# kuwt/model_matching

Measured on AMD Instinct MI355X. Metric: candidate poses verified/sec, higher is better.
Workload: dtype f32; 1 GPU; Cm: synthetic 20000-pt scene vs 5000-pt model, 65536 candidate transforms per step per GPU, eps=5mm; scene_points=20000, model_points=5000

## Files before the change

### include/stocs_hip.h

```cpp
#ifndef STOCS_HIP_H
#define STOCS_HIP_H

#include <stdint.h>

#ifdef __cplusplus
extern "C" {
#endif

typedef struct stocs_ctx stocs_ctx;

typedef enum stocs_status {
    STOCS_OK = 0,
    STOCS_ERR_INVALID = -1,
    STOCS_ERR_NO_DEVICE = -2,
    STOCS_ERR_HIP = -3,
    STOCS_ERR_CAPACITY = -4,
    STOCS_ERR_STATE = -5,
    STOCS_ERR_NOMEM = -6
} stocs_status;

typedef struct stocs_params {
    float distance_threshold;
    int   ppf_tr_discretization;
    int   ppf_rot_discretization;
    float plane_threshold;
    float min_distance_base;
    float internal_angle_threshold;
    float lcp_normal_angle;
    int   image_width, image_height;
    int   number_of_bases;
    int   maximum_congruent_sets;
} stocs_params;

void stocs_default_params(stocs_params* p);
const char* stocs_last_error(void);
const char* stocs_version(void);

int stocs_ctx_create(const stocs_params* prm,
                     const float* scene_pos3, const float* scene_nrm3, const float* scene_prob,
                     const int32_t* scene_pixel2, int nS,
                     const float* model_pos3, const float* model_nrm3, int nM,
                     int build_index, int device, stocs_ctx** out);
int stocs_ctx_destroy(stocs_ctx* ctx);
int stocs_ctx_set_scene(stocs_ctx* ctx, const float* scene_pos3, const float* scene_nrm3, const float* scene_prob,
                        const int32_t* scene_pixel2, int nS);

int stocs_get_centroids(const stocs_ctx* ctx, float* scene3, float* model3);
int stocs_get_sizes(const stocs_ctx* ctx, int* nS, int* nM);
int stocs_set_edge_map(stocs_ctx* ctx, const uint8_t* edge);
int stocs_reset_trial(stocs_ctx* ctx);

int stocs_ppf_compute_host(const float* p1, const float* n1, const float* p2, const float* n2,
                           int tr, int rot, int32_t* key4);
int stocs_index_exists(const stocs_ctx* ctx, const int32_t* key4, int* exists);
int stocs_index_lookup(stocs_ctx* ctx, const int32_t* key4, int32_t* pairs2, int64_t cap, int64_t* n);
int stocs_index_stats(const stocs_ctx* ctx, int64_t* n_pairs, int64_t* n_buckets, int64_t* n_keys);
int stocs_index_save(stocs_ctx* ctx, const char* path);
int stocs_index_load(stocs_ctx* ctx, const char* path);

int stocs_sample_bases(stocs_ctx* ctx, int mode, uint64_t seed, int first_attempt, int n_attempts,
                       float dispersion, int32_t* base_ids4, float* inv2, int32_t* valid);
int stocs_get_segment(const stocs_ctx* ctx, int32_t* scene_idx, int cap, int* n);
int stocs_get_scene(const stocs_ctx* ctx, float* pos3_centred, float* nrm3, float* class_prob, int32_t* pixel2);
int stocs_set_bases(stocs_ctx* ctx, int n, const int32_t* base_ids4, const float* inv2);
int stocs_clear_bases(stocs_ctx* ctx);
int stocs_num_bases(const stocs_ctx* ctx);
int stocs_class_pass(stocs_ctx* ctx, int pass, const int32_t* b3, const float* w_in, float* w_out);
int stocs_ppf_filter_check(stocs_ctx* ctx, uint64_t seed, int64_t n_pairs, int64_t* n_tested, int64_t* n_undecided, int64_t* n_mismatch);
int stocs_weight_fix_check(stocs_ctx* ctx, int64_t* n_mismatch);
int stocs_try_sampled_base(stocs_ctx* ctx, int32_t* ids4_inout, float* inv2, int* valid);
int stocs_draw(stocs_ctx* ctx, const float* w, int n, uint64_t r64, int* index);
enum { STOCS_FORM_LEAN = 0, STOCS_FORM_FULL_LDS = 1, STOCS_FORM_FULL_DEVICE_MEMORY = 2, STOCS_FORM_NINE_LAUNCH = 3, STOCS_FORM_INSTANCE_LDS = 4,
       STOCS_FORM_INSTANCE_DEVICE_MEMORY = 5 };
int stocs_last_sampling_form(const stocs_ctx* ctx, int* kernel, int* threads, int64_t* lds_bytes, int* cap, int* launches, int* redone);
int stocs_last_instance_attempts(stocs_ctx* ctx, int32_t* rec4, int cap, int* n);
int stocs_debug_draw_point1(stocs_ctx* ctx, const uint64_t* r64, int n, int32_t* index);

int stocs_find_congruent_all(stocs_ctx* ctx, int64_t* total_quads);
int stocs_get_quads(stocs_ctx* ctx, int base_slot, int32_t* quads4, int64_t cap, int64_t* n);
int stocs_get_quads_at(stocs_ctx* ctx, int base_slot, const int64_t* ranks, int n, int32_t* quads4);

int stocs_cone_cells_host(const float* n3, float cos_alpha, uint32_t* exact_bits11, uint32_t* kernel_bits11, int* n_samples,
                          int* n_undecided);

int stocs_make_transforms(stocs_ctx* ctx, int max_per_base, uint64_t seed, int* n_candidates);
int stocs_rigid_transform(stocs_ctx* ctx, const int32_t* ids4, const int32_t* quad4,
                          float* T16_centred, float* pose16_camera, int* ok);
int stocs_get_candidates(stocs_ctx* ctx, float* T16_centred, float* pose16_camera, float* lcp,
                         int32_t* base_index, int cap, int* n);

int stocs_score_transforms(stocs_ctx* ctx, const float* T16_centred_host, int n, float* lcp_host);
int stocs_score_transforms_device(stocs_ctx* ctx, const void* d_T16, int n, void* d_lcp);
int stocs_score_best_device(stocs_ctx* ctx, const void* d_T16, int n, void* d_lcp, uint32_t id_offset, uint64_t* key);
int stocs_score_best_device_async(stocs_ctx* ctx, const void* d_T16, int n, void* d_lcp, uint32_t id_offset, void* d_key8);
int stocs_lcp_detail(stocs_ctx* ctx, const float* T16_centred_host, int32_t* hit, uint8_t* counted);
int stocs_lcp_hit_count(stocs_ctx* ctx, const void* d_T16, int n, int64_t* hits, int64_t* counted);
int stocs_verify_all(stocs_ctx* ctx, float* best_lcp, int* best_idx, float* best_pose16_camera);
typedef struct stocs_trial_result {
    int32_t n_bases;
    int32_t n_candidates;
    int64_t n_quads;
    float   best_lcp;
    int32_t best_index;
    float   best_pose16[16];
} stocs_trial_result;
int stocs_run_trials(stocs_ctx* ctx, int mode, int n_trials, const uint64_t* seeds, int n_attempts, float dispersion, int max_per_base,
                     int keep_details, stocs_trial_result* out );
int stocs_trials_get_bases(stocs_ctx* ctx, int trial, int32_t* base_ids4, float* inv2, int32_t* valid, int cap_attempts, int* n_attempts);
int stocs_trials_get_quad_counts(stocs_ctx* ctx, int trial, int64_t* counts, int cap, int* n);
int stocs_trials_get_candidates(stocs_ctx* ctx, int trial, float* T16_centred, float* pose16_camera, float* lcp, int32_t* base_index, int cap, int* n);
typedef struct stocs_trial_post {
    float   acceptable_fraction;
    int32_t maximum_pose_count;
    float   min_distance, min_angle;
    float   sym3[3];
    int32_t refine_iterations;
    float   max_correspondence_distance;
} stocs_trial_post;
int stocs_run_trials_post(stocs_ctx* ctx, int mode, int n_trials, const uint64_t* seeds, int n_attempts, float dispersion, int max_per_base,
                          int keep_details, const stocs_trial_post* post , stocs_trial_result* out );
typedef struct stocs_trial_hypothesis {
    int32_t candidate_index, base_index;
    float   lcp, pose16[16];
    float   refined_lcp, refined_pose16[16];
    int32_t n_correspondences, iterations;
} stocs_trial_hypothesis;
int stocs_trials_get_hypotheses(stocs_ctx* ctx, int trial, stocs_trial_hypothesis* out, int cap, int* n);

int stocs_best_device(stocs_ctx* ctx, const void* d_lcp, int n, uint32_t id_offset, uint64_t* key);
uint64_t stocs_pack_best(float lcp, uint32_t global_candidate_id);
void stocs_unpack_best(uint64_t key, float* lcp, uint32_t* global_candidate_id);

typedef struct stocs_comm stocs_comm;
int stocs_comm_unique_id(void* id128);
int stocs_comm_create(const void* id128, int nranks, int rank, int device, stocs_comm** out);
int stocs_comm_destroy(stocs_comm* comm);
int stocs_allreduce_best(stocs_comm* comm, void* hip_stream, uint64_t* key_inout, float* pose16_inout, uint32_t ids_per_rank);

int stocs_cluster_poses(const float* poses16, const float* lcp, int n, float acceptable_fraction,
                        float best_score, int maximum_pose_count, float min_distance, float min_angle,
                        const float* sym3, int32_t* out_idx, int cap, int* n_out);
int stocs_cluster_trials_device(stocs_ctx* ctx, const float* poses16, const float* lcp, const int32_t* cand_off, const float* best_score, int n_trials,
                                float acceptable_fraction, int maximum_pose_count, float min_distance, float min_angle, const float* sym3,
                                int32_t* out_off, int32_t* out_cnt, int32_t* out_idx, int out_cap, int32_t* round0_survivors);

enum {
    STOCS_NORMALS_DEPTH_GRADIENT = 0,
    STOCS_NORMALS_PLANE_FIT = 1
};
typedef struct stocs_camera {
    float fx, cx, fy, cy;
    float depth_scale;
    int width, height;
    int normal_method;
} stocs_camera;
int stocs_ingest_scene(const stocs_camera* cam, const uint16_t* depth, const uint16_t* class_prob, float voxel_size,
                       float class_threshold, int device, float* pos3, float* nrm3, float* prob, int32_t* pixel2,
                       int cap, int* n_out);
#define STOCS_MAX_FRAME_OBJECTS 64
int stocs_ingest_scene_multi(const stocs_camera* cam, const uint16_t* depth, int n_objects, const uint16_t* class_probs,
                             const float* class_thresholds, float voxel_size, int device, float* pos3, float* nrm3, float* prob,
                             int32_t* pixel2, int cap, int32_t* offsets);
int stocs_preprocess_model(const float* raw_pos3, int n_raw, float normal_radius, float voxel_size, float model_scale,
                           int device, float* pos3, float* nrm3, int cap, int* n_out);
int stocs_trim(void);

int stocs_png_read(const char* path, int* width, int* height, int* channels, int* bit_depth, void* pixels, int64_t cap_bytes);
int stocs_ply_read(const char* path, float* pos3, float* nrm3, int cap, int* n, int* has_normals);
int stocs_ply_write(const char* path, const float* pos3, const float* nrm3, int n, float scale);

int stocs_icp_point_to_plane(const float* src_pos3, int nsrc, const float* tgt_pos3, const float* tgt_nrm3, int ntgt,
                             int max_iterations, float max_correspondence_distance, int device, float* T16_out,
                             int* n_correspondences);

int stocs_refine_poses(stocs_ctx* ctx, const float* T16_centred_in, int n, const int32_t* src_idx, int n_src, int max_iterations,
                       float max_correspondence_distance, float* T16_centred_out, float* pose16_camera_out, float* lcp_out,
                       int32_t* n_corr_out, int32_t* iterations_out);

int stocs_refine_detail(stocs_ctx* ctx, const float* T16_centred, const int32_t* src_idx, int n_src, float max_correspondence_distance,
// ... 152 lines not shown
```

### model_matching_amd/capi.py

```python
from __future__ import annotations

import ctypes as C
import os

import numpy as np

_HERE = os.path.dirname(os.path.abspath(__file__))
LIB_PATH = os.path.join(_HERE, "libstocs_hip.so")

STOCS_OK = 0
ERR_INVALID, ERR_CAPACITY, ERR_STATE = -1, -4, -5
FORM_NAMES = {0: "lean", 1: "full_lds", 2: "full_device_memory", 3: "nine_launch", 4: "instance_lds", 5: "instance_device_memory"}
ERR_NAMES = {0: "OK", -1: "INVALID", -2: "NO_DEVICE", -3: "HIP", -4: "CAPACITY", -5: "STATE", -6: "NOMEM"}


class StocsError(RuntimeError):
    def __init__(self, code, msg):
        super().__init__("stocs_hip error %s: %s" % (ERR_NAMES.get(code, code), msg))
        self.code = code


class Params(C.Structure):
    _fields_ = [("distance_threshold", C.c_float), ("ppf_tr_discretization", C.c_int),
                ("ppf_rot_discretization", C.c_int), ("plane_threshold", C.c_float),
# ... 50 lines not shown
    _fields_ = [("max_instances", C.c_int32), ("min_points", C.c_int32), ("min_exclusive_fraction", C.c_float)]


class InstanceResult(C.Structure):
    _fields_ = [("rank", C.c_int32), ("own", C.c_int32), ("exclusive", C.c_int32), ("lcp", C.c_float)]


class RenderParams(C.Structure):
    _fields_ = [("point_radius", C.c_float), ("max_splat_px", C.c_int32), ("tolerance", C.c_float), ("class_threshold", C.c_float)]


class RenderResult(C.Structure):
    _fields_ = [("footprint", C.c_int32), ("visible", C.c_int32), ("hidden", C.c_int32), ("no_depth", C.c_int32), ("agree", C.c_int32),
                ("in_front", C.c_int32), ("behind", C.c_int32), ("on_mask", C.c_int32)]


class SceneRecord(C.Structure):
    _fields_ = [("footprint", C.c_int32), ("no_depth", C.c_int32), ("agree", C.c_int32), ("in_front", C.c_int32), ("behind", C.c_int32),
                ("on_mask", C.c_int32), ("claimed", C.c_int32)]


class SceneParams(C.Structure):
    _fields_ = [("max_selected", C.c_int32), ("min_pixels", C.c_int32), ("min_exclusive_fraction", C.c_float), ("max_violation_fraction", C.c_float)]


class SceneResult(C.Structure):
    _fields_ = [("rank", C.c_int32), ("own", C.c_int32), ("exclusive", C.c_int32), ("reason", C.c_int32)]


class Camera(C.Structure):
    _fields_ = [("fx", C.c_float), ("cx", C.c_float), ("fy", C.c_float), ("cy", C.c_float), ("depth_scale", C.c_float),
                ("width", C.c_int), ("height", C.c_int), ("normal_method", C.c_int)]


_fp, _ip, _u8p, _vp = C.POINTER(C.c_float), C.POINTER(C.c_int32), C.POINTER(C.c_uint8), C.c_void_p
_i64p = C.POINTER(C.c_int64)
_intp = C.POINTER(C.c_int)
SIGNATURES = {
    "stocs_default_params": (None, [C.POINTER(Params)]),
    "stocs_last_error": (C.c_char_p, []),
    "stocs_version": (C.c_char_p, []),
    "stocs_ctx_create": (C.c_int, [C.POINTER(Params), _fp, _fp, _fp, _ip, C.c_int, _fp, _fp, C.c_int, C.c_int, C.c_int, C.POINTER(_vp)]),
    "stocs_ctx_destroy": (C.c_int, [_vp]),
    "stocs_ctx_set_scene": (C.c_int, [_vp, _fp, _fp, _fp, _ip, C.c_int]),
    "stocs_get_centroids": (C.c_int, [_vp, _fp, _fp]),
    "stocs_get_sizes": (C.c_int, [_vp, _intp, _intp]),
    "stocs_set_edge_map": (C.c_int, [_vp, _u8p]),
    "stocs_reset_trial": (C.c_int, [_vp]),
    "stocs_ppf_compute_host": (C.c_int, [_fp, _fp, _fp, _fp, C.c_int, C.c_int, _ip]),
    "stocs_index_exists": (C.c_int, [_vp, _ip, _intp]),
    "stocs_index_lookup": (C.c_int, [_vp, _ip, _ip, C.c_int64, _i64p]),
    "stocs_index_stats": (C.c_int, [_vp, _i64p, _i64p, _i64p]),
    "stocs_index_save": (C.c_int, [_vp, C.c_char_p]),
    "stocs_index_load": (C.c_int, [_vp, C.c_char_p]),
    "stocs_sample_bases": (C.c_int, [_vp, C.c_int, C.c_uint64, C.c_int, C.c_int, C.c_float, _ip, _fp, _ip]),
    "stocs_get_segment": (C.c_int, [_vp, _ip, C.c_int, _intp]),
    "stocs_get_scene": (C.c_int, [_vp, _fp, _fp, _fp, _ip]),
    "stocs_png_read": (C.c_int, [C.c_char_p, _intp, _intp, _intp, _intp, _vp, C.c_int64]),
    "stocs_ply_read": (C.c_int, [C.c_char_p, _fp, _fp, C.c_int, _intp, _intp]),
    "stocs_ply_write": (C.c_int, [C.c_char_p, _fp, _fp, C.c_int, C.c_float]),
    "stocs_set_bases": (C.c_int, [_vp, C.c_int, _ip, _fp]),
    "stocs_clear_bases": (C.c_int, [_vp]),
    "stocs_num_bases": (C.c_int, [_vp]),
    "stocs_class_pass": (C.c_int, [_vp, C.c_int, _ip, _fp, _fp]),
    "stocs_ppf_filter_check": (C.c_int, [_vp, C.c_uint64, C.c_int64, _i64p, _i64p, _i64p]),
    "stocs_weight_fix_check": (C.c_int, [_vp, _i64p]),
    "stocs_try_sampled_base": (C.c_int, [_vp, _ip, _fp, _intp]),
    "stocs_draw": (C.c_int, [_vp, _fp, C.c_int, C.c_uint64, _intp]),
    "stocs_last_sampling_form": (C.c_int, [_vp, _intp, _intp, _i64p, _intp, _intp, _intp]),
    "stocs_last_instance_attempts": (C.c_int, [_vp, _ip, C.c_int, _intp]),
    "stocs_debug_draw_point1": (C.c_int, [_vp, C.POINTER(C.c_uint64), C.c_int, _ip]),
    "stocs_find_congruent_all": (C.c_int, [_vp, _i64p]),
    "stocs_get_quads": (C.c_int, [_vp, C.c_int, _ip, C.c_int64, _i64p]),
    "stocs_get_quads_at": (C.c_int, [_vp, C.c_int, _i64p, C.c_int, _ip]),
    "stocs_cone_cells_host": (C.c_int, [_fp, C.c_float, C.POINTER(C.c_uint32), C.POINTER(C.c_uint32), _intp, _intp]),
    "stocs_make_transforms": (C.c_int, [_vp, C.c_int, C.c_uint64, _intp]),
    "stocs_rigid_transform": (C.c_int, [_vp, _ip, _ip, _fp, _fp, _intp]),
    "stocs_get_candidates": (C.c_int, [_vp, _fp, _fp, _fp, _ip, C.c_int, _intp]),
    "stocs_score_transforms": (C.c_int, [_vp, _fp, C.c_int, _fp]),
    "stocs_score_transforms_device": (C.c_int, [_vp, _vp, C.c_int, _vp]),
    "stocs_score_best_device": (C.c_int, [_vp, _vp, C.c_int, _vp, C.c_uint32, C.POINTER(C.c_uint64)]),
    "stocs_lcp_detail": (C.c_int, [_vp, _fp, _ip, _u8p]),
    "stocs_lcp_hit_count": (C.c_int, [_vp, _vp, C.c_int, _i64p, _i64p]),
    "stocs_verify_all": (C.c_int, [_vp, _fp, _intp, _fp]),
    "stocs_run_trials": (C.c_int, [_vp, C.c_int, C.c_int, C.POINTER(C.c_uint64), C.c_int, C.c_float, C.c_int, C.c_int, C.POINTER(TrialResult)]),
    "stocs_trials_get_bases": (C.c_int, [_vp, C.c_int, _ip, _fp, _ip, C.c_int, _intp]),
    "stocs_trials_get_quad_counts": (C.c_int, [_vp, C.c_int, _i64p, C.c_int, _intp]),
    "stocs_trials_get_candidates": (C.c_int, [_vp, C.c_int, _fp, _fp, _fp, _ip, C.c_int, _intp]),
    "stocs_run_trials_post": (C.c_int, [_vp, C.c_int, C.c_int, C.POINTER(C.c_uint64), C.c_int, C.c_float, C.c_int, C.c_int, C.POINTER(TrialPost),
                                        C.POINTER(TrialResult)]),
    "stocs_trials_get_hypotheses": (C.c_int, [_vp, C.c_int, C.POINTER(TrialHypothesis), C.c_int, _intp]),
    "stocs_best_device": (C.c_int, [_vp, _vp, C.c_int, C.c_uint32, C.POINTER(C.c_uint64)]),
    "stocs_pack_best": (C.c_uint64, [C.c_float, C.c_uint32]),
    "stocs_unpack_best": (None, [C.c_uint64, _fp, C.POINTER(C.c_uint32)]),
    "stocs_comm_unique_id": (C.c_int, [_vp]),
    "stocs_comm_create": (C.c_int, [_vp, C.c_int, C.c_int, C.c_int, C.POINTER(_vp)]),
    "stocs_comm_destroy": (C.c_int, [_vp]),
    "stocs_allreduce_best": (C.c_int, [_vp, _vp, C.POINTER(C.c_uint64), _fp, C.c_uint32]),
    "stocs_cluster_poses": (C.c_int, [_fp, _fp, C.c_int, C.c_float, C.c_float, C.c_int, C.c_float, C.c_float, _fp, _ip, C.c_int, _intp]),
    "stocs_cluster_trials_device": (C.c_int, [_vp, _fp, _fp, _ip, _fp, C.c_int, C.c_float, C.c_int, C.c_float, C.c_float, _fp, _ip, _ip, _ip, C.c_int, _ip]),
    "stocs_ingest_scene": (C.c_int, [C.POINTER(Camera), C.POINTER(C.c_uint16), C.POINTER(C.c_uint16), C.c_float, C.c_float, C.c_int, _fp, _fp, _fp, _ip, C.c_int, _intp]),
    "stocs_ingest_scene_multi": (C.c_int, [C.POINTER(Camera), C.POINTER(C.c_uint16), C.c_int, C.POINTER(C.c_uint16), _fp, C.c_float, C.c_int, _fp, _fp, _fp, _ip,
                                           C.c_int, _ip]),
    "stocs_preprocess_model": (C.c_int, [_fp, C.c_int, C.c_float, C.c_float, C.c_float, C.c_int, _fp, _fp, C.c_int, _intp]),
    "stocs_trim": (C.c_int, []),
    "stocs_icp_point_to_plane": (C.c_int, [_fp, C.c_int, _fp, _fp, C.c_int, C.c_int, C.c_float, C.c_int, _fp, _intp]),
    "stocs_refine_poses": (C.c_int, [_vp, _fp, C.c_int, _ip, C.c_int, C.c_int, C.c_float, _fp, _fp, _fp, _ip, _ip]),
    "stocs_refine_detail": (C.c_int, [_vp, _fp, _ip, C.c_int, C.c_float, _ip, _u8p, C.POINTER(C.c_double)]),
    "stocs_refine_poses_robust": (C.c_int, [_vp, _fp, C.c_int, _ip, C.c_int, C.POINTER(RefineRobustParams), _fp, _fp, _fp, _ip, _ip, _ip]),
    "stocs_refine_robust_detail": (C.c_int, [_vp, _fp, _ip, C.c_int, C.POINTER(RefineRobustParams), _ip, _u8p, _u8p, C.POINTER(C.c_uint32), _ip, _ip,
                                             C.POINTER(C.c_double)]),
    "stocs_refine_robust_workspace": (C.c_int, [_vp, C.POINTER(C.c_void_p), C.POINTER(C.c_uint64)]),
    "stocs_track_poses": (C.c_int, [_vp, _fp, C.c_int, C.POINTER(TrackParams), C.POINTER(TrackResult)]),
    "stocs_track_get_round": (C.c_int, [_vp, C.c_int, C.c_int, _fp, _fp, C.c_int, _intp]),
    "stocs_ctx_set_frame": (C.c_int, [_vp, C.POINTER(Camera), C.POINTER(C.c_uint16), C.POINTER(C.c_uint16)]),
    "stocs_default_depth_params": (None, [C.POINTER(DepthParams)]),
    "stocs_depth_check_poses": (C.c_int, [_vp, _fp, C.c_int, C.POINTER(DepthParams), C.POINTER(DepthResult)]),
    "stocs_pose_errors": (C.c_int, [_vp, _fp, C.c_int, _fp, C.c_int, C.POINTER(PoseError)]),
    "stocs_pose_errors_detail": (C.c_int, [_vp, _fp, _fp, _fp, _fp, _ip]),
    "stocs_model_diameter": (C.c_int, [_vp, _fp]),
    "stocs_default_render_params": (None, [C.POINTER(RenderParams)]),
    "stocs_render_poses": (C.c_int, [_vp, _fp, C.c_int, C.c_int, C.POINTER(RenderParams), _vp, C.c_int]),
    "stocs_render_resolve": (C.c_int, [_vp, _fp, C.c_int, C.c_int, C.POINTER(RenderParams), _vp, C.POINTER(RenderResult)]),
    "stocs_render_labels": (C.c_int, [_vp, _vp, C.POINTER(RenderParams), _ip, _u8p]),
    "stocs_explain_poses": (C.c_int, [_vp, _fp, C.c_int, C.POINTER(RenderParams), C.POINTER(RenderResult), _ip, _u8p]),
    "stocs_default_instance_params": (None, [C.POINTER(InstanceParams)]),
    "stocs_select_instances": (C.c_int, [_vp, _fp, C.c_int, C.POINTER(InstanceParams), C.POINTER(InstanceResult), _ip, _intp]),
    "stocs_select_instances_rows": (C.c_int, [_vp, _ip, _u8p, _fp, C.c_int, C.c_int, C.c_int, C.POINTER(InstanceParams), C.POINTER(InstanceResult), _ip, _intp]),
    "stocs_default_scene_params": (None, [C.POINTER(SceneParams)]),
    "stocs_scene_row_words": (C.c_int, [C.c_int, C.c_int]),
    "stocs_scene_footprints": (C.c_int, [_vp, _fp, C.c_int, C.c_int, C.c_int, C.POINTER(RenderParams), C.c_int, _vp, C.POINTER(SceneRecord)]),
    "stocs_scene_select": (C.c_int, [_vp, _vp, C.c_int, C.c_int, C.c_int, _fp, _ip, C.POINTER(SceneRecord), C.c_int, _ip, C.POINTER(SceneParams),
                                     C.POINTER(SceneResult), _ip, _intp]),
    "stocs_device_alloc_count": (C.c_int64, []),
    "stocs_debug_stream_audit_selftest": (C.c_int, [C.c_int, C.c_char_p, C.c_int]),
    "stocs_debug_streams_overlap": (C.c_int, [_vp]),
    "stocs_debug_sort_pairs": (C.c_int, [C.c_int, C.POINTER(C.c_uint32), C.POINTER(C.c_uint32), C.c_int64, C.c_int, C.c_int, C.c_int, C.POINTER(C.c_uint32), C.POINTER(C.c_uint32), _fp, C.POINTER(C.c_uint32), C.c_int]),
    "stocs_last_call_timing": (C.c_int, [_vp, C.c_int, C.POINTER(C.c_char_p), C.POINTER(C.c_double), C.c_int, _intp]),
    "stocs_set_option": (C.c_int, [_vp, C.c_char_p, C.c_int]),
    "stocs_get_cull_state": (C.c_int, [_vp, _fp, _ip, _intp, _fp, _fp, C.c_int64, _i64p]),
    "stocs_model_patch_order": (C.c_int, [_fp, C.c_int, _ip, _fp]),
    "stocs_model_subpatches": (C.c_int, [_fp, C.c_int, _ip, _fp]),
    "stocs_kdtree_nn_host": (C.c_int, [_fp, C.c_int, _fp, C.c_int, C.c_float, _ip]),
    "stocs_last_tie_counts": (C.c_int, [_vp, _i64p, _i64p]),
    "stocs_set_stream": (C.c_int, [_vp, _vp]),
    "stocs_best_device_async": (C.c_int, [_vp, _vp, C.c_int, C.c_uint32, _vp]),
    "stocs_score_best_device_async": (C.c_int, [_vp, _vp, C.c_int, _vp, C.c_uint32, _vp]),
    "stocs_sync": (C.c_int, [_vp]),
    "stocs_stream": (_vp, [_vp]),
    "stocs_time_score_kernel": (C.c_int, [_vp, _vp, C.c_int, _vp, C.c_int, _fp]),
    "stocs_dev_alloc": (C.c_int, [_vp, C.c_int64, C.POINTER(_vp)]),
    "stocs_dev_free": (C.c_int, [_vp, _vp]),
    "stocs_dev_upload": (C.c_int, [_vp, _vp, _vp, C.c_int64]),
    "stocs_dev_download": (C.c_int, [_vp, _vp, _vp, C.c_int64]),
}

_LIB = None


def load():
    global _LIB
    if _LIB is None:
        if not os.path.exists(LIB_PATH):
            raise ImportError("%s is missing: build it with `python -c 'import __graft_entry__ as g; g.build()'` "
                              "(make -C model_matching_amd/csrc).  There is no CPU fallback." % LIB_PATH)
        L = C.CDLL(LIB_PATH)
# ... 30 lines not shown
```

### model_matching_amd/csrc/ctx.hip

```cpp
#include <math.h>
#include <stdarg.h>
#include <string.h>
#include <stdlib.h>

#include <algorithm>
#include <limits>
#include <numeric>

#include "stocs_ctx.h"

namespace stocs {

static thread_local char g_err[512] = "";
unsigned long long g_dev_allocs = 0;

void set_error(const char* fmt, ...) {
    va_list ap;
    va_start(ap, fmt);
    vsnprintf(g_err, sizeof(g_err), fmt, ap);
    va_end(ap);
}

__global__ void overlap_wait_kernel(unsigned int* flag, unsigned int* seen) {
    const unsigned long long t0 = wall_clock64();
// ... 380 lines not shown
    float r_ref = 0.0f;
    model_patch_order(mpos, munit, perm, patch, sub, &r_ref);
}

}

using namespace stocs;

extern "C" {

const char* stocs_last_error(void) { return g_err; }
const char* stocs_version(void) { return "stocs_hip 0.1 (gfx950)"; }

void stocs_default_params(stocs_params* p) {
    p->distance_threshold = 0.005f;
    p->ppf_tr_discretization = 5;
    p->ppf_rot_discretization = 5;
    p->plane_threshold = 0.015f;
    p->min_distance_base = 0.01f;
    p->internal_angle_threshold = 30.0f;
    p->lcp_normal_angle = 30.0f;
    p->image_width = 640;
    p->image_height = 480;
    p->number_of_bases = 100;
    p->maximum_congruent_sets = 200;
}

int stocs_ctx_create(const stocs_params* prm, const float* sp, const float* sn, const float* sprob,
                     const int32_t* spix, int nS, const float* mp, const float* mn, int nM, int build_index,
                     int device, stocs_ctx** out) {
    if (!prm || !out || nS < 0 || nM < 0 || (nS && (!sp || !sn || !sprob)) || (nM && (!mp || !mn))) {
        set_error("stocs_ctx_create: invalid argument");
        return STOCS_ERR_INVALID;
    }
    if (nS == 0 || nM == 0) {
        set_error("stocs_ctx_create: empty scene or model cloud");
        return STOCS_ERR_INVALID;
    }
    if (nM > 65535) { set_error("model has %d points; at most 65535 supported (16-bit ids in packed pairs)", nM); return STOCS_ERR_INVALID; }
    if (prm->ppf_rot_discretization <= 0 || prm->ppf_tr_discretization <= 0 || 180 % prm->ppf_rot_discretization) {
        set_error("PPF discretisation must be positive and divide 180");
        return STOCS_ERR_INVALID;
    }
    *out = NULL;
    int ndev = 0;
    if (hipGetDeviceCount(&ndev) != hipSuccess || ndev <= 0) {
        set_error("no HIP device available: this library has no CPU fallback");
        return STOCS_ERR_NO_DEVICE;
    }
    if (device < 0) { if (hipGetDevice(&device) != hipSuccess) device = 0; }
    if (device >= ndev) { set_error("device %d out of range (%d devices)", device, ndev); return STOCS_ERR_NO_DEVICE; }
    DeviceGuard dev_guard(device);
    { int cur = -1; if (hipGetDevice(&cur) != hipSuccess || cur != device) { set_error("hipSetDevice(%d) failed", device); return STOCS_ERR_NO_DEVICE; } }

    stocs_ctx* c = new stocs_ctx();
    c->prm = *prm;
    c->device = device;
    c->nS = nS; c->nM = nM;
    c->d_scratch = NULL; c->scratch_bytes = 0;
    c->h_pin = NULL; c->pin_bytes = 0;
    for (int k = 0; k < 5; ++k) c->timing[k].n = 0;
    c->index.built = false;
    c->index.d_bucket_start = NULL; c->index.d_pairs = NULL; c->index.d_exists = NULL;
    c->cong = NULL; c->quad_id_bits = 16;
    c->refine = NULL;
    c->track = NULL;
    c->depth = NULL;
    c->instances = NULL;
    c->render = NULL;
    c->scene = NULL;
    c->pose_error = NULL;
    c->inst = NULL;
    c->trials = NULL; c->snrmw_trial0 = NULL; c->snrmw_stride = 0; c->snrmw_override = NULL; c->lcp_cand_trial = NULL;
    c->d_cand = NULL; c->cand_bytes = 0; c->n_cands = 0; c->cand_cap = 0; c->cands_stale = false;
    c->d_best = NULL; c->best_is_zero = false;
    c->best_lcp = 0; c->best_index = -1;
    c->has_edge = false;
    c->grid_div = 1;
    c->grid_prune = getenv("STOCS_GRID_PRUNE") ? atoi(getenv("STOCS_GRID_PRUNE")) : 1;
    c->lcp_variant = -1;
    c->device_clock = (getenv("STOCS_DEVICE_CLOCK") && atoi(getenv("STOCS_DEVICE_CLOCK")) != 0) ? 1 : 0;
    c->lcp_split = 1;
    c->lcp_flat = getenv("STOCS_LCP_FLAT") ? atoi(getenv("STOCS_LCP_FLAT")) : 1;
    c->lcp_order = getenv("STOCS_LCP_ORDER") ? atoi(getenv("STOCS_LCP_ORDER")) : 1;
    c->exact_ties = 0; c->kd_ready = false; c->d_kd_nodes = NULL; c->d_kd_pts = NULL; c->d_ties = NULL; c->ties_started = false;
    c->cdf_n = 0; c->prior_epoch = 1; c->cdf_epoch = 0;
    c->last_form.kernel = -1; c->last_form.threads = 0; c->last_form.lds = 0; c->last_form.cap = 0; c->last_form.launches = 0; c->last_form.redone = 0;
    memset(&c->grid, 0, sizeof(c->grid));
    c->d_spos = c->d_snrmw = c->d_mpos = c->d_mnrm = c->d_munit = c->d_mpos_raw = c->d_mpos_s = c->d_mnrm_s = NULL;
    c->d_spix = NULL; c->d_mperm = NULL; c->d_mpatch = NULL; c->d_msub = NULL; c->d_scene_mem = NULL; c->scene_cap = 0;
    c->patch_r_ref = 0.0f; c->scene_scored = 0; c->scene_work = 0.0;
    c->lcp_cull = getenv("STOCS_LCP_CULL") ? atoi(getenv("STOCS_LCP_CULL")) : 1;
    c->lcp_cull_unit = 16;
    c->lcp_cull_after = 1.0e9; c->prev_scene_warm = false; c->cull_pending = false; c->ev_cull = NULL;
    c->stream = NULL; c->own_stream = NULL; c->aux_stream = NULL;
    if (hipStreamCreateWithFlags(&c->own_stream, hipStreamNonBlocking) != hipSuccess || hipStreamCreateWithFlags(&c->aux_stream, hipStreamNonBlocking) != hipSuccess ||
        hipEventCreate(&c->ev0) != hipSuccess || hipEventCreate(&c->ev1) != hipSuccess ||
        hipEventCreateWithFlags(&c->ev_fork, hipEventDisableTiming) != hipSuccess || hipEventCreateWithFlags(&c->ev_join, hipEventDisableTiming) != hipSuccess ||
        hipEventCreateWithFlags(&c->ev_cull, hipEventDisableTiming) != hipSuccess) {
        set_error("stream/event creation failed");
        delete c;
        return STOCS_ERR_NO_DEVICE;
    }
    for (int k = 0; k < 10; ++k)
        if (hipEventCreate(&c->ev_t[k]) != hipSuccess) { set_error("event creation failed"); delete c; return STOCS_ERR_NO_DEVICE; }
    if (!getenv("STOCS_NO_STREAM_PROBE")) {
        hipStream_t spare[4]; int n_spare = 0;
        while (!streams_run_side_by_side(c->own_stream, c->aux_stream) && n_spare < 4) {
            hipStream_t s2 = NULL;
            if (hipStreamCreateWithFlags(&s2, hipStreamNonBlocking) != hipSuccess) { (void)hipGetLastError(); break; }
            spare[n_spare++] = c->aux_stream;
            c->aux_stream = s2;
        }
        for (int k = 0; k < n_spare; ++k) (void)hipStreamDestroy(spare[k]);
        if (getenv("STOCS_DEBUG_TIMING")) fprintf(stderr, "[stocs ctx] auxiliary stream: candidate %d runs next to the main stream\n", n_spare + 1);
    }
    c->stream = c->own_stream;
    compute_thresholds(c->prm, &c->thr);

    c->h_mpos.resize(nM); c->h_mnrm.resize(nM); c->h_mpos_raw.resize(nM);
    for (int i = 0; i < nM; ++i) {
        c->h_mpos_raw[i] = c->h_mpos[i] = mk3(mp[3 * i], mp[3 * i + 1], mp[3 * i + 2]);
        c->h_mnrm[i] = normalized3(mk3(mn[3 * i], mn[3 * i + 1], mn[3 * i + 2]));
    }
    V3 cm = mk3(0, 0, 0);
    for (int i = 0; i < nM; ++i) cm = cm + c->h_mpos[i];
    cm = cm / (float)nM;
    for (int i = 0; i < nM; ++i) c->h_mpos[i] = c->h_mpos[i] - cm;
    c->centroid_model = cm;

    {
        const float big = std::numeric_limits<float>::max() / 2;
        V3 bmn = mk3(big, big, big), bmx = mk3(-big, -big, -big);
        for (int i = 0; i < nM; ++i) {
            const V3 q = c->h_mpos[i];
            if (q.x < bmn.x) bmn.x = q.x; if (q.y < bmn.y) bmn.y = q.y; if (q.z < bmn.z) bmn.z = q.z;
            if (q.x > bmx.x) bmx.x = q.x; if (q.y > bmx.y) bmx.y = q.y; if (q.z > bmx.z) bmx.z = q.z;
        }
        c->gcenter = bmn + ((bmx - bmn) / 2.0f);
        const V3 ext = bmx - bmn;
        const double r = std::max((double)ext.z + 0.001, std::max((double)ext.y + 0.001, (double)ext.x + 0.001));
        c->ratio = (float)r;
        c->h_munit.resize(nM);
        const V3 half = mk3(0.5f, 0.5f, 0.5f);
        for (int i = 0; i < nM; ++i) c->h_munit[i] = (c->h_mpos[i] - c->gcenter) / c->ratio + half;
    }

    std::vector<float4> patch, sub;
    model_patch_order(c->h_mpos, c->h_munit, c->h_mperm, patch, sub, &c->patch_r_ref);
    const int n_patch = (nM + 63) / 64;

    int rc = STOCS_OK;
    {
        const int n = std::max(nM, 1);
        std::vector<float4> a(n), b(n), u(n), raw(n), as(n), bs(n);
        for (int i = 0; i < nM; ++i) {
            a[i] = make_float4(c->h_mpos[i].x, c->h_mpos[i].y, c->h_mpos[i].z, 0.f);
            b[i] = make_float4(c->h_mnrm[i].x, c->h_mnrm[i].y, c->h_mnrm[i].z, 0.f);
            u[i] = make_float4(c->h_munit[i].x, c->h_munit[i].y, c->h_munit[i].z, 0.f);
            raw[i] = make_float4(c->h_mpos_raw[i].x, c->h_mpos_raw[i].y, c->h_mpos_raw[i].z, 0.f);
        }
        for (int i = 0; i < nM; ++i) { as[i] = a[c->h_mperm[i]]; bs[i] = b[c->h_mperm[i]]; }
        as.resize((size_t)n_patch * 64 + 64, make_float4(NAN, NAN, NAN, 0.f));
        if (!rc) rc = upload(&c->d_mpos, a.data(), a.size());
        if (!rc) rc = upload(&c->d_mnrm, b.data(), b.size());
        if (!rc) rc = upload(&c->d_munit, u.data(), u.size());
        if (!rc) rc = upload(&c->d_mpos_raw, raw.data(), raw.size());
        if (!rc) rc = upload(&c->d_mpos_s, as.data(), as.size());
        if (!rc) rc = upload(&c->d_mnrm_s, bs.data(), bs.size());
        if (!rc) rc = upload(&c->d_mperm, c->h_mperm.data(), c->h_mperm.size());
        if (!rc) rc = upload(&c->d_mpatch, patch.data(), patch.size());
        if (!rc) rc = upload(&c->d_msub, sub.data(), sub.size());
    }
    if (!rc) rc = load_scene(c, sp, sn, sprob, spix, nS);
    if (!rc && build_index) rc = build_ppf_index(c);
    if (rc) { stocs_ctx_destroy(c); return rc; }
    *out = c;
    return STOCS_OK;
}

int stocs_model_patch_order(const float* model_pos3, int nM, int32_t* perm, float* patches4) {
    if (!model_pos3 || nM <= 0 || !perm || !patches4) return STOCS_ERR_INVALID;
    std::vector<int32_t> pm; std::vector<float4> patch, sub;
    model_patch_order_host(model_pos3, nM, pm, patch, sub);
    for (int i = 0; i < nM; ++i) perm[i] = pm[i];
    for (int s = 0; s < (nM + 63) / 64; ++s) { patches4[4 * s] = patch[s].x; patches4[4 * s + 1] = patch[s].y; patches4[4 * s + 2] = patch[s].z; patches4[4 * s + 3] = patch[s].w; }
    return STOCS_OK;
}

int stocs_model_subpatches(const float* model_pos3, int nM, int32_t* perm, float* spheres4) {
    if (!model_pos3 || nM <= 0 || !perm || !spheres4) return STOCS_ERR_INVALID;
    std::vector<int32_t> pm; std::vector<float4> patch, sub;
    model_patch_order_host(model_pos3, nM, pm, patch, sub);
    for (int i = 0; i < nM; ++i) perm[i] = pm[i];
    for (int q = 0; q < (nM + 15) / 16; ++q) { spheres4[4 * q] = sub[q].x; spheres4[4 * q + 1] = sub[q].y; spheres4[4 * q + 2] = sub[q].z; spheres4[4 * q + 3] = sub[q].w; }
    return STOCS_OK;
}

int stocs_ctx_destroy(stocs_ctx* c) {
    if (!c) return STOCS_OK;
    DeviceGuard dev_guard(c->device);
    if (c->stream) (void)hipStreamSynchronize(c->stream);
    void* ptrs[] = {c->d_scene_mem, c->d_mpos, c->d_mnrm, c->d_munit, c->d_mpos_raw, c->d_mpos_s,
                    c->d_mnrm_s, c->d_mperm, c->d_mpatch, c->d_msub, c->index.d_bucket_start,
                    c->index.d_pairs, c->index.d_exists, c->d_scratch, c->d_best, c->d_cand};
    stocs_internal_free_congruent(c);
    stocs_internal_free_instance(c);
    stocs_internal_free_trials(c);
    stocs_internal_free_refine(c);
    stocs_internal_free_track(c);
    stocs_internal_free_depth(c);
    stocs_internal_free_instances(c);
    stocs_internal_free_render(c);
    stocs_internal_free_scene(c);
    stocs_internal_free_pose_error(c);
    c->grid_mem.destroy(); c->grid_ws.destroy();
    c->order.free(); c->cdf.free(); c->kd.free();
    if (c->h_pin) (void)hipHostFree(c->h_pin);
    for (void* p : ptrs) if (p) (void)hipFree(p);
    (void)hipEventDestroy(c->ev0);
    (void)hipEventDestroy(c->ev1);
    (void)hipEventDestroy(c->ev_fork);
    (void)hipEventDestroy(c->ev_join);
    if (c->ev_cull) (void)hipEventDestroy(c->ev_cull);
    for (int k = 0; k < 10; ++k) (void)hipEventDestroy(c->ev_t[k]);
    if (c->aux_stream) { (void)hipStreamSynchronize(c->aux_stream); (void)hipStreamDestroy(c->aux_stream); }
    if (c->own_stream) (void)hipStreamDestroy(c->own_stream);
    delete c;
    return STOCS_OK;
}

int stocs_ctx_set_scene(stocs_ctx* c, const float* sp, const float* sn, const float* sprob, const int32_t* spix, int nS) {
    if (!c || nS <= 0 || !sp || !sn || !sprob) { set_error("stocs_ctx_set_scene: invalid argument"); return STOCS_ERR_INVALID; }
    DeviceGuard dev_guard(c->device);
    STOCS_HIP_CHECK(hipStreamSynchronize(c->stream));
    return load_scene(c, sp, sn, sprob, spix, nS);
}

int stocs_get_centroids(const stocs_ctx* c, float* s, float* m) {
    if (!c) return STOCS_ERR_INVALID;
    if (s) { s[0] = c->centroid_scene.x; s[1] = c->centroid_scene.y; s[2] = c->centroid_scene.z; }
    if (m) { m[0] = c->centroid_model.x; m[1] = c->centroid_model.y; m[2] = c->centroid_model.z; }
    return STOCS_OK;
}
int stocs_get_scene(const stocs_ctx* c, float* pos3, float* nrm3, float* prob, int32_t* pix2) {
    if (!c) return STOCS_ERR_INVALID;
// ... 114 lines not shown
```

### model_matching_amd/csrc/grid.hip

```cpp
#include <math.h>
#include <string.h>
#include <cstring>


#include <algorithm>
#include <vector>

#include "prims.h"
#include "stocs_ctx.h"

namespace stocs {

struct GridGeom {
    double of[3];
    double h, r;
    int n[3];
    int nbx, nby;
    int dense;
    double qscale;
};

__device__ __forceinline__ void cell_range(const GridGeom& G, const double p[3], int lo[3], int hi[3]) {
#pragma unroll
    for (int k = 0; k < 3; ++k) {
        lo[k] = max(0, (int)floor((p[k] - G.r - G.of[k]) / G.h));
        hi[k] = min(G.n[k] - 1, (int)floor((p[k] + G.r - G.of[k]) / G.h));
    }
}

__device__ __forceinline__ double box_dist2(const GridGeom& G, const double p[3], int cx, int cy, int cz) {
    const int cc[3] = {cx, cy, cz};
    double d2 = 0;
#pragma unroll
    for (int k = 0; k < 3; ++k) {
        const double b0 = G.of[k] + cc[k] * G.h, b1 = b0 + G.h;
        const double d = p[k] < b0 ? b0 - p[k] : (p[k] > b1 ? p[k] - b1 : 0.0);
        d2 += d * d;
    }
    return d2;
}

template <bool FILL>
__global__ __launch_bounds__(256) void incidence_kernel(GridGeom G, const float4* __restrict__ spos, int nS, uint32_t* __restrict__ cnt,
                                                        const unsigned long long* __restrict__ off, uint64_t* __restrict__ keys,
                                                        uint32_t* __restrict__ vals, uint32_t* __restrict__ keys32 = NULL) {
    const int i = blockIdx.x * blockDim.x + threadIdx.x;
    if (i >= nS) return;
    const float4 pf = spos[i];
    const double p[3] = {pf.x, pf.y, pf.z};
    int lo[3], hi[3];
    cell_range(G, p, lo, hi);
    uint32_t c = 0;
    unsigned long long o = FILL ? off[i] : 0ull;
    for (int cz = lo[2]; cz <= hi[2]; ++cz)
        for (int cy = lo[1]; cy <= hi[1]; ++cy)
            for (int cx = lo[0]; cx <= hi[0]; ++cx) {
                if (box_dist2(G, p, cx, cy, cz) > G.r * G.r) continue;
                if (FILL) {
                    const uint64_t brick = ((uint64_t)(cz >> 3) * G.nby + (uint64_t)(cy >> 3)) * G.nbx + (uint64_t)(cx >> 3);
                    uint64_t key = (brick << 9) | (uint64_t)(((cz & 7) << 6) | ((cy & 7) << 3) | (cx & 7));
                    if (G.dense) {
                        const double dx = p[0] - (G.of[0] + (cx + 0.5) * G.h), dy = p[1] - (G.of[1] + (cy + 0.5) * G.h),
                                     dz = p[2] - (G.of[2] + (cz + 0.5) * G.h);
                        const double q = sqrt(dx * dx + dy * dy + dz * dz) * G.qscale;
                        key = (key << 16) | (uint64_t)(q < 65535.0 ? (unsigned)q : 65535u);
                    }
                    if (keys32) keys32[o + c] = (uint32_t)key; else keys[o + c] = key;
                    vals[o + c] = (uint32_t)i;
                }
                c++;
            }
    if (!FILL) cnt[i] = c;
}

__global__ __launch_bounds__(256) void widen_keys_kernel(const uint32_t* __restrict__ k32, size_t n, uint64_t* __restrict__ k64) {
    const size_t e = (size_t)blockIdx.x * blockDim.x + threadIdx.x;
    if (e < n) k64[e] = (uint64_t)k32[e];
}

__global__ __launch_bounds__(256) void cell_flags_kernel(const uint64_t* __restrict__ keys, size_t n, int qbits, uint32_t* __restrict__ cflag,
                                                         uint32_t* __restrict__ bflag) {
    const size_t e = (size_t)blockIdx.x * blockDim.x + threadIdx.x;
    if (e >= n) return;
    const uint64_t ck = keys[e] >> qbits;
    const uint64_t pk = e ? (keys[e - 1] >> qbits) : ~0ull;
    cflag[e] = (e == 0 || ck != pk) ? 1u : 0u;
    bflag[e] = (e == 0 || (ck >> 9) != (pk >> 9)) ? 1u : 0u;
}

__global__ __launch_bounds__(256) void cell_records_kernel(const uint64_t* __restrict__ keys, size_t n, int qbits, const uint32_t* __restrict__ cflag,
                                                           const uint32_t* __restrict__ cidx, const uint32_t* __restrict__ bflag,
                                                           const uint32_t* __restrict__ bidx, uint32_t* __restrict__ cell_first, uint64_t* __restrict__ cell_key,
                                                           uint32_t* __restrict__ cell_brick) {
    const size_t e = (size_t)blockIdx.x * blockDim.x + threadIdx.x;
    if (e >= n || !cflag[e]) return;
    const uint32_t c = cidx[e];
    cell_first[c] = (uint32_t)e;
    cell_key[c] = keys[e] >> qbits;
    cell_brick[c] = bidx[e] + bflag[e] - 1u;
}

__global__ __launch_bounds__(256) void cell_padded_kernel(const uint32_t* __restrict__ cell_first, uint32_t n_cells, uint32_t n_inc, uint32_t pad,
                                                          uint32_t* __restrict__ padded, uint32_t* __restrict__ max_count) {
    const uint32_t c = blockIdx.x * blockDim.x + threadIdx.x;
    if (c >= n_cells) return;
    const uint32_t cnt = (c + 1 < n_cells ? cell_first[c + 1] : n_inc) - cell_first[c];
    padded[c] = (cnt + pad - 1u) & ~(pad - 1u);
    atomicMax(max_count, cnt);
}

__global__ __launch_bounds__(256) void fill_i32_kernel(int32_t* __restrict__ a, size_t n, int32_t v) {
    const size_t i = (size_t)blockIdx.x * blockDim.x + threadIdx.x;
    if (i < n) a[i] = v;
}
__global__ __launch_bounds__(256) void fill_list_kernel(float4* __restrict__ a, size_t n) {
    const size_t i = (size_t)blockIdx.x * blockDim.x + threadIdx.x;
    if (i < n) a[i] = make_float4(1.0e30f, 1.0e30f, 1.0e30f, __int_as_float(-1));
}
__global__ __launch_bounds__(256) void zero_cells_kernel(uint4* __restrict__ a, size_t n) {
    const size_t i = (size_t)blockIdx.x * blockDim.x + threadIdx.x;
    if (i < n) a[i] = make_uint4(0u, 0u, 0u, 0u);
}

__global__ __launch_bounds__(256) void cell_words_kernel(GridGeom G, int div, const uint32_t* __restrict__ cell_first, const uint64_t* __restrict__ cell_key,
                                                         const uint32_t* __restrict__ cell_brick, const uint32_t* __restrict__ list_off,
                                                         uint32_t n_cells, uint32_t n_inc, const uint32_t* __restrict__ vals,
                                                         const float4* __restrict__ spos, int32_t* __restrict__ top, uint4* __restrict__ cells,
                                                         uint4* __restrict__ flat, const uint32_t* __restrict__ kept) {
    const uint32_t c = blockIdx.x * 4 + (threadIdx.x >> 6);
    const int s = threadIdx.x & 63;
    if (c >= n_cells) return;
    const uint32_t first = cell_first[c];
    const uint32_t cnt = (c + 1 < n_cells ? cell_first[c + 1] : n_inc) - first;
    const uint64_t key = cell_key[c];
    const uint64_t brick = key >> 9;
    const uint32_t local = (uint32_t)(key & 511);
    const uint32_t b = cell_brick[c];
    uint32_t mlo = 0xFFFFFFFFu, mhi = 0xFFFFFFFFu;
    if (div == 1) {
        const int bx = (int)(brick % (uint64_t)G.nbx), by = (int)((brick / (uint64_t)G.nbx) % (uint64_t)G.nby),
                  bz = (int)(brick / ((uint64_t)G.nbx * (uint64_t)G.nby));
        const int cx = bx * 8 + (int)(local & 7), cy = by * 8 + (int)((local >> 3) & 7), cz = bz * 8 + (int)(local >> 6);
        const double hs = G.h / 4.0;
        const int sc[3] = {4 * cx + (s & 3), 4 * cy + ((s >> 2) & 3), 4 * cz + (s >> 4)};
        bool any = false;
        for (uint32_t k = 0; k < cnt && !any; ++k) {
            const float4 pf = spos[vals[first + k]];
            const double p[3] = {pf.x, pf.y, pf.z};
            double d2 = 0;
#pragma unroll
            for (int a = 0; a < 3; ++a) {
                const double b0 = G.of[a] + sc[a] * hs, b1 = b0 + hs;
                const double d = p[a] < b0 ? b0 - p[a] : (p[a] > b1 ? p[a] - b1 : 0.0);
                d2 += d * d;
            }
            any = d2 <= G.r * G.r;
        }
        const unsigned long long m = __ballot(any);
        mlo = (uint32_t)(m & 0xFFFFFFFFull); mhi = (uint32_t)(m >> 32);
    }
    if (s == 0) {
        top[brick] = (int32_t)b;
        const uint4 w = make_uint4(list_off[c], kept ? kept[c] : cnt, mlo, mhi);
        cells[(size_t)b * 512 + local] = w;
        if (flat) {
            const int bx = (int)(brick % (uint64_t)G.nbx), by = (int)((brick / (uint64_t)G.nbx) % (uint64_t)G.nby), bz = (int)(brick / ((uint64_t)G.nbx * (uint64_t)G.nby));
            const int cx = bx * 8 + (int)(local & 7), cy = by * 8 + (int)((local >> 3) & 7), cz = bz * 8 + (int)(local >> 6);
            if (cx < G.n[0] && cy < G.n[1] && cz < G.n[2]) flat[((size_t)cz * G.n[1] + cy) * G.n[0] + cx] = w;
        }
    }
}

__global__ __launch_bounds__(256) void list_fill_kernel(const uint32_t* __restrict__ cflag, const uint32_t* __restrict__ cidx,
                                                        const uint32_t* __restrict__ cell_first, const uint32_t* __restrict__ list_off,
                                                        const uint32_t* __restrict__ vals, size_t n, const float4* __restrict__ spos,
                                                        float4* __restrict__ list, const uint32_t* __restrict__ rank) {
    const size_t e = (size_t)blockIdx.x * blockDim.x + threadIdx.x;
    if (e >= n) return;
    if (rank) {
        const uint32_t r = rank[e];
        if (r == 0xFFFFFFFFu) return;
        const uint32_t c = cidx[e] + cflag[e] - 1u;
        const uint32_t pt = vals[e];
        const float4 p = spos[pt];
        list[(size_t)list_off[c] + r] = make_float4(p.x, p.y, p.z, __int_as_float((int)pt));
        return;
    }
    const uint32_t c = cidx[e] + cflag[e] - 1u;
    const uint32_t pt = vals[e];
    const float4 p = spos[pt];
    list[(size_t)list_off[c] + (e - cell_first[c])] = make_float4(p.x, p.y, p.z, __int_as_float((int)pt));
}

__global__ __launch_bounds__(256) void chunk_bounds_kernel(GridGeom G, const uint32_t* __restrict__ cell_first, const uint64_t* __restrict__ cell_key,
                                                           const uint32_t* __restrict__ list_off, uint32_t n_cells, uint32_t n_inc,
                                                           const float4* __restrict__ list, float* __restrict__ chunk_r) {
    const uint32_t c = blockIdx.x * blockDim.x + threadIdx.x;
    if (c >= n_cells) return;
    const uint32_t cnt = (c + 1 < n_cells ? cell_first[c + 1] : n_inc) - cell_first[c];
    const uint64_t key = cell_key[c];
    const uint64_t brick = key >> 9;
    const uint32_t local = (uint32_t)(key & 511);
    const int bx = (int)(brick % (uint64_t)G.nbx), by = (int)((brick / (uint64_t)G.nbx) % (uint64_t)G.nby),
              bz = (int)(brick / ((uint64_t)G.nbx * (uint64_t)G.nby));
    const int cx = bx * 8 + (int)(local & 7), cy = by * 8 + (int)((local >> 3) & 7), cz = bz * 8 + (int)(local >> 6);
    const double ccx = G.of[0] + (cx + 0.5) * G.h, ccy = G.of[1] + (cy + 0.5) * G.h, ccz = G.of[2] + (cz + 0.5) * G.h;
    const uint32_t o = list_off[c];
    double run = 1e300;
    for (int k = (int)cnt - 1; k >= 0; --k) {
        const float4 e = list[(size_t)o + k];
        const double dx = e.x - ccx, dy = e.y - ccy, dz = e.z - ccz;
        run = fmin(run, sqrt(dx * dx + dy * dy + dz * dz));
        if ((k & 7) == 0) chunk_r[(o + (uint32_t)k) >> 3] = (float)(run - (2e-6 + 2.5e-7 * run));
    }
}

__global__ __launch_bounds__(256) void cell_nearest_kernel(const uint64_t* __restrict__ cell_key, const uint32_t* __restrict__ cell_brick, const uint32_t* __restrict__ list_off,
                                                           uint32_t n_cells, const float* __restrict__ chunk_r, uint4* __restrict__ cells) {
    const uint32_t c = blockIdx.x * blockDim.x + threadIdx.x;
    if (c >= n_cells) return;
    cells[(size_t)cell_brick[c] * 512 + (uint32_t)(cell_key[c] & 511)].z = __float_as_uint(chunk_r[list_off[c] >> 3]);
}


template <int PRUNE_K, int GS>
__global__ __launch_bounds__(256) void prune_kernel(GridGeom G, double hh, double margin, const uint32_t* __restrict__ cell_first, const uint64_t* __restrict__ cell_key,
                                                    uint32_t n_cells, uint32_t n_inc, const uint32_t* __restrict__ vals, const float4* __restrict__ spos,
                                                    uint32_t* __restrict__ rank, uint32_t* __restrict__ kept, float* __restrict__ nearest) {
    const uint32_t c = blockIdx.x * (256u / GS) + (threadIdx.x / GS);
    const int lane = threadIdx.x & (GS - 1), wlane = threadIdx.x & 63;
    const bool cell_ok = c < n_cells;
    const uint32_t first = cell_ok ? cell_first[c] : 0u;
    const uint32_t cnt = cell_ok ? (c + 1 < n_cells ? cell_first[c + 1] : n_inc) - first : 0u;
    const uint64_t key = cell_ok ? cell_key[c] : 0ull;
    const uint64_t brick = key >> 9;
    const uint32_t local = (uint32_t)(key & 511);
    const int bx = (int)(brick % (uint64_t)G.nbx), by = (int)((brick / (uint64_t)G.nbx) % (uint64_t)G.nby), bz = (int)(brick / ((uint64_t)G.nbx * (uint64_t)G.nby));
    const int cx = bx * 8 + (int)(local & 7), cy = by * 8 + (int)((local >> 3) & 7), cz = bz * 8 + (int)(local >> 6);
    const double ccx = G.of[0] + (cx + 0.5) * G.h, ccy = G.of[1] + (cy + 0.5) * G.h, ccz = G.of[2] + (cz + 0.5) * G.h;
    double ux0 = 0, uy0 = 0, uz0 = 0, n20 = 0;
    if ((uint32_t)lane < cnt) {
        const float4 pf = spos[vals[first + (uint32_t)lane]];
        ux0 = (double)pf.x - ccx; uy0 = (double)pf.y - ccy; uz0 = (double)pf.z - ccz;
        n20 = ux0 * ux0 + uy0 * uy0 + uz0 * uz0;
    }
    double dux[PRUNE_K], duy[PRUNE_K], duz[PRUNE_K], dn2[PRUNE_K];
// ... 36 lines not shown
        const uint32_t k = k0 + (uint32_t)lane;
        bool keep = false;
        if (k < cnt) {
            double ux = ux0, uy = uy0, uz = uz0, n2 = n20;
            if (k0) {
                const float4 pf = spos[vals[first + k]];
                ux = (double)pf.x - ccx; uy = (double)pf.y - ccy; uz = (double)pf.z - ccz;
                n2 = ux * ux + uy * uy + uz * uz;
            }
            keep = true;
#pragma unroll
            for (int j = 0; j < PRUNE_K; ++j) {
                if (j < nd) {
                    const double fmin_ = (n2 - dn2[j]) - 2.0 * hh * (fabs(ux - dux[j]) + fabs(uy - duy[j]) + fabs(uz - duz[j]));
                    if (fmin_ > margin) keep = false;
                }
            }
        }
        unsigned long long m = __ballot(keep);
        if (GS < 64) m = (m >> (wlane & ~(GS - 1))) & ((1ull << GS) - 1ull);
        if (k < cnt) rank[first + k] = keep ? base + (uint32_t)__popcll(m & ((1ull << lane) - 1ull)) : 0xFFFFFFFFu;
        base += (uint32_t)__popcll(m);
    }
    if (lane == 0 && cell_ok) {
        kept[c] = base;
        const double d0 = nd ? sqrt(dn2[0]) : 0.0;
        nearest[c] = (float)fmax(d0 - (2e-6 + 2.5e-7 * d0), 0.0);
    }
}

__global__ __launch_bounds__(256) void cell_padded_kept_kernel(const uint32_t* __restrict__ kept, uint32_t n_cells, uint32_t pad, uint32_t* __restrict__ padded,
                                                               uint32_t* __restrict__ max_count, unsigned long long* __restrict__ total) {
    const uint32_t c = blockIdx.x * blockDim.x + threadIdx.x;
    if (c >= n_cells) return;
    const uint32_t cnt = kept[c];
    padded[c] = (cnt + pad - 1u) & ~(pad - 1u);
    atomicMax(max_count, cnt);
    unsigned long long t = cnt;
    for (int off = 32; off > 0; off >>= 1) t += __shfl_xor(t, off, 64);
    if ((threadIdx.x & 63) == 0) atomicAdd(total, t);
}

__global__ __launch_bounds__(256) void cell_nearest_store_kernel(const uint64_t* __restrict__ cell_key, const uint32_t* __restrict__ cell_brick, uint32_t n_cells,
                                                                 const float* __restrict__ nearest, uint4* __restrict__ cells) {
    const uint32_t c = blockIdx.x * blockDim.x + threadIdx.x;
    if (c >= n_cells) return;
    cells[(size_t)cell_brick[c] * 512 + (uint32_t)(cell_key[c] & 511)].z = __float_as_uint(nearest[c]);
}

struct Tmp {
    Arena* ws;
    template <class T>
    int get(T** p, size_t n) { return ws->take(std::max<size_t>(n, 1) * sizeof(T), (void**)p); }
};

static inline unsigned grid_of(size_t n) { return (unsigned)((n + 255) / 256); }

int build_grid_gpu(stocs_ctx* c, int div, int dense, int prune) {
    if (prune) dense = 0;
    SceneGrid& g = c->grid;
    const int nS = c->nS;
    const double eps = (double)c->prm.distance_threshold;
    if (div < 1 || div > 4) div = 1;
    const double h = eps / div;
    const double r = eps * 1.001;
    double mn[3] = {1e30, 1e30, 1e30}, mx[3] = {-1e30, -1e30, -1e30};
    for (int i = 0; i < nS; ++i) {
        const V3 p = c->h_spos[i];
        const double v[3] = {p.x, p.y, p.z};
        for (int k = 0; k < 3; ++k) { mn[k] = std::min(mn[k], v[k]); mx[k] = std::max(mx[k], v[k]); }
    }
    if (nS == 0) { for (int k = 0; k < 3; ++k) { mn[k] = 0; mx[k] = 0; } }
    for (int k = 0; k < 3; ++k) { g.bb_mn[k] = mn[k]; g.bb_mx[k] = mx[k]; }
    g.d_dist = NULL; g.dist_ready = false;
    const double pad = r + 2 * h;
    const double o[3] = {mn[0] - pad, mn[1] - pad, mn[2] - pad};
    int n[3];
    for (int k = 0; k < 3; ++k) n[k] = (int)floor((mx[k] + pad - o[k]) / h) + 1;
    g.ox = (float)o[0]; g.oy = (float)o[1]; g.oz = (float)o[2];
    g.inv_h = (float)(1.0 / h);
    g.nx = n[0]; g.ny = n[1]; g.nz = n[2];
    g.nbx = (n[0] + 7) / 8; g.nby = (n[1] + 7) / 8; g.nbz = (n[2] + 7) / 8;
    g.h = (float)h;
    g.n_bricks = 0; g.n_entries = 0; g.avg_list_len = 0; g.has_nearest = false;
    g.d_top = NULL; g.d_cells = NULL; g.d_list = NULL; g.d_chunk_r = NULL; g.d_flat = NULL;
    const int64_t n_top = (int64_t)g.nbx * g.nby * g.nbz;
    if (n_top > (int64_t)400 * 1000 * 1000) { set_error("scene extent too large for the brick grid"); return STOCS_ERR_INVALID; }
    int cell_bits = 1;
    while (((int64_t)1 << cell_bits) < n_top * 512) cell_bits++;

    GridGeom G;
    G.of[0] = g.ox; G.of[1] = g.oy; G.of[2] = g.oz;
    G.h = h; G.r = r;
    G.n[0] = n[0]; G.n[1] = n[1]; G.n[2] = n[2];
    G.nbx = g.nbx; G.nby = g.nby;
    G.dense = dense ? 1 : 0;
    G.qscale = 65535.0 / (r + h * 0.8660254037844387 + 1e-9);
    const int qbits = dense ? 16 : 0;

    hipStream_t st = c->stream;
    Tmp T;
    T.ws = &c->grid_ws;
    int rc;
    STOCS_HIP_CHECK(hipStreamSynchronize(st));
    if ((rc = c->grid_ws.reset()) || (rc = c->grid_mem.reset())) return rc;
    if ((rc = c->grid_mem.take((size_t)std::max<int64_t>(n_top, 1) * 4, (void**)&g.d_top))) return rc;
    hipLaunchKernelGGL(fill_i32_kernel, dim3(grid_of((size_t)n_top)), dim3(256), 0, st, g.d_top, (size_t)n_top, -1);
    if (nS == 0) {
        if ((rc = c->grid_mem.take(16, (void**)&g.d_cells)) || (rc = c->grid_mem.take(8 * 16, (void**)&g.d_list))) return rc;
        STOCS_HIP_CHECK(hipStreamSynchronize(st));
        return STOCS_OK;
    }
    uint32_t* d_cnt; unsigned long long* d_off;
    if ((rc = T.get(&d_cnt, (size_t)nS + 1)) || (rc = T.get(&d_off, (size_t)nS + 1))) return rc;
    hipLaunchKernelGGL(incidence_kernel<false>, dim3(grid_of(nS)), dim3(256), 0, st, G, c->d_spos, nS, d_cnt, (const unsigned long long*)NULL,
                       (uint64_t*)NULL, (uint32_t*)NULL);
    hipLaunchKernelGGL(fill_i32_kernel, dim3(1), dim3(256), 0, st, (int32_t*)(d_cnt + nS), (size_t)1, 0);
    size_t tb = 0;
    STOCS_HIP_CHECK(exclusive_scan(NULL, tb, d_cnt, d_off, (size_t)nS + 1, st));
    char* d_tmp;
    if ((rc = T.get(&d_tmp, tb))) return rc;
    STOCS_HIP_CHECK(exclusive_scan(d_tmp, tb, d_cnt, d_off, (size_t)nS + 1, st));
    if ((rc = ensure_pinned(c, PIN_VAR))) return rc;
    unsigned long long* rb64 = (unsigned long long*)((char*)c->h_pin + PIN_BEST + 128);
    uint32_t* rb32 = (uint32_t*)((char*)c->h_pin + PIN_BEST + 160);
    rb64[0] = 0; rb64[1] = 0; for (int k = 0; k < 5; ++k) rb32[k] = 0;
    STOCS_HIP_CHECK(hipMemcpyAsync(&rb64[0], d_off + nS, 8, hipMemcpyDeviceToHost, st));
    STOCS_HIP_CHECK(hipStreamSynchronize(st));
    const unsigned long long n_inc64 = rb64[0];
    if (n_inc64 >= (1ull << 28)) { set_error("scene grid lists too large (%llu incidences)", n_inc64); return STOCS_ERR_INVALID; }
    const size_t n_inc = (size_t)n_inc64;
    uint64_t *d_keys, *d_keys_s; uint32_t *d_vals, *d_vals_s;
    if ((rc = T.get(&d_keys, n_inc)) || (rc = T.get(&d_keys_s, n_inc)) || (rc = T.get(&d_vals, n_inc)) || (rc = T.get(&d_vals_s, n_inc))) return rc;
    size_t ts = 0;
    const unsigned end_bit = (unsigned)std::min(64, cell_bits + qbits);
    const bool own_sort = end_bit <= 32 && n_inc >= 65536 && n_inc < ((size_t)1 << 30) && !(getenv("STOCS_SORT") && !strcmp(getenv("STOCS_SORT"), "rocprim"));
    char* d_ts;
    const uint32_t* d_sort_err = NULL;
    if (own_sort) {
        uint32_t* k32 = (uint32_t*)d_keys;
        uint32_t* k32s = k32 + n_inc;
        hipLaunchKernelGGL(incidence_kernel<true>, dim3(grid_of(nS)), dim3(256), 0, st, G, c->d_spos, nS, (uint32_t*)NULL, d_off, (uint64_t*)NULL, d_vals, k32);
        STOCS_HIP_CHECK(hipGetLastError());
        STOCS_HIP_CHECK(sort_pairs_own(NULL, ts, k32, k32s, d_vals, d_vals_s, n_inc, 0, end_bit, NULL, 1, st));
        if ((rc = T.get(&d_ts, ts))) return rc;
        STOCS_HIP_CHECK(sort_pairs_own(d_ts, ts, k32, k32s, d_vals, d_vals_s, n_inc, 0, end_bit, NULL, 1, st));
        hipLaunchKernelGGL(widen_keys_kernel, dim3(grid_of(n_inc)), dim3(256), 0, st, (const uint32_t*)k32s, n_inc, d_keys_s);
        d_sort_err = (const uint32_t*)(d_ts + sort_own_err_offset());
    } else {
    hipLaunchKernelGGL(incidence_kernel<true>, dim3(grid_of(nS)), dim3(256), 0, st, G, c->d_spos, nS, (uint32_t*)NULL, d_off, d_keys, d_vals);
    STOCS_HIP_CHECK(hipGetLastError());
    STOCS_HIP_CHECK(sort_pairs(NULL, ts, d_keys, d_keys_s, d_vals, d_vals_s, n_inc, 0, end_bit, st));
    if ((rc = T.get(&d_ts, ts))) return rc;
    STOCS_HIP_CHECK(sort_pairs(d_ts, ts, d_keys, d_keys_s, d_vals, d_vals_s, n_inc, 0, end_bit, st));
    }
    uint32_t *d_cflag, *d_bflag, *d_cidx, *d_bidx;
    if ((rc = T.get(&d_cflag, n_inc + 1)) || (rc = T.get(&d_bflag, n_inc + 1)) || (rc = T.get(&d_cidx, n_inc + 1)) || (rc = T.get(&d_bidx, n_inc + 1))) return rc;
    hipLaunchKernelGGL(cell_flags_kernel, dim3(grid_of(n_inc)), dim3(256), 0, st, d_keys_s, n_inc, qbits, d_cflag, d_bflag);
    hipLaunchKernelGGL(fill_i32_kernel, dim3(1), dim3(256), 0, st, (int32_t*)(d_cflag + n_inc), (size_t)1, 0);
    hipLaunchKernelGGL(fill_i32_kernel, dim3(1), dim3(256), 0, st, (int32_t*)(d_bflag + n_inc), (size_t)1, 0);
    size_t t32 = 0;
    STOCS_HIP_CHECK(exclusive_scan(NULL, t32, d_cflag, d_cidx, (size_t)n_inc + 1, st));
    char* d_t32;
    if ((rc = T.get(&d_t32, t32))) return rc;
    STOCS_HIP_CHECK(exclusive_scan(d_t32, t32, d_cflag, d_cidx, (size_t)n_inc + 1, st));
    STOCS_HIP_CHECK(exclusive_scan(d_t32, t32, d_bflag, d_bidx, (size_t)n_inc + 1, st));
    uint32_t* counts = rb32;
    STOCS_HIP_CHECK(hipMemcpyAsync(&counts[0], d_cidx + n_inc, 4, hipMemcpyDeviceToHost, st));
    STOCS_HIP_CHECK(hipMemcpyAsync(&counts[1], d_bidx + n_inc, 4, hipMemcpyDeviceToHost, st));
    if (d_sort_err) STOCS_HIP_CHECK(hipMemcpyAsync(&rb32[2], d_sort_err, 4, hipMemcpyDeviceToHost, st));
    STOCS_HIP_CHECK(hipStreamSynchronize(st));
    const uint32_t sort_err = rb32[2];
    if (sort_err) { set_error("scene grid: the incidence sort gave up waiting for a tile (sort32.hip)"); return STOCS_ERR_HIP; }
    const uint32_t n_cells = counts[0], n_bricks = counts[1];
    uint32_t *d_cell_first, *d_cell_brick, *d_padded, *d_list_off, *d_max;
    uint64_t* d_cell_key;
    if ((rc = T.get(&d_cell_first, (size_t)n_cells + 1)) || (rc = T.get(&d_cell_brick, (size_t)n_cells + 1)) || (rc = T.get(&d_padded, (size_t)n_cells + 1)) ||
        (rc = T.get(&d_list_off, (size_t)n_cells + 1)) || (rc = T.get(&d_cell_key, (size_t)n_cells + 1)) || (rc = T.get(&d_max, 1)))
        return rc;
    hipLaunchKernelGGL(cell_records_kernel, dim3(grid_of(n_inc)), dim3(256), 0, st, d_keys_s, n_inc, qbits, d_cflag, d_cidx, d_bflag, d_bidx, d_cell_first,
                       d_cell_key, d_cell_brick);
    hipLaunchKernelGGL(fill_i32_kernel, dim3(1), dim3(256), 0, st, (int32_t*)d_max, (size_t)1, 0);
    uint32_t *d_rank = NULL, *d_kept = NULL; float* d_near = NULL; unsigned long long* d_total = NULL;
    if (prune) {
        if ((rc = T.get(&d_rank, n_inc + 1)) || (rc = T.get(&d_kept, (size_t)n_cells + 1)) || (rc = T.get(&d_near, (size_t)n_cells + 1)) || (rc = T.get(&d_total, 1))) return rc;
        double ext = 0; for (int k = 0; k < 3; ++k) ext = std::max(ext, (double)n[k] * h);
        const double hh = 0.5 * h + 2.0e-6 * (ext + 1.0) * 0.5 + 1.0e-7, reach = r + 2.0 * h;
        const double margin = 4.0e-6 * reach * reach;
        hipLaunchKernelGGL(fill_i32_kernel, dim3(1), dim3(256), 0, st, (int32_t*)d_total, (size_t)2, 0);
        const int pk = getenv("STOCS_GRID_PRUNE_K") ? atoi(getenv("STOCS_GRID_PRUNE_K")) : 8;
#define STOCS_PRUNE_LAUNCH(KV) do { if (short_lists) hipLaunchKernelGGL((prune_kernel<KV, 16>), dim3((unsigned)((n_cells + 15) / 16)), dim3(256), 0, st, G, hh, margin, d_cell_first, d_cell_key, n_cells, (uint32_t)n_inc, d_vals_s, c->d_spos, d_rank, d_kept, d_near); \
                                    else hipLaunchKernelGGL((prune_kernel<KV, 64>), dim3((unsigned)((n_cells + 3) / 4)), dim3(256), 0, st, G, hh, margin, d_cell_first, d_cell_key, n_cells, (uint32_t)n_inc, d_vals_s, c->d_spos, d_rank, d_kept, d_near); } while (0)
        const bool short_lists = (double)n_inc <= 12.0 * (double)n_cells;
        if (pk == 4) STOCS_PRUNE_LAUNCH(4); else if (pk == 16) STOCS_PRUNE_LAUNCH(16); else STOCS_PRUNE_LAUNCH(8);
#undef STOCS_PRUNE_LAUNCH
        hipLaunchKernelGGL(cell_padded_kept_kernel, dim3(grid_of(n_cells)), dim3(256), 0, st, d_kept, n_cells, 8u, d_padded, d_max, d_total);
    } else
    hipLaunchKernelGGL(cell_padded_kernel, dim3(grid_of(n_cells)), dim3(256), 0, st, d_cell_first, n_cells, (uint32_t)n_inc, 8u, d_padded, d_max);
    hipLaunchKernelGGL(fill_i32_kernel, dim3(1), dim3(256), 0, st, (int32_t*)(d_padded + n_cells), (size_t)1, 0);
    STOCS_HIP_CHECK(exclusive_scan(d_t32, t32, d_padded, d_list_off, (size_t)n_cells + 1, st));
    uint32_t* tail = rb32 + 3;
    STOCS_HIP_CHECK(hipMemcpyAsync(&tail[0], d_list_off + n_cells, 4, hipMemcpyDeviceToHost, st));
    STOCS_HIP_CHECK(hipMemcpyAsync(&tail[1], d_max, 4, hipMemcpyDeviceToHost, st));
    if (prune) STOCS_HIP_CHECK(hipMemcpyAsync(&rb64[1], d_total, 8, hipMemcpyDeviceToHost, st));
    STOCS_HIP_CHECK(hipStreamSynchronize(st));
    const unsigned long long n_kept = prune ? rb64[1] : (unsigned long long)n_inc;
    const size_t n_list = tail[0];
    if (tail[1] > 65535u) { set_error("more than 65535 scene points within epsilon of one grid cell"); return STOCS_ERR_INVALID; }
    if ((rc = c->grid_mem.take(std::max<size_t>((size_t)n_bricks * 512, 1) * sizeof(uint4), (void**)&g.d_cells)) ||
        (rc = c->grid_mem.take(std::max<size_t>(n_list, 8) * sizeof(float4), (void**)&g.d_list)))
        return rc;
    hipLaunchKernelGGL(zero_cells_kernel, dim3(grid_of((size_t)n_bricks * 512)), dim3(256), 0, st, g.d_cells, (size_t)n_bricks * 512);
    {
        const size_t n_flat = (size_t)n[0] * n[1] * n[2];
        if (!dense && div == 1 && c->lcp_flat && n_flat * sizeof(uint4) <= ((size_t)512 << 20)) {
            if ((rc = c->grid_mem.take(n_flat * sizeof(uint4), (void**)&g.d_flat))) return rc;
            hipLaunchKernelGGL(zero_cells_kernel, dim3(grid_of(n_flat)), dim3(256), 0, st, g.d_flat, n_flat);
        }
    }
    hipLaunchKernelGGL(fill_list_kernel, dim3(grid_of(std::max<size_t>(n_list, 8))), dim3(256), 0, st, g.d_list, std::max<size_t>(n_list, 8));
    hipLaunchKernelGGL(cell_words_kernel, dim3((unsigned)((n_cells + 3) / 4)), dim3(256), 0, st, G, div, d_cell_first, d_cell_key, d_cell_brick, d_list_off, n_cells,
                       (uint32_t)n_inc, d_vals_s, c->d_spos, g.d_top, g.d_cells, g.d_flat, (const uint32_t*)d_kept);
    hipLaunchKernelGGL(list_fill_kernel, dim3(grid_of(n_inc)), dim3(256), 0, st, d_cflag, d_cidx, d_cell_first, d_list_off, d_vals_s, n_inc, c->d_spos, g.d_list, (const uint32_t*)d_rank);
    STOCS_HIP_CHECK(hipGetLastError());
    if (prune && div > 1) {
        hipLaunchKernelGGL(cell_nearest_store_kernel, dim3(grid_of(n_cells)), dim3(256), 0, st, d_cell_key, d_cell_brick, n_cells, (const float*)d_near, g.d_cells);
        g.has_nearest = true;
    }
    if (dense) {
        if ((rc = c->grid_mem.take(std::max<size_t>(n_list / 8, 1) * sizeof(float), (void**)&g.d_chunk_r))) return rc;
        hipLaunchKernelGGL(fill_i32_kernel, dim3(grid_of(n_list / 8)), dim3(256), 0, st, (int32_t*)g.d_chunk_r, n_list / 8, 0);
        hipLaunchKernelGGL(chunk_bounds_kernel, dim3(grid_of(n_cells)), dim3(256), 0, st, G, d_cell_first, d_cell_key, d_list_off, n_cells, (uint32_t)n_inc,
                           g.d_list, g.d_chunk_r);
        g.has_nearest = div > 1;
        if (g.has_nearest)
            hipLaunchKernelGGL(cell_nearest_kernel, dim3(grid_of(n_cells)), dim3(256), 0, st, d_cell_key, d_cell_brick, d_list_off, n_cells, g.d_chunk_r, g.d_cells);
        STOCS_HIP_CHECK(hipGetLastError());
    }
    STOCS_HIP_CHECK(hipStreamSynchronize(st));
    g.n_bricks = (int)n_bricks;
    g.n_entries = (int64_t)n_list;
    g.avg_list_len = n_cells ? (double)n_kept / (double)n_cells : 0.0;
    g.avg_dilated_len = n_cells ? (double)n_inc / (double)n_cells : 0.0;
    g.pruned = prune != 0;
    return STOCS_OK;
}

struct CullGeom {
    double o[3], g, cap;
    int n[3], w;
};

__global__ __launch_bounds__(256) void dist_fill_kernel(float* __restrict__ t, size_t n, float v) {
    const size_t i = (size_t)blockIdx.x * blockDim.x + threadIdx.x;
    if (i < n) t[i] = v;
}

__global__ __launch_bounds__(256) void dist_splat_kernel(CullGeom G, float ox, float oy, float oz, float g, float cap, const float4* __restrict__ spos, int nS,
                                                         uint32_t* __restrict__ t) {
    const int i = blockIdx.x * 4 + (threadIdx.x >> 6);
    if (i >= nS) return;
    const int lane = threadIdx.x & 63, xo0 = lane & 15, rsub = lane >> 4;
    const int side = 2 * G.w + 1;
    const float4 p = spos[i];
    const float inv_g = 1.0f / g, cap2 = cap * cap;
    const int ix = (int)floorf((p.x - ox) * inv_g), iy0 = (int)floorf((p.y - oy) * inv_g) - G.w, iz0 = (int)floorf((p.z - oz) * inv_g) - G.w;
    for (int r = rsub; r < side * side; r += 4) {
        const int iz = iz0 + r / side, iy = iy0 + r % side;
        if (iy < 0 || iy >= G.n[1] || iz < 0 || iz >= G.n[2]) continue;
        const float dy = p.y - (oy + ((float)iy + 0.5f) * g), dz = p.z - (oz + ((float)iz + 0.5f) * g);
        const float dyz = dy * dy + dz * dz;
        if (dyz >= cap2) continue;
        const size_t row = ((size_t)iz * G.n[1] + iy) * G.n[0];
        for (int xo = xo0; xo < side; xo += 16) {
            const int cx = ix - G.w + xo;
            if (cx < 0 || cx >= G.n[0]) continue;
            const float dx = p.x - (ox + ((float)cx + 0.5f) * g);
            const float d2 = dx * dx + dyz;
            if (d2 >= cap2) continue;
            const float v = fmaxf(sqrtf(d2) * (1.0f - 2.0e-6f) - 1.0e-6f, 0.0f);
            const uint32_t u = __float_as_uint(v);
            if (u < __hip_atomic_load(&t[row + cx], __ATOMIC_RELAXED, __HIP_MEMORY_SCOPE_AGENT)) atomicMin(&t[row + cx], u);
        }
    }
}

int prepare_cull_field(stocs_ctx* c) {
    SceneGrid& g = c->grid;
    g.d_dist = NULL; g.dist_ready = false;
    if (c->nS <= 0 || c->nM < 64 || !c->d_mpatch) return STOCS_OK;
    const double eps = (double)c->prm.distance_threshold;
    if (!(eps > 0)) return STOCS_OK;
    double cg = eps;
    const double cap = std::min((double)c->patch_r_ref, 8.0 * eps) + eps + cg;
    double ext[3];
    int64_t cells = 0;
    for (;;) {
        cells = 1;
        for (int k = 0; k < 3; ++k) { ext[k] = (g.bb_mx[k] - g.bb_mn[k]) + 2.0 * (cap + cg); cells *= (int64_t)floor(ext[k] / cg) + 1; }
        if (cells <= ((int64_t)16 << 20)) break;
        cg *= 1.25;
    }
    g.cg_g = (float)cg; g.cg_inv_g = (float)(1.0 / (double)g.cg_g);
    g.cg_cap = (float)cap;
    g.cg_ox = (float)(g.bb_mn[0] - cap - cg); g.cg_oy = (float)(g.bb_mn[1] - cap - cg); g.cg_oz = (float)(g.bb_mn[2] - cap - cg);
// ... 27 lines not shown
```

### model_matching_amd/csrc/lcp.hip

```cpp
#include <stdlib.h>
#include <string.h>

#include <cstring>


#include <algorithm>
#include <utility>

#include "kdtree.h"
#include "prims.h"
#include "stocs_ctx.h"

namespace stocs {

struct LcpArgs {
    const float4* mpos;
    const float4* mnrm;
    const int32_t* mperm;
    int M;
    const int32_t* top;
    const uint4* cells;
    const uint4* flat;
    const float4* list;
    const float4* snrmw;
    const int32_t* cand_trial;
    size_t snrmw_stride;
    const float* chunk_r;
    float ox, oy, oz, inv_h, inv_h4, h;
    int nx, ny, nz, nbx, nby;
    float sq_eps, dot_lo, eps;
    float bound_margin;
    int has_nearest;
    const int32_t* order;
    int xcd_blocks;
    unsigned long long* best;
    uint32_t id_offset;
    const float4* patch;
    const float4* sub;
    const float* dist;
    float gox, goy, goz, g, inv_g, cap;
    int gnx, gny, gnz;
#ifdef STOCS_TOOLS_BUILD
    int ablate;
#endif
};
#ifdef STOCS_TOOLS_BUILD
#define STOCS_ABLATE(a, bit) (((a).ablate & (bit)) != 0)
#else
#define STOCS_ABLATE(a, bit) false
#endif

__device__ __forceinline__ int lcp_candidate(const LcpArgs& a, int n, int w, int wpb = 4) {
    int blk = blockIdx.x;
    if (a.xcd_blocks == 1) {
        const int nb = gridDim.x, per = nb >> 3, rem = nb & 7, xcd = blk & 7;
        blk = xcd * per + (xcd < rem ? xcd : rem) + (blk >> 3);
    } else if (a.xcd_blocks > 1) {
        const int C = a.xcd_blocks, nb = gridDim.x, full = (nb / (8 * C)) * (8 * C);
        if (blk < full) {
            const int xcd = blk & 7, j = blk >> 3;
            blk = ((j / C) * 8 + xcd) * C + (j % C);
        }
    }
    const int slot = __builtin_amdgcn_readfirstlane(blk * wpb + w);
    if (slot >= n) return -1;
    return a.order ? __builtin_amdgcn_readfirstlane(a.order[slot]) : slot;
}


__device__ __forceinline__ const float4* lcp_weights_of(const LcpArgs& a, int cand) {
    if (!a.cand_trial) return a.snrmw;
    const int t = __builtin_amdgcn_readfirstlane(a.cand_trial[cand < 0 ? 0 : cand]);
    return (const float4*)((const char*)a.snrmw + (size_t)t * a.snrmw_stride);
}

#define DPP_QUAD_XOR1 0xB1
#define DPP_QUAD_XOR2 0x4E
#define DPP_HALF_MIRROR 0x141

__device__ __forceinline__ void lcp_add(unsigned long long& acc, float w) {
    if (w > 0.0f) acc += (unsigned long long)(w * 4294967296.0f);
}
__device__ __forceinline__ unsigned long long lcp_wave_sum(unsigned long long acc) {
    for (int off = 32; off > 0; off >>= 1) acc += __shfl_xor(acc, off, 64);
    return acc;
}
__device__ __forceinline__ float lcp_finish(unsigned long long total, int M) {
    return (float)((double)total * (1.0 / 4294967296.0) / (double)M);
}
__device__ __forceinline__ void lcp_store(const LcpArgs& a, float* __restrict__ out, int cand, unsigned long long total) {
    const float s = lcp_finish(total, a.M);
    out[cand] = s;
    if (a.best && s > 0.0f)
        atomicMax(a.best, best_key(s, a.id_offset + (uint32_t)cand));
}

template <bool IDX>
__device__ __forceinline__ void take_if_better(float d, int ei, float& gd, int& gi) {
    if (IDX) { if (d <= gd) { gd = d; gi = ei; } }
    else { if (d < gd || (d == gd && ei > gi)) { gd = d; gi = ei; } }
}

template <bool DETAIL, bool IDX = true>
__global__ __launch_bounds__(256) void lcp_kernel(LcpArgs a, const float* __restrict__ T16, float* __restrict__ out,
                                                  int n, int32_t* __restrict__ hit_out, uint8_t* __restrict__ cnt_out) {
    const int lane = threadIdx.x & 63;
    const int cand = lcp_candidate(a, n, threadIdx.x >> 6);
    if (cand < 0) return;
    const float* T = T16 + (size_t)cand * 16;
    const float4* __restrict__ snrmw = lcp_weights_of(a, cand);
    const float t0 = T[0], t1 = T[1], t2 = T[2], t4 = T[4], t5 = T[5], t6 = T[6], t8 = T[8], t9 = T[9], t10 = T[10],
                t12 = T[12], t13 = T[13], t14 = T[14];
    unsigned long long acc = 0ull;
    for (int i = lane; i < a.M; i += 64) {
        const float4 p = a.mpos[i];
        const float qx = ((t0 * p.x + t4 * p.y) + t8 * p.z) + t12;
        const float qy = ((t1 * p.x + t5 * p.y) + t9 * p.z) + t13;
        const float qz = ((t2 * p.x + t6 * p.y) + t10 * p.z) + t14;
        const float fx = floorf((qx - a.ox) * a.inv_h);
        const float fy = floorf((qy - a.oy) * a.inv_h);
        const float fz = floorf((qz - a.oz) * a.inv_h);
        int best = -1;
        if (fx >= 0.0f && fy >= 0.0f && fz >= 0.0f && fx < (float)a.nx && fy < (float)a.ny && fz < (float)a.nz) {
            const int cx = (int)fx, cy = (int)fy, cz = (int)fz;
            const int brick = a.top[((cz >> 3) * a.nby + (cy >> 3)) * a.nbx + (cx >> 3)];
            if (brick >= 0) {
                const uint4 cw = a.cells[(size_t)brick * 512 + (((cz & 7) << 6) | ((cy & 7) << 3) | (cx & 7))];
                float bd = a.sq_eps;
                for (uint32_t k = 0; k < cw.y; ++k) {
                    const float4 s = a.list[cw.x + k];
                    const float dx = qx - s.x, dy = qy - s.y, dz = qz - s.z;
                    const float d = dx * dx + (dy * dy + dz * dz);
                    take_if_better<IDX>(d, __float_as_int(s.w), bd, best);
                }
            }
        }
        bool counted = false;
        if (best >= 0) {
            const float4 nm = a.mnrm[i];
            const float nx = t0 * nm.x + (t4 * nm.y + t8 * nm.z);
            const float ny = t1 * nm.x + (t5 * nm.y + t9 * nm.z);
            const float nz = t2 * nm.x + (t6 * nm.y + t10 * nm.z);
            const float4 sn = snrmw[best];
            const float d = sn.x * nx + (sn.y * ny + sn.z * nz);
            counted = (d >= a.dot_lo) && (d <= 1.0f);
            if (counted) lcp_add(acc, sn.w);
        }
        if (DETAIL) {
            const int orig = a.mperm[i];
            hit_out[(size_t)cand * a.M + orig] = best;
            cnt_out[(size_t)cand * a.M + orig] = counted ? 1 : 0;
        }
    }
    acc = lcp_wave_sum(acc);
    if (lane == 0) lcp_store(a, out, cand, acc);
}

template <int CTRL>
__device__ __forceinline__ float dpp_f32(float v) {
    return __int_as_float(__builtin_amdgcn_update_dpp(0, __float_as_int(v), CTRL, 0xF, 0xF, true));
}
template <int CTRL>
__device__ __forceinline__ int dpp_i32(int v) {
    return __builtin_amdgcn_update_dpp(0, v, CTRL, 0xF, 0xF, true);
}

template <int GL>
__device__ __forceinline__ float group_min_nonneg(float v) {
    uint32_t u = __float_as_uint(v);
    if (GL >= 2) u = min(u, (uint32_t)__builtin_amdgcn_update_dpp((int)u, (int)u, DPP_QUAD_XOR1, 0xF, 0xF, false));
    if (GL >= 4) u = min(u, (uint32_t)__builtin_amdgcn_update_dpp((int)u, (int)u, DPP_QUAD_XOR2, 0xF, 0xF, false));
    if (GL == 8) u = min(u, (uint32_t)__builtin_amdgcn_update_dpp((int)u, (int)u, DPP_HALF_MIRROR, 0xF, 0xF, false));
    return __uint_as_float(u);
}

constexpr int lcp_waves_per_block(bool detail, bool split) { return (split || detail) ? 4 : 1; }

template <bool DETAIL, bool SPLIT>
__global__ __launch_bounds__(64 * lcp_waves_per_block(DETAIL, SPLIT)) void lcp_coop_kernel(LcpArgs a, const float* __restrict__ T16, float* __restrict__ out,
                                                       int n, int32_t* __restrict__ hit_out, uint8_t* __restrict__ cnt_out) {
    static_assert(!(DETAIL && SPLIT), "the detail form is not split");
    constexpr int WPB = lcp_waves_per_block(DETAIL, SPLIT);
    constexpr int UNR = 2;
    __shared__ float4 qt[WPB][64];
    __shared__ uint32_t qn[WPB][64];
    __shared__ uint32_t hl[WPB][64];
    __shared__ float rd[WPB][64];
    __shared__ int ri[WPB][64];
    __shared__ float qd[WPB][64];
    __shared__ unsigned long long part[WPB];
    const int lane = threadIdx.x & 63;
    const int sub = lane & 7, grp = lane >> 3;
    const int w = threadIdx.x >> 6;
    const int cand = SPLIT ? lcp_candidate(a, n, 0, 1) : lcp_candidate(a, n, w, WPB);
    if (cand < 0) return;
    const int first = SPLIT ? 64 * w : 0, stride = SPLIT ? 64 * WPB : 64;
    const float4* __restrict__ snrmw = lcp_weights_of(a, cand);
    const float* T = T16 + (size_t)cand * 16;
    const float t0 = T[0], t1 = T[1], t2 = T[2], t4 = T[4], t5 = T[5], t6 = T[6], t8 = T[8], t9 = T[9], t10 = T[10],
                t12 = T[12], t13 = T[13], t14 = T[14];
    unsigned long long acc = 0ull;
    for (int base = first; base < a.M; base += stride) {
        const int i = base + lane;
        float qx = 0.f, qy = 0.f, qz = 0.f, qcd = 0.f;
        uint32_t off = 0, cnt = 0;
        if (i < a.M) {
            const float4 p = a.mpos[i];
            qx = ((t0 * p.x + t4 * p.y) + t8 * p.z) + t12;
            qy = ((t1 * p.x + t5 * p.y) + t9 * p.z) + t13;
            qz = ((t2 * p.x + t6 * p.y) + t10 * p.z) + t14;
            const float ux = (qx - a.ox) * a.inv_h, uy = (qy - a.oy) * a.inv_h, uz = (qz - a.oz) * a.inv_h;
            const float fx = floorf(ux), fy = floorf(uy), fz = floorf(uz);
            if (fx >= 0.0f && fy >= 0.0f && fz >= 0.0f && fx < (float)a.nx && fy < (float)a.ny && fz < (float)a.nz) {
                const int cx = (int)fx, cy = (int)fy, cz = (int)fz;
                const int brick = STOCS_ABLATE(a, 1) ? -1 : a.top[((cz >> 3) * a.nby + (cy >> 3)) * a.nbx + (cx >> 3)];
                if (brick >= 0) {
                    uint4 cw = make_uint4(0u, 0u, 0u, 0u);
                    if (!STOCS_ABLATE(a, 128)) cw = a.cells[(size_t)brick * 512 + (((cz & 7) << 6) | ((cy & 7) << 3) | (cx & 7))];
                    const int sb = ((int)((uz - fz) * 4.0f) << 4) | ((int)((uy - fy) * 4.0f) << 2) | (int)((ux - fx) * 4.0f);
                    const uint32_t mw = a.has_nearest ? 0xFFFFFFFFu : (sb < 32 ? cw.z : cw.w);
                    off = cw.x; cnt = ((mw >> (sb & 31)) & 1u) ? cw.y : 0u;
                    if (STOCS_ABLATE(a, 2)) cnt = cw.x == 0xFFFFFFF1u ? 1u : 0u;
                    const float ex = qx - (a.ox + ((float)cx + 0.5f) * a.h), ey = qy - (a.oy + ((float)cy + 0.5f) * a.h),
                                ez = qz - (a.oz + ((float)cz + 0.5f) * a.h);
                    qcd = sqrtf(ex * ex + (ey * ey + ez * ez));
                }
            }
        }
        const bool hit = cnt != 0;
        const unsigned long long mask = __ballot(hit);
        int best = -1;
        if (mask) {
            const int nh = __popcll(mask);
            if (hit) {
                const int rank = __popcll(mask & ((1ull << lane) - 1ull));
                hl[w][rank] = (uint32_t)lane;
                qt[w][lane] = make_float4(qx, qy, qz, __int_as_float((int)off));
                qn[w][lane] = cnt;
                qd[w][lane] = qcd;
            }
            __builtin_amdgcn_wave_barrier();
            for (int s = 0; s < nh; s += 8) {
                const int slot = s + grp;
                const bool gact = slot < nh;
                const uint32_t L = gact ? hl[w][slot] : 0u;
                const float4 qq = qt[w][L];
                const uint32_t c = gact ? qn[w][L] : 0u;
                const float4* lp = a.list + (uint32_t)__float_as_int(qq.w) + sub;
                float gd = a.sq_eps;
                int gi = -1;
                const float qcg = qd[w][L];
                const uint32_t chunk0 = (uint32_t)__float_as_int(qq.w) >> 3;
                uint32_t nchunks = (c + 7u) >> 3;
                float gb = a.sq_eps;
                if (STOCS_ABLATE(a, 4)) nchunks = min(nchunks, (uint32_t)UNR);
                for (uint32_t j = 0; __any(j < nchunks); j += UNR) {
                    if (j < nchunks && j > 0 && (STOCS_ABLATE(a, 256) ? 0.0f : a.chunk_r[chunk0 + j]) - qcg > sqrtf(gb) + a.bound_margin) nchunks = 0;
                    float4 e[UNR];
#pragma unroll
                    for (int u = 0; u < UNR; ++u) {
                        e[u] = make_float4(1e30f, 1e30f, 1e30f, __int_as_float(-1));
                        if (j + u < nchunks) e[u] = lp[(j + u) << 3];
                    }
#pragma unroll
                    for (int u = 0; u < UNR; ++u) {
                        const float dx = qq.x - e[u].x, dy = qq.y - e[u].y, dz = qq.z - e[u].z;
                        const float d = dx * dx + (dy * dy + dz * dz);
                        const int ei = __float_as_int(e[u].w);
                        if (d < gd || (d == gd && ei > gi)) { gd = d; gi = ei; }
                    }
                    gb = fminf(gd, dpp_f32<DPP_QUAD_XOR1>(gd));
                    gb = fminf(gb, dpp_f32<DPP_QUAD_XOR2>(gb));
                    gb = fminf(gb, dpp_f32<DPP_HALF_MIRROR>(gb));
                }
                float dm = fminf(gd, dpp_f32<DPP_QUAD_XOR1>(gd));
                dm = fminf(dm, dpp_f32<DPP_QUAD_XOR2>(dm));
                dm = fminf(dm, dpp_f32<DPP_HALF_MIRROR>(dm));
                int im = (gd == dm) ? gi : -1;
                im = max(im, dpp_i32<DPP_QUAD_XOR1>(im));
                im = max(im, dpp_i32<DPP_QUAD_XOR2>(im));
                im = max(im, dpp_i32<DPP_HALF_MIRROR>(im));
                if (gact && sub == 0) { rd[w][L] = dm; ri[w][L] = im; }
            }
            __builtin_amdgcn_wave_barrier();
            if (hit) best = ri[w][lane];
            __builtin_amdgcn_wave_barrier();
        }
        bool counted = false;
        if (best >= 0 && STOCS_ABLATE(a, 8)) lcp_add(acc, 0.5f);
        else if (best >= 0) {
            const float4 nm = a.mnrm[i];
            const float nx = t0 * nm.x + (t4 * nm.y + t8 * nm.z);
            const float ny = t1 * nm.x + (t5 * nm.y + t9 * nm.z);
            const float nz = t2 * nm.x + (t6 * nm.y + t10 * nm.z);
            const float4 sn = snrmw[best];
            const float d = sn.x * nx + (sn.y * ny + sn.z * nz);
            counted = (d >= a.dot_lo) && (d <= 1.0f);
            if (counted) lcp_add(acc, sn.w);
        }
        if (DETAIL && i < a.M) {
            const int orig = a.mperm[i];
            hit_out[(size_t)cand * a.M + orig] = best;
            cnt_out[(size_t)cand * a.M + orig] = counted ? 1 : 0;
        }
    }
    acc = lcp_wave_sum(acc);
    if (SPLIT) {
        if (lane == 0) part[w] = acc;
        __syncthreads();
        if (threadIdx.x == 0) {
            unsigned long long total = 0;
#pragma unroll
            for (int k = 0; k < WPB; ++k) total += part[k];
            lcp_store(a, out, cand, total);
        }
    } else if (lane == 0) lcp_store(a, out, cand, acc);
}

__device__ __forceinline__ float lcp_linear_norm_bound(float t0, float t1, float t2, float t4, float t5, float t6, float t8, float t9, float t10) {
    const float g00 = t0 * t0 + (t1 * t1 + t2 * t2), g11 = t4 * t4 + (t5 * t5 + t6 * t6), g22 = t8 * t8 + (t9 * t9 + t10 * t10);
    const float g01 = fabsf(t0 * t4 + (t1 * t5 + t2 * t6)), g02 = fabsf(t0 * t8 + (t1 * t9 + t2 * t10)), g12 = fabsf(t4 * t8 + (t5 * t9 + t6 * t10));
    const float rho = fmaxf(g00 + (g01 + g02), fmaxf(g11 + (g01 + g12), g22 + (g02 + g12)));
    return sqrtf(rho) * 1.00001f;
}
__device__ __forceinline__ bool lcp_patch_dead(const LcpArgs& a, const float4 sp, float sn, float t0, float t1, float t2, float t4, float t5, float t6,
                                               float t8, float t9, float t10, float t12, float t13, float t14) {
    const float cx = ((t0 * sp.x + t4 * sp.y) + t8 * sp.z) + t12;
    const float cy = ((t1 * sp.x + t5 * sp.y) + t9 * sp.z) + t13;
    const float cz = ((t2 * sp.x + t6 * sp.y) + t10 * sp.z) + t14;
    const float mag = fabsf(cx) + (fabsf(cy) + fabsf(cz));
    if (!(mag < 1.0e18f)) return false;
    const float need = (sn * sp.w + a.eps * 1.002f) + (4.0e-6f + 4.0e-6f * mag);
    const float ux = (cx - a.gox) * a.inv_g, uy = (cy - a.goy) * a.inv_g, uz = (cz - a.goz) * a.inv_g;
    const float fx = floorf(ux), fy = floorf(uy), fz = floorf(uz);
    if (fx >= 1.0f && fy >= 1.0f && fz >= 1.0f && fx < (float)(a.gnx - 1) && fy < (float)(a.gny - 1) && fz < (float)(a.gnz - 1)) {
        const float v = a.dist[((uint32_t)(int)fz * (uint32_t)a.gny + (uint32_t)(int)fy) * (uint32_t)a.gnx + (uint32_t)(int)fx];
        const float ex = cx - (a.gox + (fx + 0.5f) * a.g), ey = cy - (a.goy + (fy + 0.5f) * a.g), ez = cz - (a.goz + (fz + 0.5f) * a.g);
        return v - sqrtf(ex * ex + (ey * ey + ez * ez)) > need;
    }
    return a.cap > need;
}

constexpr int LCP_SHARED_LIVE = 512;

constexpr bool lcp_queue_form_legal(bool detail, bool dense, bool split, bool flat, bool near, int cu, bool shared) {
    return (cu == 16 || cu == 64) && (!shared || (split && cu == 16)) && (detail ? (!split && !flat && !(dense && near)) : (!dense || (split && !flat && !near)));
}

template <bool DETAIL, bool DENSE, bool SPLIT, bool FLAT, bool NEAR, int CU, bool SHARED>
__global__ __launch_bounds__(64 * lcp_waves_per_block(DETAIL, SPLIT), 8) void lcp_coopq_kernel(LcpArgs a, const float* __restrict__ T16, float* __restrict__ out,
                                                        int n, int32_t* __restrict__ hit_out, uint8_t* __restrict__ cnt_out) {
    static_assert(lcp_queue_form_legal(DETAIL, DENSE, SPLIT, FLAT, NEAR, CU, SHARED), "not one of the forms in the table above");
    constexpr int WPB = lcp_waves_per_block(DETAIL, SPLIT);
    constexpr bool IDX = !DENSE;
    constexpr bool EARLY = DENSE;
    constexpr int GL = 4, EPL = 8 / GL, NG = 64 / GL;
    constexpr int FIRST = DENSE ? 1 : 2, E0 = EPL * FIRST;
    constexpr bool NOSENT = !DENSE;
    constexpr int UNR = 1;
    constexpr int PIPE = 1;
    static_assert(!EARLY || (FIRST == 1 && !NOSENT), "early exit decides line by line");
    __shared__ float4 qt[WPB][128];
    __shared__ float qcd[EARLY ? WPB : 1][EARLY ? 128 : 1];
    __shared__ uint32_t qn[WPB][128];
    __shared__ uint32_t qs[WPB][128];
    __shared__ int ri[WPB][128];
    __shared__ uint8_t ord[WPB][64];
    __shared__ unsigned long long part[WPB];
    const int lane = threadIdx.x & 63;
    const int w = threadIdx.x >> 6;
    const int cand = SPLIT ? lcp_candidate(a, n, 0, 1) : lcp_candidate(a, n, w, WPB);
    if (cand < 0) return;
    const float4* __restrict__ snrmw = lcp_weights_of(a, cand);
    const float* T = T16 + (size_t)cand * 16;
    const float t0 = T[0], t1 = T[1], t2 = T[2], t4 = T[4], t5 = T[5], t6 = T[6], t8 = T[8], t9 = T[9], t10 = T[10],
                t12 = T[12], t13 = T[13], t14 = T[14];
    unsigned long long acc = 0ull;
    int head = 0, tail = 0;

    auto process = [&](int nq) {
        {
            uint32_t cls = 4;
            if (lane < nq) {
                const uint32_t nch = (qn[w][(head + lane) & 127] + 7u) >> 3;
                cls = nch <= (uint32_t)FIRST ? 1u : (nch <= (uint32_t)(FIRST + UNR) ? 2u : 3u);
            }
            const unsigned long long below = (1ull << lane) - 1ull;
            const unsigned long long m1 = __ballot(cls == 1u), m2 = __ballot(cls == 2u), m3 = __ballot(cls == 3u);
            const int n1 = __popcll(m1), n2 = __popcll(m2);
            const int pos = cls == 1u ? __popcll(m1 & below) : (cls == 2u ? n1 + __popcll(m2 & below) : n1 + n2 + __popcll(m3 & below));
            if (lane < nq) ord[w][pos] = (uint8_t)lane;
            __builtin_amdgcn_wave_barrier();
        }
        for (int s0 = 0; s0 < nq; s0 += NG * PIPE) {
            const int sub = lane & (GL - 1), grp = lane / GL;
            float4 e0[PIPE][E0];
            bool wide[PIPE];
            int idxs[PIPE];
            uint32_t cs[PIPE];
#pragma unroll
            for (int u = 0; u < PIPE; ++u) {
                const int slot = s0 + NG * u + grp;
                const bool gact = slot < nq;
                idxs[u] = (head + (int)ord[w][gact ? slot : 0]) & 127;
                cs[u] = gact ? qn[w][idxs[u]] : 0u;
                wide[u] = true;
                if (!NOSENT) {
#pragma unroll
                    for (int e = 0; e < E0; ++e) e0[u][e] = make_float4(1e30f, 1e30f, 1e30f, __int_as_float(-1));
                }
                if (STOCS_ABLATE(a, 4)) {
                    if (cs[u]) { const float4 qq0 = qt[w][idxs[u]]; e0[u][0] = make_float4(qq0.x, qq0.y, qq0.z, __int_as_float(0)); }
                    cs[u] = cs[u] ? 1u : 0u;
                }
                else if (NOSENT) {
                    const float4* l0 = a.list + (cs[u] ? (uint32_t)__float_as_int(qt[w][idxs[u]].w) : 0u) + sub;
                    const uint32_t last = cs[u] ? ((cs[u] - 1u) & ~7u) : 0u;
#pragma unroll
                    for (int e = 0; e < EPL; ++e) e0[u][e] = l0[GL * e];
                    wide[u] = FIRST > 1 && __any(cs[u] > 8u);
                    if (wide[u]) {
#pragma unroll
                        for (int e = EPL; e < E0; ++e) e0[u][e] = l0[min((uint32_t)(8 * (e / EPL)), last) + GL * (e % EPL)];
                    }
                }
                else if (cs[u]) {
                    const float4* l0 = a.list + (uint32_t)__float_as_int(qt[w][idxs[u]].w) + sub;
#pragma unroll
                    for (int e = 0; e < E0; ++e) e0[u][e] = l0[GL * e];
                }
            }
#pragma unroll
            for (int u = 0; u < PIPE; ++u) {
                const float4 qq = qt[w][idxs[u]];
                const uint32_t c = cs[u];
// ... 5 lines not shown
                for (int e = 0; e < EPL; ++e) {
                    const float dx = qq.x - e0[u][e].x, dy = qq.y - e0[u][e].y, dz = qq.z - e0[u][e].z;
                    const float d = dx * dx + (dy * dy + dz * dz);
                    take_if_better<IDX>(d, __float_as_int(e0[u][e].w), gd, gi);
                }
                if (FIRST > 1 && wide[u]) {
#pragma unroll
                    for (int e = EPL; e < E0; ++e) {
                        const float dx = qq.x - e0[u][e].x, dy = qq.y - e0[u][e].y, dz = qq.z - e0[u][e].z;
                        const float d = dx * dx + (dy * dy + dz * dz);
                        take_if_better<IDX>(d, __float_as_int(e0[u][e].w), gd, gi);
                    }
                }
                if (EARLY) {
                    const float qcg = qcd[w][idxs[u]];
                    const uint32_t chunk0 = (uint32_t)__float_as_int(qq.w) >> 3;
                    uint32_t cc = c;
                    for (uint32_t k = 8; __any(k < cc); k += 8 * UNR) {
                        if (k < cc && a.chunk_r[chunk0 + (k >> 3)] - qcg > sqrtf(group_min_nonneg<GL>(gd)) + a.bound_margin) cc = 0;
                        float4 e[EPL];
                        if (k < cc) {
#pragma unroll
                            for (int x = 0; x < EPL; ++x) e[x] = lp[k + GL * x];
                        } else {
#pragma unroll
                            for (int x = 0; x < EPL; ++x) e[x] = make_float4(1e30f, 1e30f, 1e30f, __int_as_float(-1));
                        }
#pragma unroll
                        for (int x = 0; x < EPL; ++x) {
                            const float dx = qq.x - e[x].x, dy = qq.y - e[x].y, dz = qq.z - e[x].z;
                            const float d = dx * dx + (dy * dy + dz * dz);
                            take_if_better<IDX>(d, __float_as_int(e[x].w), gd, gi);
                        }
                    }
                } else {
                    for (uint32_t k = 8 * FIRST; __any(k < c); k += 8 * UNR) {
                        const uint32_t kk = min(k, last_line);
                        float4 e[EPL];
#pragma unroll
                        for (int x = 0; x < EPL; ++x) e[x] = lp[kk + GL * x];
#pragma unroll
                        for (int x = 0; x < EPL; ++x) {
                            const float dx = qq.x - e[x].x, dy = qq.y - e[x].y, dz = qq.z - e[x].z;
                            const float d = dx * dx + (dy * dy + dz * dz);
                            take_if_better<IDX>(d, __float_as_int(e[x].w), gd, gi);
                        }
                    }
                }
                const float dm = group_min_nonneg<GL>(gd);
                int im = (gd == dm) ? gi : -1;
                im = max(im, dpp_i32<DPP_QUAD_XOR1>(im));
                im = max(im, dpp_i32<DPP_QUAD_XOR2>(im));
                if (c && sub == 0) ri[w][idxs[u]] = im;
            }
        }
        __builtin_amdgcn_wave_barrier();
        if (lane < nq) {
            const int idx = (head + lane) & 127;
            const int best = ri[w][idx];
            const uint32_t slot_i = qs[w][idx];
            bool counted = false;
            if (best >= 0 && STOCS_ABLATE(a, 8)) { lcp_add(acc, 0.5f); }
            else if (best >= 0) {
                const float4 nm = STOCS_ABLATE(a, 16) ? make_float4(0.f, 0.f, 1.f, 0.f) : a.mnrm[slot_i];
                const float nx = t0 * nm.x + (t4 * nm.y + t8 * nm.z);
                const float ny = t1 * nm.x + (t5 * nm.y + t9 * nm.z);
                const float nz = t2 * nm.x + (t6 * nm.y + t10 * nm.z);
                const float4 sn = STOCS_ABLATE(a, 32) ? make_float4(nx, ny, nz, 0.5f) : snrmw[best];
                const float d = sn.x * nx + (sn.y * ny + sn.z * nz);
                counted = (d >= a.dot_lo) && (d <= 1.0f);
                if (counted) lcp_add(acc, sn.w);
            }
            if (DETAIL) {
                const int orig = a.mperm[slot_i];
                hit_out[(size_t)cand * a.M + orig] = best;
                cnt_out[(size_t)cand * a.M + orig] = counted ? 1 : 0;
            }
        }
        __builtin_amdgcn_wave_barrier();
    };

    auto step = [&](const int i, const float4 p) {
        float qx = 0.f, qy = 0.f, qz = 0.f, qcentre = 0.f, nearest = 0.f;
        uint32_t off = 0, cnt = 0;
        if (!DETAIL || i < a.M) {
            qx = ((t0 * p.x + t4 * p.y) + t8 * p.z) + t12;
            qy = ((t1 * p.x + t5 * p.y) + t9 * p.z) + t13;
            qz = ((t2 * p.x + t6 * p.y) + t10 * p.z) + t14;
            const int c4x = __float2int_rd((qx - a.ox) * a.inv_h4), c4y = __float2int_rd((qy - a.oy) * a.inv_h4),
                      c4z = __float2int_rd((qz - a.oz) * a.inv_h4);
            const int cx = c4x >> 2, cy = c4y >> 2, cz = c4z >> 2;
            if ((unsigned)cx < (unsigned)a.nx && (unsigned)cy < (unsigned)a.ny && (unsigned)cz < (unsigned)a.nz) {
                const int sb = ((c4z & 3) << 4) | ((c4y & 3) << 2) | (c4x & 3);
                if (FLAT) {
                    uint4 cw = make_uint4(0u, 0u, 0u, 0u);
                    if (!STOCS_ABLATE(a, 1))
                        cw = a.flat[(uint32_t)((cz * a.ny + cy) * a.nx + cx)];
                    const uint32_t mw = sb < 32 ? cw.z : cw.w;
                    off = cw.x; cnt = ((mw >> (sb & 31)) & 1u) ? cw.y : 0u;
                    if (STOCS_ABLATE(a, 2)) cnt = cw.x == 0xFFFFFFF1u ? 1u : 0u;
                } else {
                    const int brick = a.top[((cz >> 3) * a.nby + (cy >> 3)) * a.nbx + (cx >> 3)];
                    if (brick >= 0) {
                        const uint4 cw = a.cells[(uint32_t)brick * 512u + (uint32_t)(((cz & 7) << 6) | ((cy & 7) << 3) | (cx & 7))];
                        if ((EARLY || NEAR) && a.has_nearest) { off = cw.x; cnt = cw.y; nearest = __uint_as_float(cw.z); }
                        else { const uint32_t mw = a.has_nearest ? 0xFFFFFFFFu : (sb < 32 ? cw.z : cw.w); off = cw.x; cnt = ((mw >> (sb & 31)) & 1u) ? cw.y : 0u; }
                    }
                }
            }
            if ((EARLY || (NEAR && a.has_nearest)) && cnt) {
                const float ex = qx - (a.ox + ((float)cx + 0.5f) * a.h), ey = qy - (a.oy + ((float)cy + 0.5f) * a.h), ez = qz - (a.oz + ((float)cz + 0.5f) * a.h);
                qcentre = sqrtf(ex * ex + (ey * ey + ez * ez));
                if (a.has_nearest && nearest - qcentre > a.eps + a.bound_margin) cnt = 0;
            }
            if (DETAIL && cnt == 0) {
                const int orig = a.mperm[i];
                hit_out[(size_t)cand * a.M + orig] = -1;
                cnt_out[(size_t)cand * a.M + orig] = 0;
            }
        }
        const bool hit = cnt != 0;
        const unsigned long long mask = __ballot(hit);
        if (mask) {
            if (hit) {
                const int rank = __popcll(mask & ((1ull << lane) - 1ull));
                const int sl = (tail + rank) & 127;
                qt[w][sl] = make_float4(qx, qy, qz, __int_as_float((int)off));
                qn[w][sl] = cnt;
                qs[w][sl] = (uint32_t)i;
                if (EARLY) qcd[w][sl] = qcentre;
            }
            tail += __popcll(mask);
            __builtin_amdgcn_wave_barrier();
            if (tail - head >= 64) {
                process(64);
                head += 64;
            }
        }
    };
    if (CU == 16) {
    __shared__ uint16_t live_q[WPB][128];
    const int nsteps = (a.M + 63) >> 6;
    if (SHARED) {
    __shared__ int live_n;
    uint16_t* const live_all = &live_q[0][0];
    static_assert(!SHARED || WPB * 128 == LCP_SHARED_LIVE, "the shared list is the memory of the per-wave rings");
    if (threadIdx.x == 0) live_n = 0;
    const int nsubs = (a.M + 15) >> 4;
    const float snorm = a.patch ? lcp_linear_norm_bound(t0, t1, t2, t4, t5, t6, t8, t9, t10) : 0.0f;
    unsigned long long lm[2];
#pragma unroll
    for (int j = 0; j < 2; ++j) {
        const int q = ((w + 4 * j) << 6) + lane;
        bool live = q < nsubs;
        if (a.patch && live && !STOCS_ABLATE(a, 64))
            live = !lcp_patch_dead(a, a.sub[q], snorm, t0, t1, t2, t4, t5, t6, t8, t9, t10, t12, t13, t14);
        lm[j] = __ballot(live);
    }
    __syncthreads();
#pragma unroll
    for (int j = 0; j < 2; ++j) {
        if (lm[j]) {
            int base = 0;
            if (lane == 0) base = atomicAdd(&live_n, __popcll(lm[j]));
            base = __builtin_amdgcn_readfirstlane(base);
            if ((lm[j] >> lane) & 1ull)
                live_all[base + __popcll(lm[j] & ((1ull << lane) - 1ull))] = (uint16_t)(((w + 4 * j) << 6) + lane);
        }
    }
    __syncthreads();
    const int nlive = __builtin_amdgcn_readfirstlane(live_n);
    const int nst = (nlive + 3) >> 2;
    const int mine = __builtin_amdgcn_readfirstlane((nst + 3 - w) >> 2);
    const int e0 = 4 * w + (lane >> 4);
    auto slot = [&](int k) { const int e = e0 + 16 * k; return e < nlive ? ((int)live_all[e] << 4) + (lane & 15) : (nsteps << 6) + lane; };
    if (mine > 0) {
        int i = slot(0);
        float4 p_next = a.mpos[i];
        for (int k = 0; k < mine; ++k) {
            const int ic = i;
            const float4 p = p_next;
            i = k + 1 < mine ? slot(k + 1) : ic;
            p_next = a.mpos[i];
            step(ic, p);
        }
    }
    } else {
    const int wfirst = SPLIT ? w : 0, nw = SPLIT ? WPB : 1;
    const int nsub = __builtin_amdgcn_readfirstlane(4 * ((nsteps - wfirst + nw - 1) / nw));
    const float snorm = a.patch ? lcp_linear_norm_bound(t0, t1, t2, t4, t5, t6, t8, t9, t10) : 0.0f;
    int qh = 0, qtl = 0;
    for (int s0 = 0;; s0 += 64) {
        {
            const int kl = s0 + lane, q = 4 * (wfirst + (kl >> 2) * nw) + (kl & 3);
            const bool in = kl < nsub && (q << 4) < a.M;
            bool live = in;
// ... 40 lines not shown
    }
    }
    } else {
    const int nsteps = (a.M + 63) >> 6;
    const int wfirst = SPLIT ? w : 0, nw = SPLIT ? WPB : 1;
    const int nk = (nsteps - wfirst + nw - 1) / nw;
    const float snorm = a.patch ? lcp_linear_norm_bound(t0, t1, t2, t4, t5, t6, t8, t9, t10) : 0.0f;
    for (int k0 = 0; k0 < nk; k0 += 64) {
        const int kk = k0 + lane;
        bool live = kk < nk;
        if (a.patch && live && !STOCS_ABLATE(a, 64))
            live = !lcp_patch_dead(a, a.patch[wfirst + kk * nw], snorm, t0, t1, t2, t4, t5, t6, t8, t9, t10, t12, t13, t14);
        unsigned long long todo = __ballot(live);
        if (DETAIL && a.patch) {
            unsigned long long dead = __ballot(kk < nk && !live);
            while (dead) {
                const int j = __builtin_ctzll(dead);
                dead &= dead - 1ull;
                const int i = ((wfirst + (k0 + j) * nw) << 6) + lane;
                if (i < a.M) {
                    const int orig = a.mperm[i];
                    hit_out[(size_t)cand * a.M + orig] = -1;
                    cnt_out[(size_t)cand * a.M + orig] = 0;
                }
            }
        }
        if (!todo) continue;
        int j = __builtin_ctzll(todo);
        float4 p_next = a.mpos[((wfirst + (k0 + j) * nw) << 6) + lane];
        for (;;) {
            const int i = ((wfirst + (k0 + j) * nw) << 6) + lane;
            const float4 p = p_next;
            todo &= todo - 1ull;
            j = todo ? __builtin_ctzll(todo) : j;
            p_next = a.mpos[((wfirst + (k0 + j) * nw) << 6) + lane];
            step(i, p);
            if (!todo) break;
        }
    }
    }
    if (tail - head > 0) process(tail - head);
    acc = lcp_wave_sum(acc);
    if (SPLIT) {
        if (lane == 0) part[w] = acc;
        __syncthreads();
        if (threadIdx.x == 0) {
            unsigned long long total = 0;
#pragma unroll
            for (int k = 0; k < WPB; ++k) total += part[k];
            lcp_store(a, out, cand, total);
        }
    } else if (lane == 0) lcp_store(a, out, cand, acc);
}

template <bool DETAIL>
__global__ __launch_bounds__(256) void lcp_exact_kernel(LcpArgs a, const float* __restrict__ T16, float* __restrict__ out, int n,
                                                        int32_t* __restrict__ hit_out, uint8_t* __restrict__ cnt_out,
                                                        const KdNodeP* __restrict__ kd_nodes, const float4* __restrict__ kd_pts,
                                                        unsigned long long* __restrict__ ties) {
    const int lane = threadIdx.x & 63;
    const int cand = lcp_candidate(a, n, threadIdx.x >> 6);
    if (cand < 0) return;
    const float* T = T16 + (size_t)cand * 16;
    const float4* __restrict__ snrmw = lcp_weights_of(a, cand);
    const float t0 = T[0], t1 = T[1], t2 = T[2], t4 = T[4], t5 = T[5], t6 = T[6], t8 = T[8], t9 = T[9], t10 = T[10],
                t12 = T[12], t13 = T[13], t14 = T[14];
    unsigned long long acc = 0ull, n_flag = 0ull, n_changed = 0ull;
    for (int i = lane; i < a.M; i += 64) {
        const float4 p = a.mpos[i];
        const float qx = ((t0 * p.x + t4 * p.y) + t8 * p.z) + t12;
        const float qy = ((t1 * p.x + t5 * p.y) + t9 * p.z) + t13;
        const float qz = ((t2 * p.x + t6 * p.y) + t10 * p.z) + t14;
        const float fx = floorf((qx - a.ox) * a.inv_h);
        const float fy = floorf((qy - a.oy) * a.inv_h);
        const float fz = floorf((qz - a.oz) * a.inv_h);
        int best = -1;
        bool tie = false;
        float bd = a.sq_eps;
        if (fx >= 0.0f && fy >= 0.0f && fz >= 0.0f && fx < (float)a.nx && fy < (float)a.ny && fz < (float)a.nz) {
            const int cx = (int)fx, cy = (int)fy, cz = (int)fz;
            const int brick = a.top[((cz >> 3) * a.nby + (cy >> 3)) * a.nbx + (cx >> 3)];
            if (brick >= 0) {
                const uint4 cw = a.cells[(size_t)brick * 512 + (((cz & 7) << 6) | ((cy & 7) << 3) | (cx & 7))];
                for (uint32_t k = 0; k < cw.y; ++k) {
                    const float4 s = a.list[cw.x + k];
                    const float dx = qx - s.x, dy = qy - s.y, dz = qz - s.z;
                    const float d = dx * dx + (dy * dy + dz * dz);
                    const int ei = __float_as_int(s.w);
                    if (d < bd) { bd = d; best = ei; tie = false; }
                    else if (d == bd) { if (best >= 0) { tie = true; best = max(best, ei); } else best = ei; }
                }
            }
        }
        if (tie || (best >= 0 && bd == a.sq_eps)) {
            const int kb = kd_query_closest(kd_nodes, kd_pts, qx, qy, qz, a.sq_eps);
            n_flag++;
            if (kb != best) n_changed++;
            best = kb;
        }
        bool counted = false;
        if (best >= 0) {
            const float4 nm = a.mnrm[i];
            const float nx = t0 * nm.x + (t4 * nm.y + t8 * nm.z);
            const float ny = t1 * nm.x + (t5 * nm.y + t9 * nm.z);
            const float nz = t2 * nm.x + (t6 * nm.y + t10 * nm.z);
            const float4 sn = snrmw[best];
            const float d = sn.x * nx + (sn.y * ny + sn.z * nz);
            counted = (d >= a.dot_lo) && (d <= 1.0f);
            if (counted) lcp_add(acc, sn.w);
        }
        if (DETAIL) {
            const int orig = a.mperm[i];
            hit_out[(size_t)cand * a.M + orig] = best;
            cnt_out[(size_t)cand * a.M + orig] = counted ? 1 : 0;
        }
    }
    acc = lcp_wave_sum(acc);
    n_flag = lcp_wave_sum(n_flag);
    n_changed = lcp_wave_sum(n_changed);
    if (lane == 0) {
        lcp_store(a, out, cand, acc);
        if (n_flag) atomicAdd(&ties[0], n_flag);
        if (n_changed) atomicAdd(&ties[1], n_changed);
    }
}

__global__ __launch_bounds__(256) void best_kernel(const float* __restrict__ lcp, int n, uint32_t id_offset, unsigned long long* __restrict__ best) {
    unsigned long long k = 0;
    for (int i = blockIdx.x * blockDim.x + threadIdx.x; i < n; i += gridDim.x * blockDim.x) {
        const float s = lcp[i];
        if (s > 0.0f) { const unsigned long long key = best_key(s, id_offset + (uint32_t)i); k = key > k ? key : k; }
    }
    k = wave_max_key(k);
    if ((threadIdx.x & 63) == 0 && k) atomicMax(best, k);
}

__global__ __launch_bounds__(1024) void best_single_kernel(const float* __restrict__ lcp, int n, uint32_t id_offset, unsigned long long* __restrict__ best) {
    __shared__ unsigned long long sh[16];
    unsigned long long k = 0;
    for (int i = threadIdx.x; i < n; i += 1024) {
        const float s = lcp[i];
        if (s > 0.0f) {
            const unsigned long long key = ((unsigned long long)__float_as_uint(s) << 32) | (unsigned long long)(0xFFFFFFFFu - (id_offset + (uint32_t)i));
            k = key > k ? key : k;
        }
    }
    for (int off = 32; off > 0; off >>= 1) {
        const unsigned long long o = __shfl_xor(k, off, 64);
        k = o > k ? o : k;
    }
    if ((threadIdx.x & 63) == 0) sh[threadIdx.x >> 6] = k;
    __syncthreads();
    if (threadIdx.x == 0) {
        for (int w = 1; w < 16; ++w) k = sh[w] > k ? sh[w] : k;
        *best = k;
    }
}

__device__ __forceinline__ uint32_t spread10(uint32_t x) {
    x &= 0x3ff; x = (x | (x << 16)) & 0x30000ff; x = (x | (x << 8)) & 0x300f00f; x = (x | (x << 4)) & 0x30c30c3; x = (x | (x << 2)) & 0x9249249;
    return x;
}
__global__ __launch_bounds__(256) void order_keys_kernel(const float* __restrict__ T16, int n, float ox, float oy, float oz, float sx, float sy, float sz,
                                                         uint32_t* __restrict__ keys, int32_t* __restrict__ vals, unsigned long long* __restrict__ best) {
    const int i = blockIdx.x * blockDim.x + threadIdx.x;
    if (i == 0 && best) *best = 0ull;
    if (i >= n) return;
    const float* T = T16 + (size_t)i * 16;
    const float qx = fminf(fmaxf((T[12] - ox) * sx, 0.0f), 255.0f), qy = fminf(fmaxf((T[13] - oy) * sy, 0.0f), 255.0f),
                qz = fminf(fmaxf((T[14] - oz) * sz, 0.0f), 255.0f);
    keys[i] = (spread10((uint32_t)qz) << 2) | (spread10((uint32_t)qy) << 1) | spread10((uint32_t)qx);
    vals[i] = i;
}

enum LcpKernel { LCP_PLAIN, LCP_STEP, LCP_QUEUE, LCP_EXACT };
struct LcpForm {
    LcpKernel kernel;
    bool detail;
    bool dense;
    bool split;
    bool flat, near;
    int cu;
    bool shared;
};

static bool lcp_variant_selectable(int v) { return v == 99 || v == 0 || v == 24 || v == 31 || v == 39; }

static LcpForm choose_lcp_form(const stocs_ctx* c, const LcpArgs& a, bool detail) {
    LcpForm f = {LCP_QUEUE, detail, false, false, false, false, 64, false};
    if (c->exact_ties) { f.kernel = LCP_EXACT; return f; }
    f.dense = c->grid.d_chunk_r != NULL;
    const int variant = c->lcp_variant >= 0 ? c->lcp_variant : 99;
    if (variant == 0) f.kernel = (detail && f.dense) ? LCP_STEP : LCP_PLAIN;
    else if (variant == 31 && f.dense) f.kernel = LCP_STEP;
    const bool split = c->lcp_split && a.M >= 512;
    if (f.kernel == LCP_STEP) f.split = !detail && split;
    if (f.kernel == LCP_QUEUE) {
        f.split = !detail && (f.dense || split);
        f.flat = !detail && !f.dense && c->lcp_flat && a.flat;
        f.near = !f.dense && a.has_nearest;
        f.cu = (a.patch && c->lcp_cull_unit == 16) ? 16 : 64;
        f.shared = f.split && f.cu == 16 && a.M <= 16 * LCP_SHARED_LIVE;
    }
    return f;
}

typedef void (*LcpScanFn)(LcpArgs, const float*, float*, int, int32_t*, uint8_t*);

template <int I>
static LcpScanFn lcp_queue_fn() {
    constexpr bool DETAIL = (I & 1) != 0, DENSE = (I & 2) != 0, SPLIT = (I & 4) != 0, FLAT = (I & 8) != 0, NEAR = (I & 16) != 0;
    constexpr int CU = (I & 32) ? 16 : 64;
    constexpr bool SHARED = (I & 64) != 0;
    if constexpr (lcp_queue_form_legal(DETAIL, DENSE, SPLIT, FLAT, NEAR, CU, SHARED)) return lcp_coopq_kernel<DETAIL, DENSE, SPLIT, FLAT, NEAR, CU, SHARED>;
    else return NULL;
}
template <int... I>
static LcpScanFn lcp_queue_fn(const LcpForm& f, std::integer_sequence<int, I...>) {
    static const LcpScanFn table[] = {lcp_queue_fn<I>()...};
    return table[(f.detail ? 1 : 0) | (f.dense ? 2 : 0) | (f.split ? 4 : 0) | (f.flat ? 8 : 0) | (f.near ? 16 : 0) | (f.cu == 16 ? 32 : 0) | (f.shared ? 64 : 0)];
}

static int launch_lcp_form(stocs_ctx* c, const LcpForm& f, const LcpArgs& a, const float* d_T16, int n, float* d_lcp, int32_t* d_hit, uint8_t* d_counted) {
    const bool cooperative = f.kernel == LCP_STEP || f.kernel == LCP_QUEUE;
    const bool one_wave = cooperative && !f.detail && !f.split;
    const dim3 grid((unsigned)(f.split || one_wave ? n : (n + 3) / 4)), block(one_wave ? 64 : 256);
    if (f.kernel == LCP_EXACT) {
        if (f.detail) hipLaunchKernelGGL(lcp_exact_kernel<true>, grid, block, 0, c->stream, a, d_T16, d_lcp, n, d_hit, d_counted, c->d_kd_nodes, c->d_kd_pts, c->d_ties);
        else hipLaunchKernelGGL(lcp_exact_kernel<false>, grid, block, 0, c->stream, a, d_T16, d_lcp, n, d_hit, d_counted, c->d_kd_nodes, c->d_kd_pts, c->d_ties);
    } else {
        LcpScanFn fn = NULL;
        if (f.kernel == LCP_QUEUE) fn = lcp_queue_fn(f, std::make_integer_sequence<int, 128>());
        else if (f.kernel == LCP_STEP) fn = f.detail ? lcp_coop_kernel<true, false> : (f.split ? lcp_coop_kernel<false, true> : lcp_coop_kernel<false, false>);
        else if (!f.detail) fn = f.dense ? lcp_kernel<false, false> : lcp_kernel<false, true>;
        else if (!f.dense) fn = lcp_kernel<true, true>;
        if (!fn) { set_error("launch_lcp: no kernel for this form (kernel %d, detail %d, dense %d, split %d, flat %d, near %d, cu %d, shared %d)", (int)f.kernel, (int)f.detail, (int)f.dense, (int)f.split, (int)f.flat, (int)f.near, f.cu, (int)f.shared); return STOCS_ERR_STATE; }
        hipLaunchKernelGGL(fn, grid, block, 0, c->stream, a, d_T16, d_lcp, n, d_hit, d_counted);
    }
    STOCS_HIP_CHECK(hipGetLastError());
    return STOCS_OK;
}

int launch_lcp(stocs_ctx* c, const float* d_T16, int n, float* d_lcp, int32_t* d_hit, uint8_t* d_counted, unsigned long long* d_best8, uint32_t id_offset) {
    if (n <= 0) { if (d_best8) STOCS_HIP_CHECK(hipMemsetAsync(d_best8, 0, 8, c->stream)); return STOCS_OK; }
    bool best_zeroed = false;
    LcpArgs a;
    a.best = d_best8; a.id_offset = id_offset;
#ifdef STOCS_TOOLS_BUILD
    a.ablate = getenv("STOCS_LCP_ABLATE") ? atoi(getenv("STOCS_LCP_ABLATE")) : 0;
#endif
    a.mpos = c->d_mpos_s; a.mnrm = c->d_mnrm_s; a.mperm = c->d_mperm; a.M = c->nM;
    a.top = c->grid.d_top; a.cells = c->grid.d_cells; a.flat = c->grid.d_flat; a.list = c->grid.d_list; a.snrmw = c->snrmw_override ? c->snrmw_override : c->d_snrmw;
    a.cand_trial = c->lcp_cand_trial; a.snrmw_stride = c->lcp_cand_trial ? c->snrmw_stride : 0;
    a.ox = c->grid.ox; a.oy = c->grid.oy; a.oz = c->grid.oz; a.inv_h = c->grid.inv_h; a.inv_h4 = c->grid.inv_h * 4.0f; a.h = c->grid.h; a.chunk_r = c->grid.d_chunk_r;
    a.nx = c->grid.nx; a.ny = c->grid.ny; a.nz = c->grid.nz; a.nbx = c->grid.nbx; a.nby = c->grid.nby;
    a.sq_eps = c->prm.distance_threshold * c->prm.distance_threshold;
    a.dot_lo = c->thr.lcp_dot_lo;
    a.eps = c->prm.distance_threshold;
    a.has_nearest = c->grid.has_nearest ? 1 : 0;
    {
        double mag = 0.0;
        for (int k = 0; k < 3; ++k) mag = std::max(mag, std::max(fabs(c->grid.bb_mn[k]), fabs(c->grid.bb_mx[k])));
        a.bound_margin = (float)(4.0e-4 * (double)c->prm.distance_threshold + 4.0e-6 * mag);
    }
    a.patch = NULL; a.sub = NULL; a.dist = NULL;
    a.gox = a.goy = a.goz = 0.f; a.g = a.inv_g = a.cap = 0.f; a.gnx = a.gny = a.gnz = 0;
    c->scene_scored++;
    c->scene_work += (double)n * (double)c->nM;
    if (c->exact_ties) {
        int rc = ensure_kdtree(c);
        if (rc) return rc;
        if (!c->ties_started) { STOCS_HIP_CHECK(hipMemsetAsync(c->d_ties, 0, 16, c->stream)); c->ties_started = true; }
        a.order = NULL; a.xcd_blocks = 0;
        if (d_best8 && !(d_best8 == c->d_best && c->best_is_zero)) STOCS_HIP_CHECK(hipMemsetAsync(d_best8, 0, 8, c->stream));
        if (d_best8 == c->d_best) c->best_is_zero = false;
        return launch_lcp_form(c, choose_lcp_form(c, a, d_hit != NULL), a, d_T16, n, d_lcp, d_hit, d_counted);
    }
    if (c->lcp_cull && c->grid.d_dist && c->d_mpatch && (c->grid.dist_ready || c->lcp_cull >= 2 || c->scene_work >= c->lcp_cull_after)) {
        int rc = fill_cull_field(c);
        if (rc) return rc;
        if (c->cull_pending) { STOCS_HIP_CHECK(hipStreamWaitEvent(c->stream, c->ev_cull, 0)); c->cull_pending = false; }
        a.patch = c->d_mpatch; a.sub = c->d_msub; a.dist = c->grid.d_dist;
        a.gox = c->grid.cg_ox; a.goy = c->grid.cg_oy; a.goz = c->grid.cg_oz; a.g = c->grid.cg_g; a.inv_g = c->grid.cg_inv_g; a.cap = c->grid.cg_cap;
        a.gnx = c->grid.cg_nx; a.gny = c->grid.cg_ny; a.gnz = c->grid.cg_nz;
    }
    a.order = NULL; a.xcd_blocks = 0;
    const bool lists_spill = (double)c->grid.n_entries * 16.0 >= 12.0e6;
    if (!d_hit && n >= 1024 && (double)n * (double)c->nM >= 1.5e8 && c->lcp_order && (lists_spill || c->lcp_order >= 2)) {
        const size_t kb = al256((size_t)n * 4);
        size_t tb = 0;
        STOCS_HIP_CHECK(sort_pairs(NULL, tb, (const uint32_t*)NULL, (uint32_t*)NULL, (const uint32_t*)NULL, (uint32_t*)NULL, (size_t)n, 0, 24, c->stream));
        const size_t need = 4 * kb + tb;
        { const int rc = c->order.grow(c->stream, need); if (rc) return rc; }
        char* p = c->order.p;
        uint32_t* keys = (uint32_t*)p; uint32_t* keys_s = (uint32_t*)(p + kb);
        int32_t* vals = (int32_t*)(p + 2 * kb); int32_t* order = (int32_t*)(p + 3 * kb);
        void* tmp = p + 4 * kb;
        const float sx = 256.0f / ((float)c->grid.nx * c->grid.h), sy = 256.0f / ((float)c->grid.ny * c->grid.h), sz = 256.0f / ((float)c->grid.nz * c->grid.h);
        hipLaunchKernelGGL(order_keys_kernel, dim3((unsigned)((n + 255) / 256)), dim3(256), 0, c->stream, d_T16, n, c->grid.ox, c->grid.oy, c->grid.oz, sx, sy, sz,
                           keys, vals, d_best8);
        best_zeroed = true;
        STOCS_HIP_CHECK(sort_pairs(tmp, tb, keys, keys_s, (const uint32_t*)vals, (uint32_t*)order, (size_t)n, 0, 24, c->stream));
        a.order = order;
        const bool lists_huge = (double)c->grid.n_entries * 16.0 >= 512.0e6;
        a.xcd_blocks = c->lcp_order >= 2 ? (c->lcp_order == 2 ? 1 : c->lcp_order) : (lists_huge ? 128 : 0);
    }
    if (d_best8 && d_best8 == c->d_best && c->best_is_zero) best_zeroed = true;
    if (d_best8 == c->d_best) c->best_is_zero = false;
    if (d_best8 && !best_zeroed) STOCS_HIP_CHECK(hipMemsetAsync(d_best8, 0, 8, c->stream));
    return launch_lcp_form(c, choose_lcp_form(c, a, d_hit != NULL), a, d_T16, n, d_lcp, d_hit, d_counted);
}

static int enqueue_best(stocs_ctx* c, const float* d_lcp, int n, uint32_t id_offset, unsigned long long* d_key8) {
    if (n <= (1 << 18)) {
        hipLaunchKernelGGL(best_single_kernel, dim3(1), dim3(1024), 0, c->stream, d_lcp, n, id_offset, d_key8);
    } else {
        STOCS_HIP_CHECK(hipMemsetAsync(d_key8, 0, 8, c->stream));
        const int blocks = std::min((n + 255) / 256, 1024);
        hipLaunchKernelGGL(best_kernel, dim3(blocks), dim3(256), 0, c->stream, d_lcp, n, id_offset, d_key8);
// ... 25 lines not shown
    return launch_lcp(c, (const float*)d_T16, n, (float*)d_lcp, NULL, NULL, NULL, 0);
}

int stocs_score_transforms(stocs_ctx* c, const float* T_host, int n, float* lcp_host) {
    if (!c || n < 0 || (n && (!T_host || !lcp_host))) return STOCS_ERR_INVALID;
    DeviceGuard dev_guard(c->device);
    begin_scoring_call(c);
    if (n == 0) return STOCS_OK;
    const size_t tb = (size_t)n * 64, lb = (size_t)n * 4;
    int rc = ensure_scratch(c, tb + lb + 256);
    if (rc) return rc;
    float* dT = (float*)c->d_scratch;
    float* dL = (float*)((char*)c->d_scratch + al256(tb));
    STOCS_HIP_CHECK(hipMemcpyAsync(dT, T_host, tb, hipMemcpyHostToDevice, c->stream));
    rc = launch_lcp(c, dT, n, dL, NULL, NULL, NULL, 0);
    if (rc) return rc;
    STOCS_HIP_CHECK(hipMemcpyAsync(lcp_host, dL, lb, hipMemcpyDeviceToHost, c->stream));
    STOCS_HIP_CHECK(hipStreamSynchronize(c->stream));
    return STOCS_OK;
}

int stocs_lcp_detail(stocs_ctx* c, const float* T_host, int32_t* hit, uint8_t* counted) {
    if (!c || !T_host || !hit || !counted) return STOCS_ERR_INVALID;
    DeviceGuard dev_guard(c->device);
    begin_scoring_call(c);
    const size_t M = (size_t)c->nM;
    int rc = ensure_scratch(c, 256 + 256 + M * 4 + 256 + M);
    if (rc) return rc;
    char* base = (char*)c->d_scratch;
    float* dT = (float*)base;
    float* dL = (float*)(base + 256);
    int32_t* dH = (int32_t*)(base + 512);
    uint8_t* dC = (uint8_t*)(base + 512 + al256(M * 4));
    STOCS_HIP_CHECK(hipMemcpyAsync(dT, T_host, 64, hipMemcpyHostToDevice, c->stream));
    rc = launch_lcp(c, dT, 1, dL, dH, dC, NULL, 0);
    if (rc) return rc;
    STOCS_HIP_CHECK(hipMemcpyAsync(hit, dH, M * 4, hipMemcpyDeviceToHost, c->stream));
    STOCS_HIP_CHECK(hipMemcpyAsync(counted, dC, M, hipMemcpyDeviceToHost, c->stream));
    STOCS_HIP_CHECK(hipStreamSynchronize(c->stream));
    return STOCS_OK;
}

__global__ __launch_bounds__(256) void hit_count_kernel(const int32_t* __restrict__ hit, const uint8_t* __restrict__ counted, size_t n, unsigned long long* __restrict__ out2) {
    unsigned long long h = 0, k = 0;
    for (size_t i = (size_t)blockIdx.x * blockDim.x + threadIdx.x; i < n; i += (size_t)gridDim.x * blockDim.x) { h += hit[i] >= 0 ? 1u : 0u; k += counted[i] ? 1u : 0u; }
    for (int off = 32; off > 0; off >>= 1) { h += __shfl_xor(h, off, 64); k += __shfl_xor(k, off, 64); }
    if ((threadIdx.x & 63) == 0) { if (h) atomicAdd(&out2[0], h); if (k) atomicAdd(&out2[1], k); }
}

int stocs_lcp_hit_count(stocs_ctx* c, const void* d_T16, int n, int64_t* hits, int64_t* counted) {
    if (!c || n < 0 || (n && !d_T16) || !hits) return STOCS_ERR_INVALID;
    DeviceGuard dev_guard(c->device);
    begin_scoring_call(c);
    *hits = 0;
    if (counted) *counted = 0;
    if (n == 0 || c->nM == 0) return STOCS_OK;
    const size_t M = (size_t)c->nM;
    const int chunk = (int)std::max<size_t>(1, std::min<size_t>((size_t)n, ((size_t)256 << 20) / (5 * M)));
    const size_t hb = al256((size_t)chunk * M * 4), cb = al256((size_t)chunk * M), lb = al256((size_t)chunk * 4);
    int rc = ensure_scratch(c, 256 + lb + hb + cb);
    if (rc) return rc;
    char* base = (char*)c->d_scratch;
    unsigned long long* d_out = (unsigned long long*)base;
    float* dL = (float*)(base + 256);
    int32_t* dH = (int32_t*)(base + 256 + lb);
    uint8_t* dC = (uint8_t*)(base + 256 + lb + hb);
    STOCS_HIP_CHECK(hipMemsetAsync(d_out, 0, 16, c->stream));
    for (int i0 = 0; i0 < n; i0 += chunk) {
        const int m = std::min(chunk, n - i0);
        rc = launch_lcp(c, (const float*)d_T16 + (size_t)i0 * 16, m, dL, dH, dC, NULL, 0);
        if (rc) return rc;
        hipLaunchKernelGGL(hit_count_kernel, dim3(1024), dim3(256), 0, c->stream, (const int32_t*)dH, (const uint8_t*)dC, (size_t)m * M, d_out);
        STOCS_HIP_CHECK(hipGetLastError());
    }
    if ((rc = ensure_pinned(c, PIN_VAR))) return rc;
    unsigned long long* pin = (unsigned long long*)((char*)c->h_pin + PIN_BEST);
    STOCS_HIP_CHECK(hipMemcpyAsync(pin, d_out, 16, hipMemcpyDeviceToHost, c->stream));
    STOCS_HIP_CHECK(hipStreamSynchronize(c->stream));
    *hits = (int64_t)pin[0];
    if (counted) *counted = (int64_t)pin[1];
    return STOCS_OK;
}

int stocs_best_device(stocs_ctx* c, const void* d_lcp, int n, uint32_t id_offset, uint64_t* key) {
    if (!c || !key || n < 0 || (n && !d_lcp)) return STOCS_ERR_INVALID;
    DeviceGuard dev_guard(c->device);
    *key = 0;
    if (n == 0) return STOCS_OK;
    if (!c->d_best) STOCS_HIP_CHECK(dev_malloc((void**)&c->d_best, 8));
    c->best_is_zero = false;
    int rc = enqueue_best(c, (const float*)d_lcp, n, id_offset, c->d_best);
    if (rc) return rc;
    return read_best_key(c, key);
}

int stocs_best_device_async(stocs_ctx* c, const void* d_lcp, int n, uint32_t id_offset, void* d_key8) {
    if (!c || !d_key8 || n < 0 || (n && !d_lcp)) return STOCS_ERR_INVALID;
    DeviceGuard dev_guard(c->device);
    if (n == 0) { STOCS_HIP_CHECK(hipMemsetAsync(d_key8, 0, 8, c->stream)); return STOCS_OK; }
    return enqueue_best(c, (const float*)d_lcp, n, id_offset, (unsigned long long*)d_key8);
}

int stocs_score_best_device_async(stocs_ctx* c, const void* d_T16, int n, void* d_lcp, uint32_t id_offset, void* d_key8) {
    if (!c || !d_key8 || n < 0 || (n && (!d_T16 || !d_lcp))) return STOCS_ERR_INVALID;
    DeviceGuard dev_guard(c->device);
    begin_scoring_call(c);
    return launch_lcp(c, (const float*)d_T16, n, (float*)d_lcp, NULL, NULL, (unsigned long long*)d_key8, id_offset);
}

int stocs_score_best_device(stocs_ctx* c, const void* d_T16, int n, void* d_lcp, uint32_t id_offset, uint64_t* key) {
    if (!c || !key) return STOCS_ERR_INVALID;
    DeviceGuard dev_guard(c->device);
    if (!c->d_best) STOCS_HIP_CHECK(dev_malloc((void**)&c->d_best, 8));
    int rc = stocs_score_best_device_async(c, d_T16, n, d_lcp, id_offset, c->d_best);
    if (rc) return rc;
    return read_best_key(c, key);
}

int stocs_set_option(stocs_ctx* c, const char* key, int value) {
    if (!c || !key) return STOCS_ERR_INVALID;
    if (!strcmp(key, "lcp_variant")) {
        if (!lcp_variant_selectable(value)) { set_error("stocs_set_option: lcp_variant %d is not part of this build (99 automatic, 0, 24, 31, 39)", value); return STOCS_ERR_INVALID; }
        c->lcp_variant = value;
        return STOCS_OK;
    }
    if (!strcmp(key, "lcp_order") && value >= 0 && value <= 4096) { c->lcp_order = value; return STOCS_OK; }
    if (!strcmp(key, "device_clock") && (value == 0 || value == 1)) { c->device_clock = value; return STOCS_OK; }
    if (!strcmp(key, "lcp_flat") && (value == 0 || value == 1)) { c->lcp_flat = value; return STOCS_OK; }
    if (!strcmp(key, "exact_ties")) {
        if (value != 0 && value != 1) { set_error("stocs_set_option: exact_ties takes 0 or 1, not %d", value); return STOCS_ERR_INVALID; }
        c->exact_ties = value;
        return STOCS_OK;
    }
    if (!strcmp(key, "lcp_split") && (value == 0 || value == 1)) { c->lcp_split = value; return STOCS_OK; }
    if (!strcmp(key, "lcp_cull") && value >= 0 && value <= 2) { c->lcp_cull = value; return STOCS_OK; }
    if (!strcmp(key, "lcp_cull_unit") && (value == 16 || value == 64)) { c->lcp_cull_unit = value; return STOCS_OK; }
    if (!strcmp(key, "lcp_cull_after") && value >= 0) { c->lcp_cull_after = (double)value * 1.0e6; return STOCS_OK; }
    if (!strcmp(key, "lcp_group") && value == 4) return STOCS_OK;
    set_error("stocs_set_option: unknown option or value");
    return STOCS_ERR_INVALID;
}

int stocs_get_cull_state(stocs_ctx* c, float* patches4, int32_t* perm, int* n_patches, float* geom8, float* dist, int64_t dist_cap, int64_t* n_dist) {
    if (!c || !n_patches || !n_dist) return STOCS_ERR_INVALID;
    DeviceGuard dev_guard(c->device);
    const int np = c->d_mpatch ? (c->nM + 63) / 64 : 0;
    *n_patches = np;
    const SceneGrid& g = c->grid;
    const int64_t nd = g.d_dist ? (int64_t)g.cg_nx * g.cg_ny * g.cg_nz : 0;
    *n_dist = nd;
    if (dist && nd) {
        if (dist_cap < nd) return STOCS_ERR_CAPACITY;
        int rc = fill_cull_field(c);
        if (rc) return rc;
        if (c->cull_pending) { STOCS_HIP_CHECK(hipStreamWaitEvent(c->stream, c->ev_cull, 0)); c->cull_pending = false; }
    }
    if (patches4 && np) STOCS_HIP_CHECK(hipMemcpyAsync(patches4, c->d_mpatch, (size_t)np * 16, hipMemcpyDeviceToHost, c->stream));
    if (perm) for (int i = 0; i < c->nM; ++i) perm[i] = c->h_mperm[i];
    if (geom8) {
        geom8[0] = g.cg_ox; geom8[1] = g.cg_oy; geom8[2] = g.cg_oz; geom8[3] = g.cg_g; geom8[4] = g.cg_cap;
        geom8[5] = (float)g.cg_nx; geom8[6] = (float)g.cg_ny; geom8[7] = (float)g.cg_nz;
    }
    hipError_t e = hipSuccess;
    if (dist && nd) e = hipMemcpyAsync(dist, g.d_dist, (size_t)nd * 4, hipMemcpyDeviceToHost, c->stream);
    STOCS_HIP_CHECK(hipStreamSynchronize(c->stream));
    STOCS_HIP_CHECK(e);
    return STOCS_OK;
}

int stocs_time_score_kernel(stocs_ctx* c, const void* d_T16, int n, void* d_lcp, int reps, float* avg_ms) {
    if (!c || !avg_ms || reps <= 0 || n <= 0) return STOCS_ERR_INVALID;
    DeviceGuard dev_guard(c->device);
    begin_scoring_call(c);
    STOCS_HIP_CHECK(hipEventRecord(c->ev0, c->stream));
    for (int r = 0; r < reps; ++r) {
        int rc = launch_lcp(c, (const float*)d_T16, n, (float*)d_lcp, NULL, NULL, NULL, 0);
        if (rc) return rc;
    }
    STOCS_HIP_CHECK(hipEventRecord(c->ev1, c->stream));
    STOCS_HIP_CHECK(hipEventSynchronize(c->ev1));
    float ms = 0;
    STOCS_HIP_CHECK(hipEventElapsedTime(&ms, c->ev0, c->ev1));
    *avg_ms = ms / (float)reps;
    return STOCS_OK;
}

}
```

### model_matching_amd/csrc/stocs_ctx.h

```cpp
#ifndef STOCS_CTX_H
#define STOCS_CTX_H

#include <hip/hip_runtime.h>
#include <stdint.h>
#include <stdio.h>
#include <time.h>

#include <algorithm>
#include <memory>
#include <string>
#include <utility>
#include <vector>

#include "../../include/stocs_hip.h"
#include "kdtree.h"
#include "stocs_math.h"
#include "stream_audit.h"

namespace stocs {

void set_error(const char* fmt, ...);

#define STOCS_HIP_CHECK(expr)                                                                  \
    do {                                                                                       \
// ... 37 lines not shown
        if (prev != dev) (void)hipSetDevice(dev);
    }
    ~DeviceGuard() { if (prev >= 0 && prev != dev) (void)hipSetDevice(prev); }
    DeviceGuard(const DeviceGuard&) = delete;
    DeviceGuard& operator=(const DeviceGuard&) = delete;
};

inline size_t al256(size_t b) { return (b + 255) & ~(size_t)255; }

struct DevBlock {
    char* p = NULL; size_t bytes = 0;
    int grow(hipStream_t st, size_t need, size_t slack_div = 4) {
        if (bytes >= need) return STOCS_OK;
        if (p) { STOCS_HIP_CHECK(hipStreamSynchronize(st)); (void)hipFree(p); p = NULL; bytes = 0; }
        const size_t want = need + need / slack_div;
        STOCS_HIP_CHECK(dev_malloc(&p, want));
        bytes = want;
        return STOCS_OK;
    }
    void free() { if (p) (void)hipFree(p); p = NULL; bytes = 0; }
};

struct Carve {
    size_t total = 0;
    size_t take(size_t bytes) { const size_t at = total; total += al256(bytes); return at; }
    template <class T> static T* at(void* base, size_t off) { return (T*)((char*)base + off); }
};

struct Slab { char* p; size_t cap, used; };
struct Arena {
    std::vector<Slab> slabs;
    int reset() {
        if (slabs.size() > 1) {
            size_t tot = 0;
            for (size_t i = 0; i < slabs.size(); ++i) { tot += slabs[i].cap; (void)hipFree(slabs[i].p); }
            slabs.clear();
            tot += tot;
            Slab sl = {NULL, tot, 0};
            STOCS_HIP_CHECK(dev_malloc((void**)&sl.p, tot));
            slabs.push_back(sl);
        }
        for (size_t i = 0; i < slabs.size(); ++i) slabs[i].used = 0;
        return STOCS_OK;
    }
    int reserve(size_t bytes, double headroom = 2.0) {
        if (slabs.size() == 1 && slabs[0].cap >= bytes) return STOCS_OK;
        destroy();
        Slab sl = {NULL, (size_t)((double)bytes * headroom), 0};
        const hipError_t e = dev_malloc((void**)&sl.p, sl.cap);
        if (e == hipErrorOutOfMemory) { (void)hipGetLastError(); stocs::set_error("arena of %zu bytes: out of device memory", sl.cap); return STOCS_ERR_NOMEM; }
        STOCS_HIP_CHECK(e);
        slabs.push_back(sl);
        return STOCS_OK;
    }
    int take(size_t bytes, void** out) {
        bytes = al256(std::max<size_t>(bytes, 1));
        for (size_t i = 0; i < slabs.size(); ++i)
            if (slabs[i].cap - slabs[i].used >= bytes) { *out = slabs[i].p + slabs[i].used; slabs[i].used += bytes; return STOCS_OK; }
        Slab sl = {NULL, std::max<size_t>(bytes + bytes / 4, slabs.empty() ? ((size_t)64 << 20) : 2 * slabs.back().cap), 0};
        STOCS_HIP_CHECK(dev_malloc((void**)&sl.p, sl.cap));
        sl.used = bytes;
        slabs.push_back(sl);
        *out = sl.p;
        return STOCS_OK;
    }
    void destroy() { for (size_t i = 0; i < slabs.size(); ++i) (void)hipFree(slabs[i].p); slabs.clear(); }
};

struct SceneGrid {
    float ox, oy, oz, inv_h;
    int nx, ny, nz;
    int nbx, nby, nbz;
    int n_bricks;
    int64_t n_entries;
    double avg_list_len;
    double avg_dilated_len;
    bool pruned;
    int32_t* d_top;
    uint4* d_flat;
    uint4* d_cells;
    float4* d_list;
    float* d_chunk_r;
    float h;
    bool has_nearest;
    float* d_dist;
    bool dist_ready;
    float cg_ox, cg_oy, cg_oz, cg_g, cg_inv_g, cg_cap;
    int cg_nx, cg_ny, cg_nz, cg_w;
    double bb_mn[3], bb_mx[3];
};

struct PpfIndex {
    bool built;
    int tr, rot, NA, nD;
    int64_t n_keys;
    int64_t n_pairs;
    uint32_t* d_bucket_start;
    uint32_t* d_pairs;
    uint32_t* d_exists;
    std::vector<uint32_t> h_bucket_start;
    std::vector<uint32_t> h_exists;
    int64_t n_nonempty_buckets, n_exist_keys;
};

struct BaseRec {
    int ids[4];
    float inv1, inv2;
};

struct BaseOut { int32_t ids[4]; float inv[2]; int32_t valid; int32_t pad; };

struct Candidate {
    float T[16];
    float pose[16];
    float lcp;
    int base_index;
};

struct XformJob { int32_t s[4]; int32_t q[4]; };
struct alignas(16) Pick { int32_t base, rank, dst, sorted; };
STOCS_HD bool base_used_whole(long long nq, int max_per_base) { return nq < max_per_base; }
STOCS_HD long long base_pick_count(long long nq, int max_per_base) { return base_used_whole(nq, max_per_base) ? nq : (long long)max_per_base; }

struct Thresholds {
    float lcp_dot_lo;
    float ang_dot_hi;
    float ang_dot_lo;
};

}

struct stocs_ctx {
    stocs_params prm;
    int device;
    hipStream_t stream;
    hipStream_t own_stream;
    hipStream_t aux_stream;
    hipEvent_t ev0, ev1, ev_fork, ev_join;
    hipEvent_t ev_t[10];
    int nS, nM;
    stocs::Thresholds thr;

    std::vector<stocs::V3> h_spos, h_snrm, h_mpos, h_mnrm, h_mpos_raw, h_munit;
    std::vector<float> h_sprob;
    std::vector<float> h_sprob0;
    std::vector<int32_t> h_spix;
    stocs::V3 centroid_scene, centroid_model, gcenter;
    float ratio;
    std::vector<int32_t> h_mperm;

    char* d_scene_mem; size_t scene_cap;
    float4* d_spos;
    float4* d_snrmw;
    int2* d_spix;
    float4* d_mpos;
    float4* d_mnrm;
    float4* d_munit;
    float4* d_mpos_raw;
    float4* d_mpos_s;
    float4* d_mnrm_s;
    int32_t* d_mperm;
    float4* d_mpatch;
    float4* d_msub;
    float patch_r_ref;
    int lcp_cull;
    int lcp_cull_unit;
    double lcp_cull_after;
    bool prev_scene_warm;
    bool cull_pending;
    hipEvent_t ev_cull;
    int scene_scored;
    double scene_work;

    stocs::SceneGrid grid;
    stocs::Arena grid_mem;
    stocs::Arena grid_ws;
    int grid_div;
    int grid_prune;
    int lcp_variant;
    int device_clock;
    int lcp_split;
    int lcp_flat;
    int lcp_order;
    stocs::DevBlock order;
    int exact_ties;
    bool kd_ready;
    stocs::KdTreeHost kd_host;
    stocs::DevBlock kd;
    const stocs::KdNodeP* d_kd_nodes;
    const float4* d_kd_pts;
    unsigned long long* d_ties;
    bool ties_started;
    stocs::DevBlock cdf; size_t cdf_n; unsigned long long prior_epoch, cdf_epoch;
    stocs::PpfIndex index;

    bool has_edge;
    std::vector<uint8_t> edge_map;
    void* inst;

    std::vector<int32_t> last_segment;

    std::vector<stocs::BaseRec> bases;
    std::vector<uint64_t> base_seed;
    std::vector<int32_t> base_local;
    std::vector<int32_t> trial_first_base;
    std::vector<int32_t> trial_cand_off;
    const float4* snrmw_trial0;
    size_t snrmw_stride;
    const int32_t* lcp_cand_trial;
    const float4* snrmw_override;
    void* trials;
    void* cong;
    std::vector<unsigned long long> quad_off;
    void* refine;
    void* track;
    int quad_id_bits;
    std::vector<stocs::Candidate> cands;
    char* d_cand;
    size_t cand_bytes;
    int n_cands, cand_cap;
    bool cands_stale;
    float best_lcp;
    int best_index;

    unsigned long long* d_best;
    bool best_is_zero;

    void* h_pin;
    size_t pin_bytes;
    stocs::CallTiming timing[5];

    stocs::StreamAudit audit;

    void* d_scratch;
    size_t scratch_bytes;

    void* depth;

    struct { int kernel, threads; size_t lds; int cap, launches, redone; } last_form;

    void* instances;

    void* render;

    void* scene;

    void* pose_error;
};

namespace stocs {
inline void clear_candidates(stocs_ctx* c) { c->cands.clear(); c->n_cands = 0; c->cands_stale = false; }
inline void clear_trial_batch(stocs_ctx* c) {
    if (c->base_seed.empty() && c->trial_first_base.empty()) return;
    c->base_seed.clear(); c->base_local.clear(); c->trial_first_base.clear(); c->trial_cand_off.clear();
    c->snrmw_trial0 = NULL; c->snrmw_stride = 0;
    c->bases.clear(); c->quad_off.clear(); clear_candidates(c);
}
inline float* cand_T(stocs_ctx* c) { return (float*)c->d_cand; }
inline float* cand_P(stocs_ctx* c) { return (float*)c->d_cand + (size_t)c->cand_cap * 16; }
inline float* cand_lcp(stocs_ctx* c) { return (float*)c->d_cand + (size_t)c->cand_cap * 32; }
inline int32_t* cand_base(stocs_ctx* c) { return (int32_t*)((float*)c->d_cand + (size_t)c->cand_cap * 33); }
int ensure_scratch(stocs_ctx* c, size_t bytes);
int ensure_pinned(stocs_ctx* c, size_t bytes);
enum { PIN_CONGRUENT = 0, PIN_TRANSFORMS = 256, PIN_VERIFY = 512, PIN_BEST = 768, PIN_VAR = 1024 };
int pinned_var(stocs_ctx* c, size_t bytes, char** h);
// ... 42 lines not shown
```

### model_matching_amd/estimator.py

```python
from __future__ import annotations

import atexit
import ctypes as C
import math
import weakref

import numpy as np

from . import capi

_LIVE = weakref.WeakSet()


@atexit.register
def _close_all():
    for est in list(_LIVE):
        try:
            est.close()
        except Exception:
            pass


_TRIAL_DTYPE = np.dtype([("n_bases", np.int32), ("n_candidates", np.int32), ("n_quads", np.int64), ("best_lcp", np.float32), ("best_index", np.int32),
                         ("best_pose16", np.float32, (16,))])
# ... 407 lines not shown
        H, W = self._frame_shape("explain_poses")
        lab = np.zeros((H, W), np.int32); st = np.zeros((H, W), np.uint8)
        capi.check(self.L.stocs_explain_poses(self.h, pP, n, C.byref(prm), buf, lab.ctypes.data_as(capi._ip), st.ctypes.data_as(capi._u8p)))
        return np.frombuffer(buf, dtype=_RENDER_DTYPE, count=n).copy(), lab, st

    def scene_footprints(self, poses16, rows, slot_base, n_slots, claim="agree", **render_params):
        P, pP = capi.f32(poses16)
        n = P.size // 16
        if claim not in SCENE_CLAIMS:
            raise ValueError("scene_footprints: claim %r is neither 'agree' nor 'on_mask'" % (claim,))
        prm = self._render_params("scene_footprints", render_params)
        buf = (capi.SceneRecord * max(n, 1))()
        capi.check(self.L.stocs_scene_footprints(self.h, pP, n, int(slot_base), int(n_slots), C.byref(prm), SCENE_CLAIMS[claim], rows, buf))
        return np.frombuffer(buf, dtype=_SCENE_RECORD_DTYPE, count=n).copy()

    def scene_select(self, rows, shape, score, group, rec, group_cap=None, **params):
        sc, psc = capi.f32(score)
        gr, pgr = capi.i32(group)
        rc = np.ascontiguousarray(rec, _SCENE_RECORD_DTYPE)
        n = sc.size
        if gr.size != n or rc.size != n:
            raise ValueError("scene_select: %d scores, %d groups, %d records" % (n, gr.size, rc.size))
        params = dict(params)
        pcap = None
        if group_cap is not None:
            cap, pcap = capi.i32(group_cap)
        n_groups = params.pop("n_groups", None)
        if n_groups is None:
            n_groups = cap.size if group_cap is not None else (int(gr.max()) + 1 if n else 1)
        if group_cap is not None and cap.size != n_groups:
            raise ValueError("scene_select: %d caps for %d groups" % (cap.size, n_groups))
        prm = capi.SceneParams()
        self.L.stocs_default_scene_params(C.byref(prm))
        for k, v in params.items():
            if k not in dict(capi.SceneParams._fields_):
                raise TypeError("scene_select: unknown parameter %r" % k)
            setattr(prm, k, v)
        buf = (capi.SceneResult * max(n, 1))()
        sel = np.zeros(max(n, 1), np.int32); ns = C.c_int(0)
        capi.check(self.L.stocs_scene_select(self.h, rows, n, int(shape[1]), int(shape[0]), psc, pgr, rc.ctypes.data_as(C.POINTER(capi.SceneRecord)), int(n_groups),
                                             pcap, C.byref(prm), buf, sel.ctypes.data_as(capi._ip), C.byref(ns)))
        return np.frombuffer(buf, dtype=_SCENE_RESULT_DTYPE, count=n).copy(), sel[:ns.value].copy()

    def select_instances(self, T16, max_instances=16, min_points=20, min_exclusive_fraction=0.5):
        T, pT = capi.f32(T16)
        n = T.size // 16
        prm = capi.InstanceParams(max_instances, min_points, min_exclusive_fraction)
        buf = (capi.InstanceResult * max(n, 1))()
        sel = np.zeros(max(min(max(int(max_instances), 0), n), 1), np.int32); ns = C.c_int(0)
        capi.check(self.L.stocs_select_instances(self.h, pT, n, C.byref(prm), buf, sel.ctypes.data_as(capi._ip), C.byref(ns)))
        return np.frombuffer(buf, dtype=_INSTANCE_DTYPE, count=n).copy(), sel[:ns.value].copy()

    def select_instances_rows(self, hit, counted, lcp, nS, max_instances=16, min_points=20, min_exclusive_fraction=0.5):
        H, pH = capi.i32(hit)
        K = np.ascontiguousarray(counted, np.uint8)
        l, pl = capi.f32(lcp)
        n = l.size
        if H.shape != K.shape or H.ndim != 2 or H.shape[0] != n:
            raise ValueError("hit %s and counted %s must both be (n, nM) with n = %d scores" % (H.shape, K.shape, n))
        prm = capi.InstanceParams(max_instances, min_points, min_exclusive_fraction)
        buf = (capi.InstanceResult * max(n, 1))()
        sel = np.zeros(max(min(max(int(max_instances), 0), n), 1), np.int32); ns = C.c_int(0)
        capi.check(self.L.stocs_select_instances_rows(self.h, pH, K.ctypes.data_as(capi._u8p), pl, n, H.shape[1], int(nS), C.byref(prm), buf,
                                                      sel.ctypes.data_as(capi._ip), C.byref(ns)))
        return np.frombuffer(buf, dtype=_INSTANCE_DTYPE, count=n).copy(), sel[:ns.value].copy()

    def track_round(self, prior, round):
        n = C.c_int(0)
        capi.check(self.L.stocs_track_get_round(self.h, prior, round, None, None, 0, C.byref(n)))
        T = np.zeros((n.value, 16), np.float32); l = np.zeros(n.value, np.float32)
        capi.check(self.L.stocs_track_get_round(self.h, prior, round, T.ctypes.data_as(capi._fp), l.ctypes.data_as(capi._fp), n.value, C.byref(n)))
        return T, l

    def lcp_detail(self, T16):
        T, pT = capi.f32(T16)
        hit = np.zeros(self.nM, np.int32); counted = np.zeros(self.nM, np.uint8)
        capi.check(self.L.stocs_lcp_detail(self.h, pT, hit.ctypes.data_as(capi._ip), counted.ctypes.data_as(capi._u8p)))
        return hit, counted

    def lcp_hit_count(self, dT, n):
        h = C.c_int64(0); k = C.c_int64(0)
        capi.check(self.L.stocs_lcp_hit_count(self.h, dT, n, C.byref(h), C.byref(k)))
        return h.value, k.value

    def compute_best_transform(self):
        s = C.c_float(0); i = C.c_int(-1)
        P = np.zeros(16, np.float32)
        capi.check(self.L.stocs_verify_all(self.h, C.byref(s), C.byref(i), P.ctypes.data_as(capi._fp)))
        self.best_lcp, self.best_index, self.best_pose = s.value, i.value, P
        return s.value, i.value, P

    def run_trials(self, seeds, n_attempts=100, mode=0, dispersion=0.9, max_per_base=200, keep_details=False, post=None):
        sd = np.ascontiguousarray(seeds, np.uint64)
        res = (capi.TrialResult * max(len(sd), 1))()
        if post is None:
            capi.check(self.L.stocs_run_trials(self.h, mode, len(sd), sd.ctypes.data_as(C.POINTER(C.c_uint64)), n_attempts, dispersion, max_per_base,
                                               1 if keep_details else 0, res))
        else:
            pp = post if isinstance(post, capi.TrialPost) else trial_post(**post)
            capi.check(self.L.stocs_run_trials_post(self.h, mode, len(sd), sd.ctypes.data_as(C.POINTER(C.c_uint64)), n_attempts, dispersion, max_per_base,
                                                    1 if keep_details else 0, C.byref(pp), res))
        a = np.frombuffer(res, dtype=_TRIAL_DTYPE, count=len(sd))
        nb, nc, nq, bl, bi, bp = (a["n_bases"].tolist(), a["n_candidates"].tolist(), a["n_quads"].tolist(), a["best_lcp"].tolist(), a["best_index"].tolist(),
                                  a["best_pose16"].copy())
        return [dict(n_bases=nb[t], n_candidates=nc[t], n_quads=nq[t], best_lcp=bl[t], best_index=bi[t], best_pose=bp[t]) for t in range(len(sd))]

    def trial_bases(self, trial):
        n = C.c_int(0)
        capi.check(self.L.stocs_trials_get_bases(self.h, trial, None, None, None, 0, C.byref(n)))
        ids = np.zeros((n.value, 4), np.int32); inv = np.zeros((n.value, 2), np.float32); valid = np.zeros(n.value, np.int32)
        capi.check(self.L.stocs_trials_get_bases(self.h, trial, ids.ctypes.data_as(capi._ip), inv.ctypes.data_as(capi._fp), valid.ctypes.data_as(capi._ip),
                                                 n.value, C.byref(n)))
        return valid.astype(bool), ids, inv

    def trial_quad_counts(self, trial):
        n = C.c_int(0)
        capi.check(self.L.stocs_trials_get_quad_counts(self.h, trial, None, 0, C.byref(n)))
        out = np.zeros(n.value, np.int64)
        if n.value:
            capi.check(self.L.stocs_trials_get_quad_counts(self.h, trial, out.ctypes.data_as(capi._i64p), n.value, C.byref(n)))
        return out

    def trials_get_hypotheses(self, trial):
        n = C.c_int(0)
        capi.check(self.L.stocs_trials_get_hypotheses(self.h, trial, None, 0, C.byref(n)))
        buf = (capi.TrialHypothesis * max(n.value, 1))()
        if n.value:
            capi.check(self.L.stocs_trials_get_hypotheses(self.h, trial, buf, n.value, C.byref(n)))
        return np.frombuffer(buf, dtype=_HYP_DTYPE, count=n.value).copy()

    def trial_candidates(self, trial):
        n = C.c_int(0)
        capi.check(self.L.stocs_trials_get_candidates(self.h, trial, None, None, None, None, 0, C.byref(n)))
        T = np.zeros((n.value, 16), np.float32); P = np.zeros((n.value, 16), np.float32)
        l = np.zeros(n.value, np.float32); b = np.zeros(n.value, np.int32)
        if n.value:
            capi.check(self.L.stocs_trials_get_candidates(self.h, trial, T.ctypes.data_as(capi._fp), P.ctypes.data_as(capi._fp), l.ctypes.data_as(capi._fp),
                                                          b.ctypes.data_as(capi._ip), n.value, C.byref(n)))
        return T, P, l, b

    def dev_alloc(self, nbytes):
        p = C.c_void_p()
        capi.check(self.L.stocs_dev_alloc(self.h, nbytes, C.byref(p)))
        return p

    def dev_free(self, p):
        capi.check(self.L.stocs_dev_free(self.h, p))

    def dev_upload(self, p, arr):
        arr = np.ascontiguousarray(arr)
        capi.check(self.L.stocs_dev_upload(self.h, p, arr.ctypes.data_as(C.c_void_p), arr.nbytes))

    def dev_download(self, p, arr):
        capi.check(self.L.stocs_dev_download(self.h, arr.ctypes.data_as(C.c_void_p), p, arr.nbytes))

    def score_device(self, dT, n, dL):
        capi.check(self.L.stocs_score_transforms_device(self.h, dT, n, dL))

    def get_scene(self):
        pos = np.zeros((self.nS, 3), np.float32); nrm = np.zeros((self.nS, 3), np.float32)
        prob = np.zeros(self.nS, np.float32); pix = np.zeros((self.nS, 2), np.int32)
        capi.check(self.L.stocs_get_scene(self.h, pos.ctypes.data_as(capi._fp), nrm.ctypes.data_as(capi._fp), prob.ctypes.data_as(capi._fp),
                                          pix.ctypes.data_as(capi._ip)))
        return pos, nrm, prob, pix

    def get_segment(self):
# ... 253 lines not shown
```

Baseline: 71.40 million poses/s.

## Gate LCP cell scans with per-cell scene-normal cones

During grid build, each cell now stores a packed normal cone (octahedral axis plus sine class) in the upper bits of its count word, computed from the normals of the scene points in that cell. The LCP queue kernel transforms each model normal and skips the cell's point scan when the cone shows no scene normal can pass the normal-agreement threshold. This targets wasted distance checks on cells whose normals can never match, at the cost of an extra normal load and transform per model point and a longer grid build. A diagnostic gate_count API is also added to measure how often the gate fires.

```diff
diff --git a/include/stocs_hip.h b/include/stocs_hip.h
--- a/include/stocs_hip.h
+++ b/include/stocs_hip.h
@@ -95,6 +95,7 @@
 int stocs_score_best_device_async(stocs_ctx* ctx, const void* d_T16, int n, void* d_lcp, uint32_t id_offset, void* d_key8);
 int stocs_lcp_detail(stocs_ctx* ctx, const float* T16_centred_host, int32_t* hit, uint8_t* counted);
 int stocs_lcp_hit_count(stocs_ctx* ctx, const void* d_T16, int n, int64_t* hits, int64_t* counted);
+int stocs_lcp_gate_count(stocs_ctx* ctx, const void* d_T16, int n, int64_t out[3]);
 int stocs_verify_all(stocs_ctx* ctx, float* best_lcp, int* best_idx, float* best_pose16_camera);
 typedef struct stocs_trial_result {
     int32_t n_bases;
diff --git a/model_matching_amd/capi.py b/model_matching_amd/capi.py
--- a/model_matching_amd/capi.py
+++ b/model_matching_amd/capi.py
@@ -156,6 +156,7 @@
     "stocs_score_best_device": (C.c_int, [_vp, _vp, C.c_int, _vp, C.c_uint32, C.POINTER(C.c_uint64)]),
     "stocs_lcp_detail": (C.c_int, [_vp, _fp, _ip, _u8p]),
     "stocs_lcp_hit_count": (C.c_int, [_vp, _vp, C.c_int, _i64p, _i64p]),
+    "stocs_lcp_gate_count": (C.c_int, [_vp, _vp, C.c_int, _i64p]),
     "stocs_verify_all": (C.c_int, [_vp, _fp, _intp, _fp]),
     "stocs_run_trials": (C.c_int, [_vp, C.c_int, C.c_int, C.POINTER(C.c_uint64), C.c_int, C.c_float, C.c_int, C.c_int, C.POINTER(TrialResult)]),
     "stocs_trials_get_bases": (C.c_int, [_vp, C.c_int, _ip, _fp, _ip, C.c_int, _intp]),
diff --git a/model_matching_amd/csrc/ctx.hip b/model_matching_amd/csrc/ctx.hip
--- a/model_matching_amd/csrc/ctx.hip
+++ b/model_matching_amd/csrc/ctx.hip
@@ -486,6 +486,7 @@
     c->device_clock = (getenv("STOCS_DEVICE_CLOCK") && atoi(getenv("STOCS_DEVICE_CLOCK")) != 0) ? 1 : 0;
     c->lcp_split = 1;
     c->lcp_flat = getenv("STOCS_LCP_FLAT") ? atoi(getenv("STOCS_LCP_FLAT")) : 1;
+    c->lcp_normal_gate = 1;
     c->lcp_order = getenv("STOCS_LCP_ORDER") ? atoi(getenv("STOCS_LCP_ORDER")) : 1;
     c->exact_ties = 0; c->kd_ready = false; c->d_kd_nodes = NULL; c->d_kd_pts = NULL; c->d_ties = NULL; c->ties_started = false;
     c->cdf_n = 0; c->prior_epoch = 1; c->cdf_epoch = 0;
@@ -566,6 +567,7 @@
         }
         for (int i = 0; i < nM; ++i) { as[i] = a[c->h_mperm[i]]; bs[i] = b[c->h_mperm[i]]; }
         as.resize((size_t)n_patch * 64 + 64, make_float4(NAN, NAN, NAN, 0.f));
+        bs.resize((size_t)n_patch * 64 + 64, make_float4(0.f, 0.f, 0.f, 0.f));
         if (!rc) rc = upload(&c->d_mpos, a.data(), a.size());
         if (!rc) rc = upload(&c->d_mnrm, b.data(), b.size());
         if (!rc) rc = upload(&c->d_munit, u.data(), u.size());
diff --git a/model_matching_amd/csrc/grid.hip b/model_matching_amd/csrc/grid.hip
--- a/model_matching_amd/csrc/grid.hip
+++ b/model_matching_amd/csrc/grid.hip
@@ -6,6 +6,7 @@
 #include <algorithm>
 #include <vector>
 
+#include "normal_cone.h"
 #include "prims.h"
 #include "stocs_ctx.h"
 
@@ -126,7 +127,8 @@
                                                          const uint32_t* __restrict__ cell_brick, const uint32_t* __restrict__ list_off,
                                                          uint32_t n_cells, uint32_t n_inc, const uint32_t* __restrict__ vals,
                                                          const float4* __restrict__ spos, int32_t* __restrict__ top, uint4* __restrict__ cells,
-                                                         uint4* __restrict__ flat, const uint32_t* __restrict__ kept) {
+                                                         uint4* __restrict__ flat, const uint32_t* __restrict__ kept,
+                                                         const uint32_t* __restrict__ rank, const float4* __restrict__ snrmw, int cones) {
     const uint32_t c = blockIdx.x * 4 + (threadIdx.x >> 6);
     const int s = threadIdx.x & 63;
     if (c >= n_cells) return;
@@ -159,9 +161,52 @@
         const unsigned long long m = __ballot(any);
         mlo = (uint32_t)(m & 0xFFFFFFFFull); mhi = (uint32_t)(m >> 32);
     }
+    uint32_t cone = 0u;
+    if (cones) {
+        float4 n0 = make_float4(0.f, 0.f, 0.f, 0.f);
+        bool have0 = false, bad = false;
+        float sx = 0.f, sy = 0.f, sz = 0.f;
+        for (uint32_t k = (uint32_t)s; k < cnt; k += 64) {
+            if (rank && rank[first + k] == 0xFFFFFFFFu) continue;
+            const float4 nf = snrmw[vals[first + k]];
+            if (k < 64) { n0 = nf; have0 = true; }
+            const double n2 = (double)nf.x * nf.x + (double)nf.y * nf.y + (double)nf.z * nf.z;
+            if (!(n2 >= 0.99980001 && n2 <= 1.00020001)) { bad = true; continue; }
+            sx += nf.x; sy += nf.y; sz += nf.z;
+        }
+        for (int off = 32; off > 0; off >>= 1) { sx += __shfl_xor(sx, off, 64); sy += __shfl_xor(sy, off, 64); sz += __shfl_xor(sz, off, 64); }
+        const double l1 = fabs((double)sx) + fabs((double)sy) + fabs((double)sz);
+        if (!__any(bad) && l1 > 1.0e-9) {
+            double px = sx / l1, py = sy / l1;
+            if (sz < 0) { const double qx = (1.0 - fabs(py)) * (px >= 0 ? 1.0 : -1.0), qy = (1.0 - fabs(px)) * (py >= 0 ? 1.0 : -1.0); px = qx; py = qy; }
+            const double amax = (double)STOCS_CONE_AXIS_MAX;
+            const uint32_t u8 = (uint32_t)fmin(fmax(floor((px * 0.5 + 0.5) * amax + 0.5), 0.0), amax);
+            const uint32_t v8 = (uint32_t)fmin(fmax(floor((py * 0.5 + 0.5) * amax + 0.5), 0.0), amax);
+            float fx, fy, fz;
+            cone_axis(cone_pack(u8, v8, 0u), fx, fy, fz);
+            const double o2 = (double)fx * fx + (double)fy * fy + (double)fz * fz;
+            auto cos_down = [&](const float4 nf) {
+                const double n2 = (double)nf.x * nf.x + (double)nf.y * nf.y + (double)nf.z * nf.z;
+                return __double2float_rd(((double)nf.x * fx + (double)nf.y * fy + (double)nf.z * fz) / sqrt(n2 * o2));
+            };
+            float cmin = 1.0f;
+            if (have0) cmin = fminf(cmin, cos_down(n0));
+            for (uint32_t k = (uint32_t)s + 64; k < cnt; k += 64) {
+                if (rank && rank[first + k] == 0xFFFFFFFFu) continue;
+                cmin = fminf(cmin, cos_down(snrmw[vals[first + k]]));
+            }
+            for (int off = 32; off > 0; off >>= 1) cmin = fminf(cmin, __shfl_xor(cmin, off, 64));
+            if (cmin > 0.0f) {
+                const double cm = (double)cmin;
+                const double sd = sqrt(fmax((1.0 - cm) * (1.0 + cm), 0.0));
+                const uint32_t cls = (uint32_t)floor(sd * (double)STOCS_CONE_SIN_STEPS + 1.0e-4) + 1u;
+                if (cls <= STOCS_CONE_MAX_CLASS) cone = cone_pack(u8, v8, cls);
+            }
+        }
+    }
     if (s == 0) {
         top[brick] = (int32_t)b;
-        const uint4 w = make_uint4(list_off[c], kept ? kept[c] : cnt, mlo, mhi);
+        const uint4 w = make_uint4(list_off[c], (kept ? kept[c] : cnt) | cone, mlo, mhi);
         cells[(size_t)b * 512 + local] = w;
         if (flat) {
             const int bx = (int)(brick % (uint64_t)G.nbx), by = (int)((brick / (uint64_t)G.nbx) % (uint64_t)G.nby), bz = (int)(brick / ((uint64_t)G.nbx * (uint64_t)G.nby));
@@ -364,7 +409,7 @@
     g.nx = n[0]; g.ny = n[1]; g.nz = n[2];
     g.nbx = (n[0] + 7) / 8; g.nby = (n[1] + 7) / 8; g.nbz = (n[2] + 7) / 8;
     g.h = (float)h;
-    g.n_bricks = 0; g.n_entries = 0; g.avg_list_len = 0; g.has_nearest = false;
+    g.n_bricks = 0; g.n_entries = 0; g.avg_list_len = 0; g.has_nearest = false; g.has_cones = false;
     g.d_top = NULL; g.d_cells = NULL; g.d_list = NULL; g.d_chunk_r = NULL; g.d_flat = NULL;
     const int64_t n_top = (int64_t)g.nbx * g.nby * g.nbz;
     if (n_top > (int64_t)400 * 1000 * 1000) { set_error("scene extent too large for the brick grid"); return STOCS_ERR_INVALID; }
@@ -489,6 +534,7 @@
     const unsigned long long n_kept = prune ? rb64[1] : (unsigned long long)n_inc;
     const size_t n_list = tail[0];
     if (tail[1] > 65535u) { set_error("more than 65535 scene points within epsilon of one grid cell"); return STOCS_ERR_INVALID; }
+    g.has_cones = !(getenv("STOCS_GRID_CONES") && atoi(getenv("STOCS_GRID_CONES")) == 0);
     if ((rc = c->grid_mem.take(std::max<size_t>((size_t)n_bricks * 512, 1) * sizeof(uint4), (void**)&g.d_cells)) ||
         (rc = c->grid_mem.take(std::max<size_t>(n_list, 8) * sizeof(float4), (void**)&g.d_list)))
         return rc;
@@ -502,7 +548,8 @@
     }
     hipLaunchKernelGGL(fill_list_kernel, dim3(grid_of(std::max<size_t>(n_list, 8))), dim3(256), 0, st, g.d_list, std::max<size_t>(n_list, 8));
     hipLaunchKernelGGL(cell_words_kernel, dim3((unsigned)((n_cells + 3) / 4)), dim3(256), 0, st, G, div, d_cell_first, d_cell_key, d_cell_brick, d_list_off, n_cells,
-                       (uint32_t)n_inc, d_vals_s, c->d_spos, g.d_top, g.d_cells, g.d_flat, (const uint32_t*)d_kept);
+                       (uint32_t)n_inc, d_vals_s, c->d_spos, g.d_top, g.d_cells, g.d_flat, (const uint32_t*)d_kept,
+                       (const uint32_t*)d_rank, (const float4*)c->d_snrmw, g.has_cones ? 1 : 0);
     hipLaunchKernelGGL(list_fill_kernel, dim3(grid_of(n_inc)), dim3(256), 0, st, d_cflag, d_cidx, d_cell_first, d_list_off, d_vals_s, n_inc, c->d_spos, g.d_list, (const uint32_t*)d_rank);
     STOCS_HIP_CHECK(hipGetLastError());
     if (prune && div > 1) {
diff --git a/model_matching_amd/csrc/lcp.hip b/model_matching_amd/csrc/lcp.hip
--- a/model_matching_amd/csrc/lcp.hip
+++ b/model_matching_amd/csrc/lcp.hip
@@ -8,6 +8,7 @@
 #include <utility>
 
 #include "kdtree.h"
+#include "normal_cone.h"
 #include "prims.h"
 #include "stocs_ctx.h"
 
@@ -127,7 +128,8 @@
             if (brick >= 0) {
                 const uint4 cw = a.cells[(size_t)brick * 512 + (((cz & 7) << 6) | ((cy & 7) << 3) | (cx & 7))];
                 float bd = a.sq_eps;
-                for (uint32_t k = 0; k < cw.y; ++k) {
+                const uint32_t cn = cw.y & STOCS_CONE_COUNT_MASK;
+                for (uint32_t k = 0; k < cn; ++k) {
                     const float4 s = a.list[cw.x + k];
                     const float dx = qx - s.x, dy = qy - s.y, dz = qz - s.z;
                     const float d = dx * dx + (dy * dy + dz * dz);
@@ -219,7 +221,7 @@
                     if (!STOCS_ABLATE(a, 128)) cw = a.cells[(size_t)brick * 512 + (((cz & 7) << 6) | ((cy & 7) << 3) | (cx & 7))];
                     const int sb = ((int)((uz - fz) * 4.0f) << 4) | ((int)((uy - fy) * 4.0f) << 2) | (int)((ux - fx) * 4.0f);
                     const uint32_t mw = a.has_nearest ? 0xFFFFFFFFu : (sb < 32 ? cw.z : cw.w);
-                    off = cw.x; cnt = ((mw >> (sb & 31)) & 1u) ? cw.y : 0u;
+                    off = cw.x; cnt = ((mw >> (sb & 31)) & 1u) ? (cw.y & STOCS_CONE_COUNT_MASK) : 0u;
                     if (STOCS_ABLATE(a, 2)) cnt = cw.x == 0xFFFFFFF1u ? 1u : 0u;
                     const float ex = qx - (a.ox + ((float)cx + 0.5f) * a.h), ey = qy - (a.oy + ((float)cy + 0.5f) * a.h),
                                 ez = qz - (a.oz + ((float)cz + 0.5f) * a.h);
@@ -343,14 +345,14 @@
 
 constexpr int LCP_SHARED_LIVE = 512;
 
-constexpr bool lcp_queue_form_legal(bool detail, bool dense, bool split, bool flat, bool near, int cu, bool shared) {
-    return (cu == 16 || cu == 64) && (!shared || (split && cu == 16)) && (detail ? (!split && !flat && !(dense && near)) : (!dense || (split && !flat && !near)));
-}
-
-template <bool DETAIL, bool DENSE, bool SPLIT, bool FLAT, bool NEAR, int CU, bool SHARED>
+constexpr bool lcp_queue_form_legal(bool detail, bool dense, bool split, bool flat, bool near, int cu, bool shared, bool gate) {
+    return !(gate && (detail || dense || (split && cu == 16 && !shared))) && (cu == 16 || cu == 64) && (!shared || (split && cu == 16)) && (detail ? (!split && !flat && !(dense && near)) : (!dense || (split && !flat && !near)));
+}
+
+template <bool DETAIL, bool DENSE, bool SPLIT, bool FLAT, bool NEAR, int CU, bool SHARED, bool GATE>
 __global__ __launch_bounds__(64 * lcp_waves_per_block(DETAIL, SPLIT), 8) void lcp_coopq_kernel(LcpArgs a, const float* __restrict__ T16, float* __restrict__ out,
                                                         int n, int32_t* __restrict__ hit_out, uint8_t* __restrict__ cnt_out) {
-    static_assert(lcp_queue_form_legal(DETAIL, DENSE, SPLIT, FLAT, NEAR, CU, SHARED), "not one of the forms in the table above");
+    static_assert(lcp_queue_form_legal(DETAIL, DENSE, SPLIT, FLAT, NEAR, CU, SHARED, GATE), "not one of the forms in the table above");
     constexpr int WPB = lcp_waves_per_block(DETAIL, SPLIT);
     constexpr bool IDX = !DENSE;
     constexpr bool EARLY = DENSE;
@@ -522,7 +524,10 @@
 
     auto step = [&](const int i, const float4 p) {
         float qx = 0.f, qy = 0.f, qz = 0.f, qcentre = 0.f, nearest = 0.f;
-        uint32_t off = 0, cnt = 0;
+        uint32_t off = 0, cnt = 0, yw = 0;
+        float4 gnm = make_float4(0.f, 0.f, 0.f, 0.f);
+        if (GATE) gnm = a.mnrm[i];
+        constexpr uint32_t cmask = STOCS_CONE_COUNT_MASK;
         if (!DETAIL || i < a.M) {
             qx = ((t0 * p.x + t4 * p.y) + t8 * p.z) + t12;
             qy = ((t1 * p.x + t5 * p.y) + t9 * p.z) + t13;
@@ -537,14 +542,15 @@
                     if (!STOCS_ABLATE(a, 1))
                         cw = a.flat[(uint32_t)((cz * a.ny + cy) * a.nx + cx)];
                     const uint32_t mw = sb < 32 ? cw.z : cw.w;
-                    off = cw.x; cnt = ((mw >> (sb & 31)) & 1u) ? cw.y : 0u;
+                    off = cw.x; yw = cw.y; cnt = ((mw >> (sb & 31)) & 1u) ? (cw.y & cmask) : 0u;
                     if (STOCS_ABLATE(a, 2)) cnt = cw.x == 0xFFFFFFF1u ? 1u : 0u;
                 } else {
                     const int brick = a.top[((cz >> 3) * a.nby + (cy >> 3)) * a.nbx + (cx >> 3)];
                     if (brick >= 0) {
                         const uint4 cw = a.cells[(uint32_t)brick * 512u + (uint32_t)(((cz & 7) << 6) | ((cy & 7) << 3) | (cx & 7))];
-                        if ((EARLY || NEAR) && a.has_nearest) { off = cw.x; cnt = cw.y; nearest = __uint_as_float(cw.z); }
-                        else { const uint32_t mw = a.has_nearest ? 0xFFFFFFFFu : (sb < 32 ? cw.z : cw.w); off = cw.x; cnt = ((mw >> (sb & 31)) & 1u) ? cw.y : 0u; }
+                        yw = cw.y;
+                        if ((EARLY || NEAR) && a.has_nearest) { off = cw.x; cnt = cw.y & cmask; nearest = __uint_as_float(cw.z); }
+                        else { const uint32_t mw = a.has_nearest ? 0xFFFFFFFFu : (sb < 32 ? cw.z : cw.w); off = cw.x; cnt = ((mw >> (sb & 31)) & 1u) ? (cw.y & cmask) : 0u; }
                     }
                 }
             }
@@ -552,6 +558,12 @@
                 const float ex = qx - (a.ox + ((float)cx + 0.5f) * a.h), ey = qy - (a.oy + ((float)cy + 0.5f) * a.h), ez = qz - (a.oz + ((float)cz + 0.5f) * a.h);
                 qcentre = sqrtf(ex * ex + (ey * ey + ez * ez));
                 if (a.has_nearest && nearest - qcentre > a.eps + a.bound_margin) cnt = 0;
+            }
+            if (GATE && cnt) {
+                const float nx = t0 * gnm.x + (t4 * gnm.y + t8 * gnm.z);
+                const float ny = t1 * gnm.x + (t5 * gnm.y + t9 * gnm.z);
+                const float nz = t2 * gnm.x + (t6 * gnm.y + t10 * gnm.z);
+                if (cone_rules_out(yw, nx, ny, nz, a.dot_lo)) cnt = 0;
             }
             if (DETAIL && cnt == 0) {
                 const int orig = a.mperm[i];
@@ -758,7 +770,8 @@
             const int brick = a.top[((cz >> 3) * a.nby + (cy >> 3)) * a.nbx + (cx >> 3)];
             if (brick >= 0) {
                 const uint4 cw = a.cells[(size_t)brick * 512 + (((cz & 7) << 6) | ((cy & 7) << 3) | (cx & 7))];
-                for (uint32_t k = 0; k < cw.y; ++k) {
+                const uint32_t cn = cw.y & STOCS_CONE_COUNT_MASK;
+                for (uint32_t k = 0; k < cn; ++k) {
                     const float4 s = a.list[cw.x + k];
                     const float dx = qx - s.x, dy = qy - s.y, dz = qz - s.z;
                     const float d = dx * dx + (dy * dy + dz * dz);
@@ -858,12 +871,13 @@
     bool flat, near;
     int cu;
     bool shared;
+    bool gate;
 };
 
 static bool lcp_variant_selectable(int v) { return v == 99 || v == 0 || v == 24 || v == 31 || v == 39; }
 
 static LcpForm choose_lcp_form(const stocs_ctx* c, const LcpArgs& a, bool detail) {
-    LcpForm f = {LCP_QUEUE, detail, false, false, false, false, 64, false};
+    LcpForm f = {LCP_QUEUE, detail, false, false, false, false, 64, false, false};
     if (c->exact_ties) { f.kernel = LCP_EXACT; return f; }
     f.dense = c->grid.d_chunk_r != NULL;
     const int variant = c->lcp_variant >= 0 ? c->lcp_variant : 99;
@@ -877,6 +891,7 @@
         f.near = !f.dense && a.has_nearest;
         f.cu = (a.patch && c->lcp_cull_unit == 16) ? 16 : 64;
         f.shared = f.split && f.cu == 16 && a.M <= 16 * LCP_SHARED_LIVE;
+        f.gate = !detail && !f.dense && c->grid.has_cones && c->lcp_normal_gate != 0 && !(f.split && f.cu == 16 && !f.shared);
     }
     return f;
 }
@@ -887,14 +902,14 @@
 static LcpScanFn lcp_queue_fn() {
     constexpr bool DETAIL = (I & 1) != 0, DENSE = (I & 2) != 0, SPLIT = (I & 4) != 0, FLAT = (I & 8) != 0, NEAR = (I & 16) != 0;
     constexpr int CU = (I & 32) ? 16 : 64;
-    constexpr bool SHARED = (I & 64) != 0;
-    if constexpr (lcp_queue_form_legal(DETAIL, DENSE, SPLIT, FLAT, NEAR, CU, SHARED)) return lcp_coopq_kernel<DETAIL, DENSE, SPLIT, FLAT, NEAR, CU, SHARED>;
+    constexpr bool SHARED = (I & 64) != 0, GATE = (I & 128) != 0;
+    if constexpr (lcp_queue_form_legal(DETAIL, DENSE, SPLIT, FLAT, NEAR, CU, SHARED, GATE)) return lcp_coopq_kernel<DETAIL, DENSE, SPLIT, FLAT, NEAR, CU, SHARED, GATE>;
     else return NULL;
 }
 template <int... I>
 static LcpScanFn lcp_queue_fn(const LcpForm& f, std::integer_sequence<int, I...>) {
     static const LcpScanFn table[] = {lcp_queue_fn<I>()...};
-    return table[(f.detail ? 1 : 0) | (f.dense ? 2 : 0) | (f.split ? 4 : 0) | (f.flat ? 8 : 0) | (f.near ? 16 : 0) | (f.cu == 16 ? 32 : 0) | (f.shared ? 64 : 0)];
+    return table[(f.detail ? 1 : 0) | (f.dense ? 2 : 0) | (f.split ? 4 : 0) | (f.flat ? 8 : 0) | (f.near ? 16 : 0) | (f.cu == 16 ? 32 : 0) | (f.shared ? 64 : 0) | (f.gate ? 128 : 0)];
 }
 
 static int launch_lcp_form(stocs_ctx* c, const LcpForm& f, const LcpArgs& a, const float* d_T16, int n, float* d_lcp, int32_t* d_hit, uint8_t* d_counted) {
@@ -906,11 +921,11 @@
         else hipLaunchKernelGGL(lcp_exact_kernel<false>, grid, block, 0, c->stream, a, d_T16, d_lcp, n, d_hit, d_counted, c->d_kd_nodes, c->d_kd_pts, c->d_ties);
     } else {
         LcpScanFn fn = NULL;
-        if (f.kernel == LCP_QUEUE) fn = lcp_queue_fn(f, std::make_integer_sequence<int, 128>());
+        if (f.kernel == LCP_QUEUE) fn = lcp_queue_fn(f, std::make_integer_sequence<int, 256>());
         else if (f.kernel == LCP_STEP) fn = f.detail ? lcp_coop_kernel<true, false> : (f.split ? lcp_coop_kernel<false, true> : lcp_coop_kernel<false, false>);
         else if (!f.detail) fn = f.dense ? lcp_kernel<false, false> : lcp_kernel<false, true>;
         else if (!f.dense) fn = lcp_kernel<true, true>;
-        if (!fn) { set_error("launch_lcp: no kernel for this form (kernel %d, detail %d, dense %d, split %d, flat %d, near %d, cu %d, shared %d)", (int)f.kernel, (int)f.detail, (int)f.dense, (int)f.split, (int)f.flat, (int)f.near, f.cu, (int)f.shared); return STOCS_ERR_STATE; }
+        if (!fn) { set_error("launch_lcp: no kernel for this form (kernel %d, detail %d, dense %d, split %d, flat %d, near %d, cu %d, shared %d, gate %d)", (int)f.kernel, (int)f.detail, (int)f.dense, (int)f.split, (int)f.flat, (int)f.near, f.cu, (int)f.shared, (int)f.gate); return STOCS_ERR_STATE; }
         hipLaunchKernelGGL(fn, grid, block, 0, c->stream, a, d_T16, d_lcp, n, d_hit, d_counted);
     }
     STOCS_HIP_CHECK(hipGetLastError());
@@ -1102,6 +1117,89 @@
     return STOCS_OK;
 }
 
+__global__ __launch_bounds__(256) void gate_count_kernel(LcpArgs a, const float* __restrict__ T16, size_t total, const uint8_t* __restrict__ counted,
+                                                         unsigned long long* __restrict__ out3, int has_cones) {
+    const size_t g = (size_t)blockIdx.x * blockDim.x + threadIdx.x;
+    unsigned long long nq = 0, nr = 0, nb = 0;
+    if (g < total) {
+        const size_t cand = g / (size_t)a.M;
+        const int i = (int)(g % (size_t)a.M);
+        const float* T = T16 + cand * 16;
+        const float t0 = T[0], t1 = T[1], t2 = T[2], t4 = T[4], t5 = T[5], t6 = T[6], t8 = T[8], t9 = T[9], t10 = T[10], t12 = T[12], t13 = T[13], t14 = T[14];
+        const float4 p = a.mpos[i];
+        const float qx = ((t0 * p.x + t4 * p.y) + t8 * p.z) + t12;
+        const float qy = ((t1 * p.x + t5 * p.y) + t9 * p.z) + t13;
+        const float qz = ((t2 * p.x + t6 * p.y) + t10 * p.z) + t14;
+        const int c4x = __float2int_rd((qx - a.ox) * a.inv_h4), c4y = __float2int_rd((qy - a.oy) * a.inv_h4), c4z = __float2int_rd((qz - a.oz) * a.inv_h4);
+        const int cx = c4x >> 2, cy = c4y >> 2, cz = c4z >> 2;
+        uint32_t cnt = 0, yw = 0;
+        if ((unsigned)cx < (unsigned)a.nx && (unsigned)cy < (unsigned)a.ny && (unsigned)cz < (unsigned)a.nz) {
+            const int sb = ((c4z & 3) << 4) | ((c4y & 3) << 2) | (c4x & 3);
+            const int brick = a.top[((cz >> 3) * a.nby + (cy >> 3)) * a.nbx + (cx >> 3)];
+            if (brick >= 0) {
+                const uint4 cw = a.cells[(uint32_t)brick * 512u + (uint32_t)(((cz & 7) << 6) | ((cy & 7) << 3) | (cx & 7))];
+                const uint32_t mw = a.has_nearest ? 0xFFFFFFFFu : (sb < 32 ? cw.z : cw.w);
+                yw = cw.y; cnt = ((mw >> (sb & 31)) & 1u) ? (cw.y & STOCS_CONE_COUNT_MASK) : 0u;
+            }
+        }
+        if (cnt) {
+            nq = 1;
+            const float4 nm = a.mnrm[i];
+            const float nx = t0 * nm.x + (t4 * nm.y + t8 * nm.z);
+            const float ny = t1 * nm.x + (t5 * nm.y + t9 * nm.z);
+            const float nz = t2 * nm.x + (t6 * nm.y + t10 * nm.z);
+            if (has_cones && cone_rules_out(yw, nx, ny, nz, a.dot_lo)) {
+                nr = 1;
+                nb = counted[cand * (size_t)a.M + (size_t)a.mperm[i]] ? 1 : 0;
+            }
+        }
+    }
+    nq = lcp_wave_sum(nq); nr = lcp_wave_sum(nr); nb = lcp_wave_sum(nb);
+    if ((threadIdx.x & 63) == 0) { if (nq) atomicAdd(&out3[0], nq); if (nr) atomicAdd(&out3[1], nr); if (nb) atomicAdd(&out3[2], nb); }
+}
+
+int stocs_lcp_gate_count(stocs_ctx* c, const void* d_T16, int n, int64_t out[3]) {
+    if (!c || n < 0 || (n && !d_T16) || !out) return STOCS_ERR_INVALID;
+    DeviceGuard dev_guard(c->device);
+    begin_scoring_call(c);
+    out[0] = out[1] = out[2] = 0;
+    if (n == 0 || c->nM == 0 || c->nS == 0) return STOCS_OK;
+    const size_t M = (size_t)c->nM;
+    const int chunk = (int)std::max<size_t>(1, std::min<size_t>((size_t)n, ((size_t)256 << 20) / (5 * M)));
+    const size_t hb = al256((size_t)chunk * M * 4), cb = al256((size_t)chunk * M), lb = al256((size_t)chunk * 4);
+    int rc = ensure_scratch(c, 256 + lb + hb + cb);
+    if (rc) return rc;
+    char* base = (char*)c->d_scratch;
+    unsigned long long* d_out = (unsigned long long*)base;
+    float* dL = (float*)(base + 256);
+    int32_t* dH = (int32_t*)(base + 256 + lb);
+    uint8_t* dC = (uint8_t*)(base + 256 + lb + hb);
+    LcpArgs a;
+    memset(&a, 0, sizeof(a));
+    a.mpos = c->d_mpos_s; a.mnrm = c->d_mnrm_s; a.mperm = c->d_mperm; a.M = c->nM;
+    a.top = c->grid.d_top; a.cells = c->grid.d_cells;
+    a.ox = c->grid.ox; a.oy = c->grid.oy; a.oz = c->grid.oz; a.inv_h4 = c->grid.inv_h * 4.0f;
+    a.nx = c->grid.nx; a.ny = c->grid.ny; a.nz = c->grid.nz; a.nbx = c->grid.nbx; a.nby = c->grid.nby;
+    a.dot_lo = c->thr.lcp_dot_lo;
+    a.has_nearest = c->grid.has_nearest ? 1 : 0;
+    STOCS_HIP_CHECK(hipMemsetAsync(d_out, 0, 24, c->stream));
+    for (int i0 = 0; i0 < n; i0 += chunk) {
+        const int m = std::min(chunk, n - i0);
+        const float* dT = (const float*)d_T16 + (size_t)i0 * 16;
+        rc = launch_lcp(c, dT, m, dL, dH, dC, NULL, 0);
+        if (rc) return rc;
+        const size_t total = (size_t)m * M;
+        hipLaunchKernelGGL(gate_count_kernel, dim3((unsigned)((total + 255) / 256)), dim3(256), 0, c->stream, a, dT, total, (const uint8_t*)dC, d_out, c->grid.has_cones ? 1 : 0);
+        STOCS_HIP_CHECK(hipGetLastError());
+    }
+    if ((rc = ensure_pinned(c, PIN_VAR))) return rc;
+    unsigned long long* pin = (unsigned long long*)((char*)c->h_pin + PIN_BEST);
+    STOCS_HIP_CHECK(hipMemcpyAsync(pin, d_out, 24, hipMemcpyDeviceToHost, c->stream));
+    STOCS_HIP_CHECK(hipStreamSynchronize(c->stream));
+    for (int k = 0; k < 3; ++k) out[k] = (int64_t)pin[k];
+    return STOCS_OK;
+}
+
 int stocs_best_device(stocs_ctx* c, const void* d_lcp, int n, uint32_t id_offset, uint64_t* key) {
     if (!c || !key || n < 0 || (n && !d_lcp)) return STOCS_ERR_INVALID;
     DeviceGuard dev_guard(c->device);
@@ -1147,6 +1245,11 @@
     if (!strcmp(key, "lcp_order") && value >= 0 && value <= 4096) { c->lcp_order = value; return STOCS_OK; }
     if (!strcmp(key, "device_clock") && (value == 0 || value == 1)) { c->device_clock = value; return STOCS_OK; }
     if (!strcmp(key, "lcp_flat") && (value == 0 || value == 1)) { c->lcp_flat = value; return STOCS_OK; }
+    if (!strcmp(key, "lcp_normal_gate")) {
+        if (value != 0 && value != 1) { set_error("stocs_set_option: lcp_normal_gate takes 0 or 1, not %d", value); return STOCS_ERR_INVALID; }
+        c->lcp_normal_gate = value;
+        return STOCS_OK;
+    }
     if (!strcmp(key, "exact_ties")) {
         if (value != 0 && value != 1) { set_error("stocs_set_option: exact_ties takes 0 or 1, not %d", value); return STOCS_ERR_INVALID; }
         c->exact_ties = value;
diff --git a/model_matching_amd/csrc/normal_cone.h b/model_matching_amd/csrc/normal_cone.h
--- /dev/null
+++ b/model_matching_amd/csrc/normal_cone.h
@@ -0,0 +1,53 @@
+#ifndef STOCS_NORMAL_CONE_H
+#define STOCS_NORMAL_CONE_H
+
+#include "stocs_math.h"
+
+namespace stocs {
+
+#define STOCS_CONE_COUNT_MASK 0xFFFFu
+#define STOCS_CONE_MAX_CLASS 15u
+#define STOCS_CONE_AXIS_MAX 63u
+#define STOCS_CONE_SIN_STEPS 16.0f
+
+#if defined(__HIP_DEVICE_COMPILE__)
+#define STOCS_NC_FMAF(a, b, c) __fmaf_rn((a), (b), (c))
+#define STOCS_NC_SQRTF(a) __builtin_amdgcn_sqrtf(a)
+#define STOCS_NC_RSQRTF(a) __builtin_amdgcn_rsqf(a)
+#else
+#define STOCS_NC_FMAF(a, b, c) fmaf((a), (b), (c))
+#define STOCS_NC_SQRTF(a) sqrtf(a)
+#define STOCS_NC_RSQRTF(a) (1.0f / sqrtf(a))
+#endif
+
+STOCS_HD uint32_t cone_pack(uint32_t u8, uint32_t v8, uint32_t cls) { return (u8 << 16) | (v8 << 22) | (cls << 28); }
+STOCS_HD uint32_t cone_class(uint32_t y) { return y >> 28; }
+
+STOCS_HD void cone_axis(uint32_t yw, float& ox, float& oy, float& oz) {
+    float x = STOCS_NC_FMAF((float)((yw >> 16) & 63u), 2.0f / 63.0f, -1.0f);
+    float y0 = STOCS_NC_FMAF((float)((yw >> 22) & 63u), 2.0f / 63.0f, -1.0f);
+    const float z = (1.0f - fabsf(x)) - fabsf(y0);
+    const float t = fmaxf(-z, 0.0f);
+    x += x >= 0.0f ? -t : t;
+    y0 += y0 >= 0.0f ? -t : t;
+    ox = x; oy = y0; oz = z;
+}
+
+STOCS_HD bool cone_rules_out(uint32_t y, float vx, float vy, float vz, float dot_lo) {
+    float ox, oy, oz;
+    cone_axis(y, ox, oy, oz);
+    const float S = STOCS_NC_FMAF(ox, ox, STOCS_NC_FMAF(oy, oy, oz * oz));
+    const float W = STOCS_NC_FMAF(vx, ox, STOCS_NC_FMAF(vy, oy, vz * oz));
+    const float vv = STOCS_NC_FMAF(vx, vx, STOCS_NC_FMAF(vy, vy, vz * vz));
+    const float va = W * STOCS_NC_RSQRTF(S);
+    const float vp = STOCS_NC_SQRTF(fmaxf(STOCS_NC_FMAF(-va, va, vv), 0.0f));
+    const float sd = (float)cone_class(y) * (1.0f / STOCS_CONE_SIN_STEPS);
+    const float cd = STOCS_NC_SQRTF(STOCS_NC_FMAF(-sd, sd, 1.0f));
+    const float bound = STOCS_NC_FMAF(va, cd, vp * sd);
+    const float l1 = fabsf(vx) + (fabsf(vy) + fabsf(vz));
+    const bool outside = vp * cd > va * sd;
+    return cone_class(y) != 0u && outside && STOCS_NC_FMAF(bound, 1.0001f, 2.0e-3f * l1) < dot_lo;
+}
+
+}
+#endif
diff --git a/model_matching_amd/csrc/stocs_ctx.h b/model_matching_amd/csrc/stocs_ctx.h
--- a/model_matching_amd/csrc/stocs_ctx.h
+++ b/model_matching_amd/csrc/stocs_ctx.h
@@ -143,6 +143,7 @@
     float4* d_list;
     float* d_chunk_r;
     float h;
+    bool has_cones;
     bool has_nearest;
     float* d_dist;
     bool dist_ready;
@@ -242,6 +243,7 @@
     int device_clock;
     int lcp_split;
     int lcp_flat;
+    int lcp_normal_gate;
     int lcp_order;
     stocs::DevBlock order;
     int exact_ties;
diff --git a/model_matching_amd/estimator.py b/model_matching_amd/estimator.py
--- a/model_matching_amd/estimator.py
+++ b/model_matching_amd/estimator.py
@@ -513,6 +513,11 @@
         h = C.c_int64(0); k = C.c_int64(0)
         capi.check(self.L.stocs_lcp_hit_count(self.h, dT, n, C.byref(h), C.byref(k)))
         return h.value, k.value
+
+    def lcp_gate_count(self, dT, n):
+        out = (C.c_int64 * 3)(0, 0, 0)
+        capi.check(self.L.stocs_lcp_gate_count(self.h, dT, n, out))
+        return int(out[0]), int(out[1]), int(out[2])
 
     def compute_best_transform(self):
         s = C.c_float(0); i = C.c_int(-1)
```

New measurement: 76.15 million poses/s (median of 6 runs). +6.7%, better.
